# ma921/SOBER

Measured on AMD Instinct MI355X. Metric: recombination-step candidates/sec (N_rec=100000, N_nys=500, d=10, batch=100), higher is better.
Workload: dtype f64

## Files before the change

include/sober_hip.h:

```cpp
#ifndef SOBER_HIP_H
#define SOBER_HIP_H

#include <stdint.h>

#ifdef __cplusplus
extern "C" {
#endif

#define SOBER_ABI_VERSION 7

#define SOBER_KIND_RBF       0
#define SOBER_KIND_MATERN52  1
#define SOBER_KIND_TANIMOTO  2

#define SOBER_E_ARG      -1
#define SOBER_E_DIM      -2
#define SOBER_E_WS       -3
#define SOBER_E_EXCHANGE -5

int sober_abi_version(void);
int sober_diag_build(void);
int sober_reload_switches(void);
int sober_level_job_size(void);
int sober_nystrom_job_size(void);

int sober_padded_dim(int d);
int sober_bit_words(int d);

int sober_mt19937_uniform53(uint8_t* state, int64_t state_bytes, int64_t numel, double* out);
int sober_box_muller(const double* u, int64_t numel, double* out, void* stream);

int sober_scale_points(const double* X, int64_t n, int d, int64_t ldx,
                       const double* lengthscale, int ls_len,
                       double* out, int dt, void* stream);

int sober_scale_points_idx(const double* X, const int32_t* idx, int64_t n, int d, int64_t ldx, const double* lengthscale,
                           int ls_len, double* out, int dt, const double* gather_src, double* gather_out, void* stream);
int sober_pack_bits(const double* X, int64_t n, int d, int64_t ldx,
                    uint64_t* words, int nwords, double* norms, int32_t* bad_flag, void* stream);

int sober_pairwise(int kind, const void* a, const double* a_norm, int64_t m,
                   const void* b, const double* b_norm, const int32_t* idx, int64_t n,
                   int dt, double outputscale, double* out, int64_t ldo, void* stream);

int sober_kernel_matvec(int kind, const void* a, const double* a_norm, const double* v, int64_t m,
                        const void* b, const double* b_norm, int64_t n,
                        int dt, double outputscale, double c0, double* out, void* stream);

int sober_level_reduce(int kind, const void* rows, const double* rows_norm, int n_rows,
                       const void* cand, const double* cand_norm, int dt,
                       const int32_t* idx, int64_t pos0, int64_t count, int S,
                       const double* mu, const double* wmul, double outputscale,
                       int n_chunks, double* partG, int ldg, int col0,
                       double* partTot, int64_t tot_limit, void* stream);
int sober_aug_dim(int d);
int sober_augment_plan(const double* X_nys, int64_t M, int64_t ld_nys, const double* X_obs, int64_t n_obs, int64_t ld_obs,
                       const double* X_cand, int64_t N, int64_t ld_cand, int d, const double* lengthscale, int ls_len,
                       double* center, double* rows_aug, double* cand_aug, int da, void* stream);
int sober_augment_points(const double* X, int64_t n, int d, int64_t ldx, const double* lengthscale,
                         int ls_len, const double* center, int side, double* out, int da, void* stream);
int sober_level_reduce_mfma(int kind, const double* rows, int n_rows, const double* cand, int da,
                            const int32_t* idx, int64_t pos0, int64_t count, int S,
                            const double* mu, const double* wmul, double outputscale,
                            int n_chunks, double* partG, int ldg, int col0,
                            double* partTot, int64_t tot_limit, void* stream);

int64_t sober_nonzero_ws_bytes(int64_t N);
int sober_nonzero_i32(const double* mu, int64_t N, int32_t* idx_out, int64_t* count_out, void* ws, int64_t ws_bytes,
                      void* stream);

int sober_level_chunks(int n_rows, int64_t pos0, int64_t count, int S);
int sober_level_parts_mfma(int n_rows, int64_t pos0, int64_t count, int S);
int sober_level_parts_mfma_cap(int n_rows, int64_t e_total_ub, int S);

int sober_sum_partials(const double* partG, const double* partTot, int n_chunks, int n_rows,
                       int ldg, int S, const double* extraG, const double* extraTot,
                       int n_xchunks, int n_xcols, double* G, int ldo, double* tot, void* stream);

int sober_dgemm(int transa, int transb, int m, int n, int k, double alpha,
                const double* A, int lda, const double* B, int ldb,
                double beta, double* C, int ldc, void* stream);

int sober_barycentres(const double* Xtr, int ldx, int n, int S, const double* tot,
                      double* X_tmp, void* stream);
int sober_dgemm_coldiv_t(int m, int n, int k, const double* A, int lda, const double* B, int ldb, const double* coldiv,
                         double* Ct, int ldct, void* stream);

int sober_level_update(const int32_t* idx_cur, int64_t pos0, int64_t count, int S, int64_t E,
                       const int32_t* keep_rank, const double* w_star, const double* tot,
                       int n_keep, double* mu, int32_t* idx_new, int64_t new_pos0, void* stream);

int sober_scatter_weights(const int32_t* idx_cur, const int32_t* sel, const double* w, int n_sel,
                          double* mu, int64_t* out_idx, void* stream);

int sober_gather_f64(const double* src, const int32_t* idx, int64_t n, double* out, void* stream);
int sober_final_scatter(const int32_t* idx, int n, const int32_t* keep_rank, const double* w_star,
                        int64_t row_offset, double* mu, int64_t* out_idx, double* out_w, void* stream);
int sober_final_commit(const int32_t* idx, int n, const int32_t* keep_rank, const double* w_star, const int32_t* n_keep,
                       int64_t row_offset, double* mu, int64_t N, int64_t* out_idx, double* out_w, void* stream);

int sober_i64_to_i32(const int64_t* in, int64_t n, int32_t* out, void* stream);

int sober_car_pivot_host(double* h_Phi, int N, int m, double* h_mu);
int sober_car_pivot_host_fast(double* h_Phi, int N, int m, double* h_mu);

int sober_car_supported(int N, int m);
int64_t sober_car_ws_bytes(int N, int m);
int sober_car_device(const double* X, int ldx, int N, int m, const double* mu_in,
                     int32_t* keep_rank, double* w_star, int32_t* n_keep, double* mu_out,
                     double* phi_out, void* ws, int64_t ws_bytes, void* stream);
int sober_probe_rcp(const double* x, double* out, int64_t n, void* stream);

#define SOBER_CAR_DEFAULT 0
#define SOBER_CAR_SAFE 1
int sober_car_safe_supported(int N, int m);
int sober_car_giveup_forced(void);
int sober_car_device_ex(const double* X, int ldx, int N, int m, const double* mu_in,
                        int32_t* keep_rank, double* w_star, int32_t* n_keep, double* mu_out,
                        double* phi_out, void* ws, int64_t ws_bytes, int mode, void* stream);
int sober_obj_set_sums(const double* obj, const double* mu, const int32_t* idx, int64_t pos0, int64_t count, int S, int64_t E,
                       double* out, void* stream);
int sober_second_elimination(const double* phi, const double* objp, const double* w1, const int32_t* rank1, int n1,
                             int Nsets, int32_t* keep_rank, double* w_star, int32_t* n_keep, void* stream);
int sober_null_vector_supported(int nfun);
int sober_null_vector(const double* X, int ldx, int Nsets, int nfun, const int32_t* rank1, const int32_t* n_keep1, int n1,
                      double* null_row, int32_t* status, void* stream);
int sober_second_elimination_rows(const double* null_row, const double* obj_row, const double* w1, const int32_t* rank1,
                                  const int32_t* n_keep1, const int32_t* status, int n1, int Nsets, int32_t* keep_rank,
                                  double* w_star, int32_t* n_keep, void* stream);
int sober_obj_set_sums_queued(const double* obj, const double* mu, const int32_t* idx, int S, const int64_t* dR, int64_t R_known,
                              const double* tot, double* xcol, int ldx, double* ocol, void* stream);

int sober_car_mc_supported(int N, int m);
int64_t sober_car_mc_ws_bytes(int N, int m);
int sober_car_mc_device(const double* X, int ldx, int N, int m, const double* mu_in,
                        int32_t* keep_rank, double* w_star, int32_t* n_keep, double* mu_out,
                        double* phi_out, void* ws, int64_t ws_bytes, void* stream);
int sober_car_big_supported(int N, int m);
int64_t sober_car_big_ws_bytes(int N, int m);
int sober_car_big_device(const double* X, int ldx, int N, int m, const double* mu_in,
                         int32_t* keep_rank, double* w_star, int32_t* n_keep, double* mu_out,
                         double* phi_out, void* ws, int64_t ws_bytes, void* stream);
int sober_mc_selftest(const double* in, double* out, void* stream);

int sober_chol_max_n(void);
int sober_nystrom_max_n(void);
int sober_cholesky_probe_batched(const double* src, int n, int ld_src, const double* shifts, int n_shifts,
                                 double* work, int32_t* info, double* min_pivot, void* xinv_ws, int64_t ws_bytes,
                                 void* stream);
int sober_cholesky(double* A, int n, int ld, double shift, int32_t* info, double* min_pivot, void* stream);
int sober_cholesky_inv(double* A, int n, int ld, double shift, int32_t* info, double* min_pivot, double* xinv,
                       void* stream);
int sober_cholesky_inv_ratio(double* A, int n, int ld, double shift, int32_t* info, double* min_pivot, double* xinv,
                             double* ratio_out, void* stream);
int sober_trsm_blocks(const double* Y, int64_t m, int q, int ldy, const double* L, int ldl, const double* Xinv,
                      double* Q, int ldq, void* stream);
int sober_cholesky_probe(const double* src, int n, int ld_src, const double* shifts, int n_shifts,
                         double* work, int32_t* info, void* stream);
int sober_cholesky_probe_piv(const double* src, int n, int ld_src, const double* shifts, int n_shifts,
                             double* work, int32_t* info, double* min_pivot, void* stream);

int64_t sober_cholesky_probe_mc_ws_bytes(int n, int n_shifts);
int sober_cholesky_probe_mc(const double* src, int n, int ld_src, const double* shifts, int n_shifts,
                            double* work, int32_t* info, double* min_pivot, void* ws, int64_t ws_bytes,
                            void* stream);
int sober_abs_sym(const double* C, int n, int ld, double* out, int ldo, int32_t* flag, void* stream);
int sober_abs_sym_dmax(const double* C, int n, int ld, double* out, int ldo, int32_t* flag, double* dmax,
                       void* stream);

int sober_jitter_ladder(double* A, int n, int ld, int k, void* stream);
int sober_jitter_ladder_auto(double* A, int n, int ld, const int32_t* info, int n_rungs, int32_t* k_out,
                             void* stream);

int sober_level_reduce_tani_supported(int dt);
int sober_level_reduce_tani(const void* rows, const double* rows_norm, int n_rows, const void* cand,
                            const double* cand_norm, int dt, const int32_t* idx, int64_t pos0, int64_t count, int S,
                            const double* mu, const double* wmul, double outputscale, int n_chunks, double* partG,
                            int ldg, int col0, double* partTot, int64_t tot_limit, void* stream);

int sober_rank_scatter(const double* X, int ldx, int N, int n, const double* ocol, const int32_t* rank, int n1,
                       double* Xp, double* objp, void* stream);
int sober_set_i64(int64_t* dst, int64_t v, void* stream);

int sober_level_reduce_mfma_queued(int kind, const double* rows, int n_rows, const double* cand, int da,
                                   const int32_t* idx, int64_t count_ub, int S, int S_main, int leftover,
                                   const double* mu, const double* wmul, double outputscale, int n_chunks_ub,
                                   double* partG, int ldg, double* partTot, const int64_t* dR, void* stream);
int sober_level_reduce_mfma_queued_pair(int kind, const double* rows, int n_rows, const double* cand, int da,
                                        const int32_t* idx, int64_t count_ub, int S, int n_xcols, const double* mu,
                                        const double* wmul, double outputscale, int n_chunks_ub, double* partG,
                                        int ldg, double* partTot, int n_xchunks_ub, double* extraG, double* extraTot,
                                        const int64_t* dR, void* stream);
int sober_sum_partials_queued(const double* partG, const double* partTot, int n_rows, int ldg, int S,
                              const double* extraG, const double* extraTot, int n_xcols, double* G, int ldo,
                              double* tot, const int64_t* dR, int chunked, void* stream);
int sober_level_reduce_tani_queued(const void* rows, const double* rows_norm, int n_rows, const void* cand,
                                   const double* cand_norm, int dt, const int32_t* idx, int64_t count_ub, int S,
                                   int S_main, int leftover, const double* mu, const double* wmul, double outputscale,
                                   int n_chunks_ub, double* partG, int ldg, double* partTot, const int64_t* dR,
                                   void* stream);
int sober_level_reduce_tani_queued_pair(const void* rows, const double* rows_norm, int n_rows, const void* cand,
                                        const double* cand_norm, int dt, const int32_t* idx, int64_t count_ub, int S,
                                        int n_xcols, const double* mu, const double* wmul, double outputscale,
                                        int n_chunks_ub, double* partG, int ldg, double* partTot, int n_xchunks_ub,
                                        double* extraG, double* extraTot, const int64_t* dR, void* stream);
int sober_level_chunks_cap(int n_rows, int64_t e_total_ub, int S);
int sober_level_chunks_tani(int n_rows, int64_t pos0, int64_t count, int S);
int sober_level_chunks_tani_cap(int n_rows, int64_t e_total_ub, int S);
int sober_level_update_queued(const int32_t* idx_cur, int64_t R_ub, int S, const int32_t* keep_rank,
                              const double* w_star, const double* tot, double* mu, int32_t* idx_new,
                              const int64_t* dR_cur, int64_t* dR_next, int64_t R_ub_next, void* stream);

int sober_level_class_wpt(int n_rows, int64_t e_total, int S);
int sober_level_class_slots(int wpt);
int sober_level_reduce_mfma_wpt(int kind, const double* rows, int n_rows, const double* cand, int da,
                                const int32_t* idx, int64_t count, int S, const double* mu, const double* wmul,
                                double outputscale, int wpt, int n_chunks, double* partG, int ldg, double* partTot,
                                void* stream);
int sober_class_sum(const double* partG, const double* partTot, int n_chunks, int n_rows, int S, int CL,
                    double* Gc, double* totc, double* G, double* tot, void* stream);
int sober_class_derive_queued(const double* Gc, const double* totc, int n_rows, int S, int CL, const double* scale,
                              const int32_t* sof, double* Gn, double* totn, double* G, double* tot, const int64_t* dR,
                              void* stream);
int sober_level_update_queued_ex(const int32_t* idx_cur, int64_t R_ub, int S, const int32_t* keep_rank,
                                 const double* w_star, const double* tot, double* mu, int32_t* idx_new,
                                 const int64_t* dR_cur, int64_t* dR_next, int64_t R_ub_next, int need_keep,
                                 double* cls_scale, int32_t* cls_sof, int64_t R_known, void* stream);
int sober_level_update_queued_cls(const int32_t* idx_cur, int64_t R_ub, int S, const int32_t* keep_rank,
                                  const double* w_star, const double* tot, double* mu, int32_t* idx_new,
                                  const int64_t* dR_cur, int64_t* dR_next, int64_t R_ub_next, int need_keep,
                                  double* cls_scale, int32_t* cls_sof, void* stream);
#define SOBER_CLASS_MAX_DEPTH 4
int sober_level_class_depth(int variant, int n_rows, int64_t R, int S);

int64_t sober_kmeans_ws_bytes(int64_t N, int d, int K);
int64_t sober_kmeans_stat_offset(int64_t N, int d, int K);
int64_t sober_kmeans_ws_bytes_screened(int64_t N, int d, int K);
int sober_kmeans_lloyd(const double* X, int64_t N, int d, int K, int iters,
                       double* centroids, int32_t* labels, void* ws, int64_t ws_bytes, void* stream);

int sober_predict_fused_supported(int kind, int n_obs, int dt);
int sober_predict_fused(int kind, const void* obs, const double* obs_norm, int n_obs, const void* cand,
                        const double* cand_norm, int64_t N, int dt, double outputscale, const double* W, int ldw,
                        const double* alpha, double c0, double kxx_const, double noise, double* mean_out, double* var_out,
                        double eta, const double* eta_ptr, double* lfi_out, int log_flag, void* stream);
int sober_predict_fused_root(int kind, const void* obs, const double* obs_norm, int n_obs, const void* cand,
                             const double* cand_norm, int64_t N, int dt, double outputscale, const double* St, int ldst,
                             const int32_t* tri_flag, const double* alpha, double c0, double kxx_const, double noise,
                             double* mean_out, double* var_out, double eta, const double* eta_ptr, double* lfi_out, int log_flag,
                             void* stream);
int sober_predict_finish(const double* KX, const double* V, int n_obs, int64_t N, int64_t ld,
                         const double* mean, double kxx_const, const double* norms, double outputscale,
                         double noise, double* var_out, double eta, double* lfi_out, int log_flag,
                         void* stream);

int64_t sober_reduce_ws_bytes(int64_t n);
int sober_cleansing_weights(double* w, int64_t n, double eps, void* ws, int64_t ws_bytes, void* stream);

int sober_wkde_draw(const double* eps, int64_t n, int d, const int32_t* comp, const double* Xobs, int ldx,
                    const double* L, const double* lo, const double* hi, double* x, int32_t* inside,
                    void* stream);

int sober_level_gather(const double* Kmat, int n_rows, int64_t ldk, const int32_t* idx, int64_t pos0,
                       int64_t count, int S, const double* mu, const double* wmul, int n_chunks,
                       double* partG, int ldg, int col0, double* partTot, int64_t tot_limit, void* stream);

int sober_gspace_finish(double* K, const double* corr, int64_t n, int m, int64_t ldk, int64_t ldc,
                        const double* mug_cand, const double* mug_rows, void* stream);

#define SOBER_LEVEL_VALU        0
#define SOBER_LEVEL_MFMA        1
#define SOBER_LEVEL_GATHER      2
#define SOBER_LEVEL_TANI        3
#define SOBER_LEVEL_MAX_CHUNKS  64
#define SOBER_LEVEL_XS          16
typedef struct sober_level_job {
    int32_t variant, kind;
    const void* rows;   const double* rows_norm;
    const void* cand;   const double* cand_norm;
    int32_t n_rows, dim;
    int64_t kmat_ld;
    const double* wmul; double outputscale;
    int32_t S, n;
    const double* P;
    double *partG, *partTot, *extraG, *extraTot;
    double *G, *Xtr, *tot;
    double *X_tmp;
    int32_t* keep_rank;
    double *w_star, *mu_out;
    void* car_ws; int64_t car_ws_bytes;
    int32_t* h_flags;
    void* ev[4];
    const int32_t* idx; int64_t pos0, count, E;
    double* mu;
    int32_t phase;
    int64_t* dR; int64_t* h_dR;
    int32_t car_mode;
    uint64_t ev_used[2];
    int32_t class_depth;
    double* Gc[2]; double* totc[2];
    double* cls_scale; int32_t* cls_sof;
} sober_level_job;
#define SOBER_LEVEL_QUEUE 24
int sober_level_moments(const sober_level_job* job, void* stream);
int sober_level_car(const sober_level_job* job, void* stream);
int sober_level_car_retry(sober_level_job* job, void* stream);
#define SOBER_E_NOPROGRESS -4
int sober_level_loop(sober_level_job* job, int64_t R, int32_t* idx_a, int32_t* idx_b, int first_sums_ready,
                     void** events, int max_levels, int64_t* level_R, int32_t* n_levels, int64_t* R_final,
                     int32_t* in_b, void* stream);
typedef struct sober_obj_job {
    const double* obj;
    double* X_tmp;
    double* ocol;
    int32_t* kr1; double* w1; int32_t* nk1;
    double* null_row;
    int32_t* status;
} sober_obj_job;
int sober_obj_job_size(void);
int sober_level_loop_obj(sober_level_job* job, const sober_obj_job* obj_job, int64_t R, int32_t* idx_a, int32_t* idx_b,
                         int first_sums_ready, int max_levels, int64_t* level_R, int32_t* n_levels, int64_t* R_final,
                         int32_t* in_b, void* stream);
typedef int (*sober_allreduce_fn)(void* comm, double* buf, int64_t n, void* stream);
int sober_level_loop_sharded(sober_level_job* job, int rank, int world, int64_t* bounds, int32_t* idx_a,
                             int32_t* idx_b, int first_sums_ready, sober_allreduce_fn allreduce, void* comm,
                             int64_t R_stop, int max_levels, int64_t* level_R, int32_t* n_levels, int32_t* in_b,
                             void* stream);
int sober_rccl_load(const char* path);
int sober_rccl_unique_id(char* out128);
int sober_rccl_comm_init(const char* id128, int rank, int world, void** comm);
int sober_rccl_comm_destroy(void* comm);
int sober_rccl_allreduce_f64(void* comm, double* buf, int64_t n, void* stream);
int64_t sober_rccl_allreduce_ptr(void);

int64_t sober_peer_region_bytes(int64_t n_max);
int sober_peer_create(int rank, int world, int64_t n_max, void** comm, char* handle64);
int sober_peer_connect(void* comm, const char* handles);
int sober_peer_connect_ptrs(void* comm, void* const* regions);
int64_t sober_peer_region(void* comm);
int sober_peer_set_spin_limit(void* comm, unsigned spin_limit);
int sober_peer_allreduce_f64(void* comm, double* buf, int64_t n, void* stream);
int64_t sober_peer_allreduce_ptr(void);
int sober_peer_status(void* comm, double* restore, int64_t n, void* stream);
int sober_peer_destroy(void* comm);

int sober_level_final(const sober_level_job* job, const void* rows_sc, const double* rows_norm, const void* cand_sc,
                      const double* cand_norm, int dt, const int32_t* idx, int R, int64_t N, int64_t row_offset,
                      double* K, double* mu_live, int64_t* out_idx, double* out_w, void* stream);
int sober_plan_rows(int kind, const double* X_nys, int M, int64_t ld_nys, const double* X_obs, int n_obs,
                    int64_t ld_obs, int d, const double* lengthscale, int ls_len, double outputscale,
                    const double* S_cache, int ld_s, double* rows, int dt, double* Kall, double* W, double* T,
                    double* G, void* stream);

typedef struct sober_final_job {
    const void* rows_sc; const double* rows_norm;
    const void* cand_sc; const double* cand_norm;
    int32_t dt, done;
    int64_t N, row_offset;
    double *K, *mu_live;
    int64_t* out_idx; double* out_w;
    const double* cand_raw; int64_t ld_raw; int32_t d_raw, ls_len; const double* ls; double* sc_buf;
} sober_final_job;
int sober_level_final_job(const sober_level_job* job, const sober_final_job* final, const int32_t* idx, int R, void* stream);
int sober_final_job_size(void);
int sober_level_loop_final(sober_level_job* job, sober_final_job* final, int64_t R, int32_t* idx_a, int32_t* idx_b,
                           int first_sums_ready, void** events, int max_levels, int64_t* level_R, int32_t* n_levels,
                           int64_t* R_final, int32_t* in_b, void* stream);
int sober_projection(const double* Ut, int s, int M, const double* mean, const double* T, int n_obs, double* P,
                     void* stream);

typedef struct sober_nystrom_job {
    int32_t M, s, n_rungs, niter, probe_mc;
    int32_t reserved0;
    const double* G;
    const double* shifts;
    const double* R;
    double* C;
    double* chol_work;
    void* probe_ws; int64_t probe_ws_bytes;
    double* Y[2];
    double* Gm;
    double* xinv;
    void* flags_block; int64_t flags_bytes;
    void* h_flags_block;
    double* Ut;
    const double* T; int32_t n_obs;
    const double* mean_nys; double* P;
} sober_nystrom_job;
int64_t sober_nystrom_flags_bytes(int n_rungs, int niter);
int sober_nystrom_basis(const sober_nystrom_job* job, int phase, void* stream);

int sober_set_launch_events(void* start, void* stop);
int sober_record_event_pair(void* ev0, void* ev1, void* stream);

#ifdef __cplusplus
}
#endif
#endif
```

sober_amd/_native.py:

```python
from __future__ import annotations

import ctypes as C
import os
from typing import Optional

import torch

_HERE = os.path.dirname(os.path.abspath(__file__))
LIB_PATH = os.environ.get("SOBER_HIP_LIB") or os.path.join(_HERE, "libsober_hip.so")
ABI_VERSION = 7

KIND_RBF, KIND_MATERN52, KIND_TANIMOTO = 0, 1, 2
KIND_BY_NAME = {"rbf": KIND_RBF, "matern52": KIND_MATERN52, "tanimoto": KIND_TANIMOTO}

_vp, _i32, _i64, _f64 = C.c_void_p, C.c_int, C.c_int64, C.c_double

SIGNATURES = {
    "sober_abi_version": (_i32, []),
    "sober_diag_build": (_i32, []),
    "sober_reload_switches": (_i32, []),
    "sober_level_job_size": (_i32, []),
    "sober_nystrom_job_size": (_i32, []),
    "sober_final_job_size": (_i32, []),
    "sober_set_i64": (_i32, [_vp, _i64, _vp]),
    "sober_rank_scatter": (_i32, [_vp, _i32, _i32, _i32, _vp, _vp, _i32, _vp, _vp, _vp]),
    "sober_plan_rows": (_i32, [_i32, _vp, _i32, _i64, _vp, _i32, _i64, _i32, _vp, _i32, _f64, _vp, _i32, _vp, _i32, _vp,
                               _vp, _vp, _vp, _vp]),
    "sober_level_loop_final": (_i32, [_vp, _vp, _i64, _vp, _vp, _i32, _vp, _i32, _vp, _vp, _vp, _vp, _vp]),
    "sober_padded_dim": (_i32, [_i32]),
    "sober_bit_words": (_i32, [_i32]),
    "sober_scale_points": (_i32, [_vp, _i64, _i32, _i64, _vp, _i32, _vp, _i32, _vp]),
    "sober_augment_plan": (_i32, [_vp, _i64, _i64, _vp, _i64, _i64, _vp, _i64, _i64, _i32, _vp, _i32, _vp, _vp, _vp, _i32, _vp]),
    "sober_scale_points_idx": (_i32, [_vp, _vp, _i64, _i32, _i64, _vp, _i32, _vp, _i32, _vp, _vp, _vp]),
    "sober_pack_bits": (_i32, [_vp, _i64, _i32, _i64, _vp, _i32, _vp, _vp, _vp]),
    "sober_mt19937_uniform53": (_i32, [_vp, _i64, _i64, _vp]),
    "sober_box_muller": (_i32, [_vp, _i64, _vp, _vp]),
    "sober_pairwise": (_i32, [_i32, _vp, _vp, _i64, _vp, _vp, _vp, _i64, _i32, _f64, _vp, _i64, _vp]),
    "sober_kernel_matvec": (_i32, [_i32, _vp, _vp, _vp, _i64, _vp, _vp, _i64, _i32, _f64, _f64, _vp, _vp]),
    "sober_level_reduce": (_i32, [_i32, _vp, _vp, _i32, _vp, _vp, _i32, _vp, _i64, _i64, _i32, _vp, _vp,
                                  _f64, _i32, _vp, _i32, _i32, _vp, _i64, _vp]),
    "sober_nonzero_ws_bytes": (_i64, [_i64]),
    "sober_nonzero_i32": (_i32, [_vp, _i64, _vp, _vp, _vp, _i64, _vp]),
    "sober_dgemm_coldiv_t": (_i32, [_i32, _i32, _i32, _vp, _i32, _vp, _i32, _vp, _vp, _i32, _vp]),
    "sober_level_chunks": (_i32, [_i32, _i64, _i64, _i32]),
    "sober_level_parts_mfma": (_i32, [_i32, _i64, _i64, _i32]),
    "sober_level_parts_mfma_cap": (_i32, [_i32, _i64, _i32]),
    "sober_aug_dim": (_i32, [_i32]),
    "sober_augment_points": (_i32, [_vp, _i64, _i32, _i64, _vp, _i32, _vp, _i32, _vp, _i32, _vp]),
    "sober_level_reduce_mfma": (_i32, [_i32, _vp, _i32, _vp, _i32, _vp, _i64, _i64, _i32, _vp, _vp, _f64, _i32,
                                       _vp, _i32, _i32, _vp, _i64, _vp]),
    "sober_sum_partials": (_i32, [_vp, _vp, _i32, _i32, _i32, _i32, _vp, _vp, _i32, _i32, _vp, _i32, _vp, _vp]),
    "sober_dgemm": (_i32, [_i32, _i32, _i32, _i32, _i32, _f64, _vp, _i32, _vp, _i32, _f64, _vp, _i32, _vp]),
    "sober_barycentres": (_i32, [_vp, _i32, _i32, _i32, _vp, _vp, _vp]),
    "sober_level_update": (_i32, [_vp, _i64, _i64, _i32, _i64, _vp, _vp, _vp, _i32, _vp, _vp, _i64, _vp]),
    "sober_scatter_weights": (_i32, [_vp, _vp, _vp, _i32, _vp, _vp, _vp]),
    "sober_i64_to_i32": (_i32, [_vp, _i64, _vp, _vp]),
    "sober_car_pivot_host": (_i32, [_vp, _i32, _i32, _vp]),
    "sober_car_pivot_host_fast": (_i32, [_vp, _i32, _i32, _vp]),
    "sober_car_supported": (_i32, [_i32, _i32]),
    "sober_car_ws_bytes": (_i64, [_i32, _i32]),
    "sober_car_device": (_i32, [_vp, _i32, _i32, _i32, _vp, _vp, _vp, _vp, _vp, _vp, _vp, _i64, _vp]),
    "sober_probe_rcp": (_i32, [_vp, _vp, _i64, _vp]),
    "sober_second_elimination": (_i32, [_vp, _vp, _vp, _vp, _i32, _i32, _vp, _vp, _vp, _vp]),
    "sober_car_mc_supported": (_i32, [_i32, _i32]),
    "sober_car_mc_ws_bytes": (_i64, [_i32, _i32]),
    "sober_car_mc_device": (_i32, [_vp, _i32, _i32, _i32, _vp, _vp, _vp, _vp, _vp, _vp, _vp, _i64, _vp]),
    "sober_car_big_supported": (_i32, [_i32, _i32]),
    "sober_car_big_ws_bytes": (_i64, [_i32, _i32]),
    "sober_car_big_device": (_i32, [_vp, _i32, _i32, _i32, _vp, _vp, _vp, _vp, _vp, _vp, _vp, _i64, _vp]),
    "sober_car_device_ex": (_i32, [_vp, _i32, _i32, _i32, _vp, _vp, _vp, _vp, _vp, _vp, _vp, _i64, _i32, _vp]),
    "sober_obj_set_sums": (_i32, [_vp, _vp, _vp, _i64, _i64, _i32, _i64, _vp, _vp]),
    "sober_null_vector_supported": (_i32, [_i32]),
    "sober_null_vector": (_i32, [_vp, _i32, _i32, _i32, _vp, _vp, _i32, _vp, _vp, _vp]),
    "sober_second_elimination_rows": (_i32, [_vp, _vp, _vp, _vp, _vp, _vp, _i32, _i32, _vp, _vp, _vp, _vp]),
    "sober_obj_set_sums_queued": (_i32, [_vp, _vp, _vp, _i32, _vp, _i64, _vp, _vp, _i32, _vp, _vp]),
    "sober_obj_job_size": (_i32, []),
    "sober_level_loop_obj": (_i32, [_vp, _vp, _i64, _vp, _vp, _i32, _i32, _vp, _vp, _vp, _vp, _vp]),
    "sober_car_safe_supported": (_i32, [_i32, _i32]),
    "sober_car_giveup_forced": (_i32, []),
    "sober_final_commit": (_i32, [_vp, _i32, _vp, _vp, _vp, _i64, _vp, _i64, _vp, _vp, _vp]),
    "sober_level_car_retry": (_i32, [_vp, _vp]),
    "sober_mc_selftest": (_i32, [_vp, _vp, _vp]),
    "sober_chol_max_n": (_i32, []),
    "sober_nystrom_max_n": (_i32, []),
    "sober_cholesky_probe_batched": (_i32, [_vp, _i32, _i32, _vp, _i32, _vp, _vp, _vp, _vp, _i64, _vp]),
    "sober_cholesky": (_i32, [_vp, _i32, _i32, _f64, _vp, _vp, _vp]),
    "sober_cholesky_inv": (_i32, [_vp, _i32, _i32, _f64, _vp, _vp, _vp, _vp]),
    "sober_cholesky_inv_ratio": (_i32, [_vp, _i32, _i32, _f64, _vp, _vp, _vp, _vp, _vp]),
    "sober_trsm_blocks": (_i32, [_vp, _i64, _i32, _i32, _vp, _i32, _vp, _vp, _i32, _vp]),
    "sober_cholesky_probe": (_i32, [_vp, _i32, _i32, _vp, _i32, _vp, _vp, _vp]),
    "sober_cholesky_probe_piv": (_i32, [_vp, _i32, _i32, _vp, _i32, _vp, _vp, _vp, _vp]),
    "sober_cholesky_probe_mc_ws_bytes": (_i64, [_i32, _i32]),
    "sober_cholesky_probe_mc": (_i32, [_vp, _i32, _i32, _vp, _i32, _vp, _vp, _vp, _vp, _i64, _vp]),
    "sober_abs_sym": (_i32, [_vp, _i32, _i32, _vp, _i32, _vp, _vp]),
    "sober_abs_sym_dmax": (_i32, [_vp, _i32, _i32, _vp, _i32, _vp, _vp, _vp]),
    "sober_jitter_ladder": (_i32, [_vp, _i32, _i32, _i32, _vp]),
    "sober_jitter_ladder_auto": (_i32, [_vp, _i32, _i32, _vp, _i32, _vp, _vp]),
    "sober_kmeans_ws_bytes": (_i64, [_i64, _i32, _i32]),
    "sober_kmeans_stat_offset": (_i64, [_i64, _i32, _i32]),
    "sober_kmeans_ws_bytes_screened": (_i64, [_i64, _i32, _i32]),
    "sober_kmeans_lloyd": (_i32, [_vp, _i64, _i32, _i32, _i32, _vp, _vp, _vp, _i64, _vp]),
    "sober_predict_fused_supported": (_i32, [_i32, _i32, _i32]),
    "sober_predict_fused": (_i32, [_i32, _vp, _vp, _i32, _vp, _vp, _i64, _i32, _f64, _vp, _i32, _vp, _f64, _f64, _f64, _vp, _vp,
                                   _f64, _vp, _vp, _i32, _vp]),
    "sober_predict_fused_root": (_i32, [_i32, _vp, _vp, _i32, _vp, _vp, _i64, _i32, _f64, _vp, _i32, _vp, _vp, _f64, _f64, _f64, _vp,
                                        _vp, _f64, _vp, _vp, _i32, _vp]),
    "sober_predict_finish": (_i32, [_vp, _vp, _i32, _i64, _i64, _vp, _f64, _vp, _f64, _f64, _vp, _f64, _vp, _i32, _vp]),
    "sober_reduce_ws_bytes": (_i64, [_i64]),
    "sober_cleansing_weights": (_i32, [_vp, _i64, _f64, _vp, _i64, _vp]),
    "sober_level_gather": (_i32, [_vp, _i32, _i64, _vp, _i64, _i64, _i32, _vp, _vp, _i32, _vp, _i32, _i32, _vp, _i64,
                                  _vp]),
    "sober_gspace_finish": (_i32, [_vp, _vp, _i64, _i32, _i64, _i64, _vp, _vp, _vp]),
    "sober_wkde_draw": (_i32, [_vp, _i64, _i32, _vp, _vp, _i32, _vp, _vp, _vp, _vp, _vp, _vp]),
    "sober_level_moments": (_i32, [_vp, _vp]),
    "sober_level_car": (_i32, [_vp, _vp]),
    "sober_level_reduce_tani_supported": (_i32, [_i32]),
    "sober_level_reduce_tani": (_i32, [_vp, _vp, _i32, _vp, _vp, _i32, _vp, _i64, _i64, _i32, _vp, _vp, _f64, _i32, _vp,
                                       _i32, _i32, _vp, _i64, _vp]),
    "sober_level_loop_sharded": (_i32, [_vp, _i32, _i32, _vp, _vp, _vp, _i32, _vp, _vp, _i64, _i32, _vp, _vp, _vp, _vp]),
    "sober_rccl_load": (_i32, [C.c_char_p]),
    "sober_rccl_unique_id": (_i32, [_vp]),
    "sober_rccl_comm_init": (_i32, [_vp, _i32, _i32, _vp]),
    "sober_rccl_comm_destroy": (_i32, [_vp]),
    "sober_rccl_allreduce_f64": (_i32, [_vp, _vp, _i64, _vp]),
    "sober_rccl_allreduce_ptr": (_i64, []),
    "sober_peer_region_bytes": (_i64, [_i64]),
    "sober_peer_create": (_i32, [_i32, _i32, _i64, _vp, _vp]),
    "sober_peer_connect": (_i32, [_vp, C.c_char_p]),
    "sober_peer_connect_ptrs": (_i32, [_vp, _vp]),
    "sober_peer_region": (_i64, [_vp]),
    "sober_peer_set_spin_limit": (_i32, [_vp, C.c_uint]),
    "sober_peer_allreduce_f64": (_i32, [_vp, _vp, _i64, _vp]),
    "sober_peer_allreduce_ptr": (_i64, []),
    "sober_peer_status": (_i32, [_vp, _vp, _i64, _vp]),
    "sober_peer_destroy": (_i32, [_vp]),
    "sober_level_reduce_mfma_queued": (_i32, [_i32, _vp, _i32, _vp, _i32, _vp, _i64, _i32, _i32, _i32, _vp, _vp, _f64,
                                              _i32, _vp, _i32, _vp, _vp, _vp]),
    "sober_level_reduce_mfma_queued_pair": (_i32, [_i32, _vp, _i32, _vp, _i32, _vp, _i64, _i32, _i32, _vp, _vp, _f64, _i32,
                                                   _vp, _i32, _vp, _i32, _vp, _vp, _vp, _vp]),
    "sober_sum_partials_queued": (_i32, [_vp, _vp, _i32, _i32, _i32, _vp, _vp, _i32, _vp, _i32, _vp, _vp, _i32, _vp]),
    "sober_level_reduce_tani_queued": (_i32, [_vp, _vp, _i32, _vp, _vp, _i32, _vp, _i64, _i32, _i32, _i32, _vp, _vp, _f64,
                                              _i32, _vp, _i32, _vp, _vp, _vp]),
    "sober_level_reduce_tani_queued_pair": (_i32, [_vp, _vp, _i32, _vp, _vp, _i32, _vp, _i64, _i32, _i32, _vp, _vp, _f64, _i32,
                                                   _vp, _i32, _vp, _i32, _vp, _vp, _vp, _vp]),
    "sober_level_chunks_cap": (_i32, [_i32, _i64, _i32]),
    "sober_level_chunks_tani": (_i32, [_i32, _i64, _i64, _i32]),
    "sober_level_chunks_tani_cap": (_i32, [_i32, _i64, _i32]),
    "sober_level_update_queued": (_i32, [_vp, _i64, _i32, _vp, _vp, _vp, _vp, _vp, _vp, _vp, _i64, _vp]),
    "sober_level_update_queued_ex": (_i32, [_vp, _i64, _i32, _vp, _vp, _vp, _vp, _vp, _vp, _vp, _i64, _i32, _vp, _vp, _i64, _vp]),
    "sober_level_update_queued_cls": (_i32, [_vp, _i64, _i32, _vp, _vp, _vp, _vp, _vp, _vp, _vp, _i64, _i32, _vp, _vp, _vp]),
    "sober_level_class_wpt": (_i32, [_i32, _i64, _i32]),
    "sober_level_class_slots": (_i32, [_i32]),
    "sober_level_class_depth": (_i32, [_i32, _i32, _i64, _i32]),
    "sober_level_reduce_mfma_wpt": (_i32, [_i32, _vp, _i32, _vp, _i32, _vp, _i64, _i32, _vp, _vp, _f64, _i32, _i32, _vp, _i32,
                                           _vp, _vp]),
    "sober_class_sum": (_i32, [_vp, _vp, _i32, _i32, _i32, _i32, _vp, _vp, _vp, _vp, _vp]),
    "sober_class_derive_queued": (_i32, [_vp, _vp, _i32, _i32, _i32, _vp, _vp, _vp, _vp, _vp, _vp, _vp, _vp]),
    "sober_record_event_pair": (_i32, [_vp, _vp, _vp]),
    "sober_set_launch_events": (_i32, [_vp, _vp]),
    "sober_projection": (_i32, [_vp, _i32, _i32, _vp, _vp, _i32, _vp, _vp]),
    "sober_nystrom_flags_bytes": (_i64, [_i32, _i32]),
    "sober_nystrom_basis": (_i32, [_vp, _i32, _vp]),
    "sober_gather_f64": (_i32, [_vp, _vp, _i64, _vp, _vp]),
    "sober_final_scatter": (_i32, [_vp, _i32, _vp, _vp, _i64, _vp, _vp, _vp, _vp]),
    "sober_level_final": (_i32, [_vp, _vp, _vp, _vp, _vp, _i32, _vp, _i32, _i64, _i64, _vp, _vp, _vp, _vp, _vp]),
    "sober_level_final_job": (_i32, [_vp, _vp, _vp, _i32, _vp]),
    "sober_level_loop": (_i32, [_vp, _i64, _vp, _vp, _i32, _vp, _i32, _vp, _vp, _vp, _vp, _vp]),
}

LEVEL_VALU, LEVEL_MFMA, LEVEL_GATHER, LEVEL_TANI = 0, 1, 2, 3
LEVEL_MAX_CHUNKS, LEVEL_XS, LEVEL_QUEUE = 64, 16, 24


class FinalJob(C.Structure):
    _fields_ = [
        ("rows_sc", _vp), ("rows_norm", _vp), ("cand_sc", _vp), ("cand_norm", _vp),
        ("dt", _i32), ("done", _i32), ("N", _i64), ("row_offset", _i64),
        ("K", _vp), ("mu_live", _vp), ("out_idx", _vp), ("out_w", _vp),
        ("cand_raw", _vp), ("ld_raw", _i64), ("d_raw", _i32), ("ls_len", _i32), ("ls", _vp), ("sc_buf", _vp),
    ]


class ObjJob(C.Structure):
    _fields_ = [("obj", _vp), ("X_tmp", _vp), ("ocol", _vp), ("kr1", _vp), ("w1", _vp), ("nk1", _vp), ("null_row", _vp),
                ("status", _vp)]


class NystromJob(C.Structure):
    _fields_ = [
        ("M", _i32), ("s", _i32), ("n_rungs", _i32), ("niter", _i32), ("probe_mc", _i32), ("_pad0", _i32),
        ("G", _vp), ("shifts", _vp), ("R", _vp), ("C", _vp), ("chol_work", _vp),
        ("probe_ws", _vp), ("probe_ws_bytes", _i64),
        ("Y", _vp * 2), ("Gm", _vp), ("xinv", _vp),
        ("flags_block", _vp), ("flags_bytes", _i64), ("h_flags_block", _vp),
        ("Ut", _vp),
        ("T", _vp), ("n_obs", _i32), ("mean_nys", _vp), ("P", _vp),
    ]


class LevelJob(C.Structure):
    _fields_ = [
        ("variant", _i32), ("kind", _i32),
        ("rows", _vp), ("rows_norm", _vp), ("cand", _vp), ("cand_norm", _vp),
        ("n_rows", _i32), ("dim", _i32), ("kmat_ld", _i64),
        ("wmul", _vp), ("outputscale", _f64),
        ("S", _i32), ("n", _i32), ("P", _vp),
        ("partG", _vp), ("partTot", _vp), ("extraG", _vp), ("extraTot", _vp),
        ("G", _vp), ("Xtr", _vp), ("tot", _vp), ("X_tmp", _vp),
        ("keep_rank", _vp), ("w_star", _vp), ("mu_out", _vp),
        ("car_ws", _vp), ("car_ws_bytes", _i64), ("h_flags", _vp),
        ("ev", _vp * 4),
        ("idx", _vp), ("pos0", _i64), ("count", _i64), ("E", _i64), ("mu", _vp),
        ("phase", _i32),
        ("dR", _vp), ("h_dR", _vp),
        ("car_mode", _i32),
        ("ev_used", C.c_uint64 * 2),
        ("class_depth", _i32), ("Gc", _vp * 2), ("totc", _vp * 2), ("cls_scale", _vp), ("cls_sof", _vp),
    ]

E_DIM = -2
E_EXCHANGE = -5
CLASS_MAX_DEPTH = 4
CAR_DEFAULT, CAR_SAFE, CAR_HOST = 0, 1, 2

_lib: Optional[C.CDLL] = None


class SoberHipError(RuntimeError):
    pass


def load() -> C.CDLL:
    global _lib
    if _lib is not None:
        return _lib
    if not os.path.exists(LIB_PATH):
        raise SoberHipError(
            f"{LIB_PATH} not found: build it with `make -C sober_amd/csrc` "
            "(python -c 'import __graft_entry__ as g; g.build()').  sober_amd has no CPU fallback.")
    lib = C.CDLL(LIB_PATH)
    lib.sober_abi_version.restype = _i32
    got = lib.sober_abi_version()
    if got != ABI_VERSION:
        raise SoberHipError(f"libsober_hip ABI {got} != expected {ABI_VERSION}; rebuild (make -C sober_amd/csrc)")
    for name, (res, args) in SIGNATURES.items():
        fn = getattr(lib, name)
        fn.restype, fn.argtypes = res, args
    if lib.sober_diag_build() and os.environ.get("SOBER_ALLOW_DIAG_LIB") != "1":
        raise SoberHipError(f"{LIB_PATH} is a diagnostic build (in-kernel time stamps): not a library to compute with; "
                            "`make -C sober_amd/csrc` builds the product (SOBER_ALLOW_DIAG_LIB=1: the stamp scripts)")
    for name, cls in (("sober_level_job_size", LevelJob), ("sober_nystrom_job_size", NystromJob),
                      ("sober_final_job_size", FinalJob), ("sober_obj_job_size", ObjJob)):
        if getattr(lib, name)() != C.sizeof(cls):
            raise SoberHipError(f"{cls.__name__}: {C.sizeof(cls)} bytes here, {getattr(lib, name)()} in libsober_hip; "
                                "include/sober_hip.h and sober_amd/_native.py disagree")
    _lib = lib
    return lib


def reload_switches():
    load().sober_reload_switches()


def _check(rc: int, what: str):
    if rc == 0:
        return
    if rc < 0:
        msg = {-1: "bad argument", -2: "dimension not supported by the compiled tile set",
               -3: "workspace too small",
               -5: "a multi-workgroup Caratheodory kernel gave up waiting for a partner workgroup (no result)"}.get(rc, "error")
        raise SoberHipError(f"{what}: {msg} (code {rc})")
    raise SoberHipError(f"{what}: hipError_t {rc}")


def _ptr(t: Optional[torch.Tensor]) -> Optional[int]:
    return None if t is None else t.data_ptr()


_raw_stream = getattr(torch._C, "_cuda_getCurrentRawStream", None)


def _stream(t: torch.Tensor) -> Optional[int]:
    if not t.is_cuda:
        raise SoberHipError("sober_amd runs on the MI355X only: tensor is not on a HIP device")
    if _raw_stream is not None:
        return _raw_stream(t.device.index)
    return torch.cuda.current_stream(t.device).cuda_stream


def _req(t: torch.Tensor, dtype, name: str):
    if t.dtype != dtype or not t.is_contiguous():
        raise SoberHipError(f"{name}: need contiguous {dtype}, got {t.dtype} contiguous={t.is_contiguous()}")
    return t


def padded_dim(d: int, generic: bool = False) -> int:
    r = load().sober_padded_dim(d)
    if r == E_DIM and generic and d > 0:
        return (d + 3) // 4 * 4
    _check(min(r, 0), f"padded_dim({d})")
    return r


def bit_words(d: int, generic: bool = False) -> int:
    r = load().sober_bit_words(d)
    if r == E_DIM and generic and d > 0:
        return (d + 63) // 64
    _check(min(r, 0), f"bit_words({d})")
    return r


def fused_dim_supported(kind: int, d: int) -> bool:
    r = load().sober_bit_words(d) if kind == KIND_TANIMOTO else load().sober_padded_dim(d)
    return r > 0


def scale_points_idx(X, idx, n, lengthscale, out):
    _req(lengthscale, torch.float64, "lengthscale"); _req(out, torch.float64, "out"); _req(idx, torch.int32, "idx")
    if X.dtype != torch.float64 or X.stride(-1) != 1:
        raise SoberHipError("scale_points_idx: X must be float64 with unit inner stride")
    _check(load().sober_scale_points_idx(X.data_ptr(), idx.data_ptr(), int(n), X.shape[1], X.stride(0), lengthscale.data_ptr(),
                                         lengthscale.numel(), out.data_ptr(), out.shape[1], None, None, _stream(X)),
           "sober_scale_points_idx")


def scale_points(X, lengthscale, out):
    n, d = X.shape
    _req(X, torch.float64, "X"); _req(lengthscale, torch.float64, "lengthscale"); _req(out, torch.float64, "out")
    _check(load().sober_scale_points(X.data_ptr(), n, d, X.stride(0), lengthscale.data_ptr(),
                                     lengthscale.numel(), out.data_ptr(), out.shape[1], _stream(X)),
           "sober_scale_points")


def mt19937_uniform53(state, numel, out):
    _req(state, torch.uint8, "state"); _req(out, torch.float64, "out")
    if state.is_cuda or out.is_cuda or out.numel() < numel + 16:
        raise ValueError("mt19937_uniform53 takes host tensors, out of numel + 16 doubles")
    _check(load().sober_mt19937_uniform53(state.data_ptr(), state.numel(), numel, out.data_ptr()),
           "sober_mt19937_uniform53")


def box_muller(u, numel, out):
    _req(u, torch.float64, "u"); _req(out, torch.float64, "out")
    if u.numel() < numel + 16 or out.numel() < numel:
        raise ValueError("box_muller: u holds numel + 16 uniforms, out numel normals")
    _check(load().sober_box_muller(u.data_ptr(), numel, out.data_ptr(), _stream(out)), "sober_box_muller")


def pack_bits(X, words, norms, bad_flag):
    n, d = X.shape
    _req(X, torch.float64, "X"); _req(words, torch.int64, "words"); _req(norms, torch.float64, "norms")
    _req(bad_flag, torch.int32, "bad_flag")
    _check(load().sober_pack_bits(X.data_ptr(), n, d, X.stride(0), words.data_ptr(), words.shape[1],
                                  norms.data_ptr(), bad_flag.data_ptr(), _stream(X)), "sober_pack_bits")


def rank_scatter(X, n, ocol, rank, n1, Xp, objp):
    _req(X, torch.float64, "X"); _req(ocol, torch.float64, "ocol"); _req(rank, torch.int32, "rank")
    _check(load().sober_rank_scatter(X.data_ptr(), X.stride(0), X.shape[0], n, ocol.data_ptr(), rank.data_ptr(), n1,
                                     Xp.data_ptr(), objp.data_ptr(), _stream(X)), "sober_rank_scatter")


def plan_rows(kind, X_nys, X_obs, lengthscale, outputscale, S_cache, rows, Kall, W, T, G):
    M, d = X_nys.shape
    n_obs = 0 if X_obs is None else X_obs.shape[0]
    for t in (X_nys, X_obs, S_cache, rows, Kall, W, T, G):
        if t is not None and (t.dtype != torch.float64 or t.stride(-1) != 1):
            raise SoberHipError("plan_rows: float64 tensors with unit inner stride")
    _check(load().sober_plan_rows(kind, X_nys.data_ptr(), M, X_nys.stride(0), _ptr(X_obs), n_obs,
                                  X_obs.stride(0) if X_obs is not None else 0, d, lengthscale.data_ptr(),
                                  lengthscale.numel(), float(outputscale), _ptr(S_cache),
                                  S_cache.stride(0) if S_cache is not None else 0, rows.data_ptr(), rows.shape[1],
                                  _ptr(Kall), _ptr(W), _ptr(T), G.data_ptr(), _stream(G)), "sober_plan_rows")


def pairwise(kind, a, a_norm, b, b_norm, idx, n, dt, outputscale, out):
    _check(load().sober_pairwise(kind, a.data_ptr(), _ptr(a_norm), a.shape[0], b.data_ptr(), _ptr(b_norm),
                                 _ptr(idx), n, dt, float(outputscale), out.data_ptr(), out.stride(0),
                                 _stream(out)), "sober_pairwise")


def kernel_matvec(kind, a, a_norm, v, b, b_norm, dt, outputscale, c0, out):
    _check(load().sober_kernel_matvec(kind, a.data_ptr(), _ptr(a_norm), v.data_ptr(), a.shape[0],
                                      b.data_ptr(), _ptr(b_norm), b.shape[0], dt, float(outputscale),
                                      float(c0), out.data_ptr(), _stream(out)), "sober_kernel_matvec")


def nonzero_ws_bytes(N) -> int:
    r = load().sober_nonzero_ws_bytes(N)
    _check(min(int(r), 0), "sober_nonzero_ws_bytes")
    return int(r)


def nonzero_i32(mu, idx_out, count_out, ws):
    _req(mu, torch.float64, "mu"); _req(idx_out, torch.int32, "idx_out"); _req(count_out, torch.int64, "count_out")
    _check(load().sober_nonzero_i32(mu.data_ptr(), mu.numel(), idx_out.data_ptr(), count_out.data_ptr(), ws.data_ptr(),
                                    ws.numel() * ws.element_size(), _stream(mu)), "sober_nonzero_i32")


def level_chunks(n_rows, pos0, count, S) -> int:
    r = load().sober_level_chunks(n_rows, pos0, count, S)
    _check(min(r, 0), "sober_level_chunks")
    return r


def level_parts_mfma(n_rows, pos0, count, S) -> int:
    r = load().sober_level_parts_mfma(n_rows, pos0, count, S)
    _check(min(r, 0), "sober_level_parts_mfma")
    return r


def level_reduce(kind, rows, rows_norm, cand, cand_norm, dt, idx, idx_off, pos0, count, S, mu, wmul,
                 outputscale, n_chunks, partG, ldg, col0, partTot, tot_limit):
    _req(idx, torch.int32, "idx"); _req(mu, torch.float64, "mu")
    _check(load().sober_level_reduce(kind, rows.data_ptr(), _ptr(rows_norm), rows.shape[0], cand.data_ptr(),
                                     _ptr(cand_norm), dt, idx.data_ptr() + 4 * idx_off, pos0, count, S,
                                     mu.data_ptr(), _ptr(wmul), float(outputscale), n_chunks,
                                     partG.data_ptr(), ldg, col0, _ptr(partTot), tot_limit, _stream(mu)),
           "sober_level_reduce")


def aug_dim(d: int) -> int:
    r = load().sober_aug_dim(d)
    return r if r > 0 else -1


def augment_plan(X_nys, X_obs, X_cand, lengthscale, center, rows_aug, cand_aug):
    for t_, nm in ((X_nys, "X_nys"), (X_cand, "X_cand"), (X_obs, "X_obs")):
        if t_ is not None and (t_.dtype != torch.float64 or t_.stride(-1) != 1):
            raise SoberHipError(f"augment_plan: {nm} must be float64 with unit inner stride")
    _req(rows_aug, torch.float64, "rows_aug"); _req(cand_aug, torch.float64, "cand_aug"); _req(center, torch.float64, "center")
    n_obs = 0 if X_obs is None else X_obs.shape[0]
    _check(load().sober_augment_plan(X_nys.data_ptr(), X_nys.shape[0], X_nys.stride(0), _ptr(X_obs), n_obs,
                                     X_obs.stride(0) if n_obs else 0, X_cand.data_ptr(), X_cand.shape[0], X_cand.stride(0),
                                     X_nys.shape[1], lengthscale.data_ptr(), lengthscale.numel(), center.data_ptr(),
                                     rows_aug.data_ptr(), cand_aug.data_ptr(), rows_aug.shape[1], _stream(X_cand)),
           "sober_augment_plan")


def augment_points(X, lengthscale, center, side, out):
    n, d = X.shape
    _req(X, torch.float64, "X"); _req(out, torch.float64, "out"); _req(center, torch.float64, "center")
    _check(load().sober_augment_points(X.data_ptr(), n, d, X.stride(0), lengthscale.data_ptr(),
                                       lengthscale.numel(), center.data_ptr(), side, out.data_ptr(),
                                       out.shape[1], _stream(X)), "sober_augment_points")


def level_reduce_mfma(kind, rows, cand, da, idx, idx_off, pos0, count, S, mu, wmul, outputscale, n_chunks,
                      partG, ldg, col0, partTot, tot_limit):
    _req(idx, torch.int32, "idx"); _req(mu, torch.float64, "mu")
    _check(load().sober_level_reduce_mfma(kind, rows.data_ptr(), rows.shape[0], cand.data_ptr(), da,
                                          idx.data_ptr() + 4 * idx_off, pos0, count, S, mu.data_ptr(),
                                          _ptr(wmul), float(outputscale), n_chunks, partG.data_ptr(), ldg,
                                          col0, _ptr(partTot), tot_limit, _stream(mu)),
           "sober_level_reduce_mfma")


def sum_partials(partG, partTot, n_chunks, n_rows, ldg, S, extraG, extraTot, n_xchunks, n_xcols, G, tot):
    _check(load().sober_sum_partials(partG.data_ptr(), _ptr(partTot), n_chunks, n_rows, ldg, S,
                                     _ptr(extraG), _ptr(extraTot), n_xchunks, n_xcols, G.data_ptr(),
                                     G.stride(0), _ptr(tot), _stream(G)), "sober_sum_partials")


def dgemm(A, B, C_, transa=False, transb=False, alpha=1.0, beta=0.0):
    m, n = C_.shape
    k = A.shape[0] if transa else A.shape[1]
    for t, nm in ((A, "A"), (B, "B"), (C_, "C")):
        if t.dtype != torch.float64 or t.stride(1) != 1:
            raise SoberHipError(f"dgemm {nm}: need float64 with unit inner stride")
    ka = B.shape[1] if transb else B.shape[0]
    ma = A.shape[1] if transa else A.shape[0]
    na = B.shape[0] if transb else B.shape[1]
    if (ma, na, ka) != (m, n, k):
        raise SoberHipError(f"dgemm shape mismatch {A.shape} {B.shape} -> {C_.shape}")
    _check(load().sober_dgemm(int(transa), int(transb), m, n, k, float(alpha), A.data_ptr(), A.stride(0),
                              B.data_ptr(), B.stride(0), float(beta), C_.data_ptr(), C_.stride(0),
                              _stream(C_)), "sober_dgemm")


def barycentres(Xtr, n, S, tot, X_tmp):
    _check(load().sober_barycentres(Xtr.data_ptr(), Xtr.stride(0), n, S, _ptr(tot), X_tmp.data_ptr(),
                                    _stream(X_tmp)), "sober_barycentres")


def level_update(idx_cur, idx_off, pos0, count, S, E, keep_rank, w_star, tot, n_keep, mu, idx_new, new_pos0):
    _check(load().sober_level_update(idx_cur.data_ptr() + 4 * idx_off, pos0, count, S, E,
                                     keep_rank.data_ptr(), w_star.data_ptr(), tot.data_ptr(), n_keep,
                                     mu.data_ptr(), idx_new.data_ptr(), new_pos0, _stream(mu)),
           "sober_level_update")


def scatter_weights(idx_cur, sel, w, n_sel, mu, out_idx):
    _check(load().sober_scatter_weights(idx_cur.data_ptr(), sel.data_ptr(), w.data_ptr(), n_sel,
                                        mu.data_ptr(), out_idx.data_ptr(), _stream(mu)),
           "sober_scatter_weights")


def i64_to_i32(src, dst):
    _check(load().sober_i64_to_i32(src.data_ptr(), src.numel(), dst.data_ptr(), _stream(src)),
           "sober_i64_to_i32")


def car_pivot_host(Phi: torch.Tensor, mu: torch.Tensor, fast=None) -> int:
    if Phi.is_cuda or mu.is_cuda:
        raise SoberHipError("car_pivot_host takes host tensors")
    _req(Phi, torch.float64, "Phi"); _req(mu, torch.float64, "mu")
    N, m = Phi.shape
    fn = load().sober_car_pivot_host_fast if (fast or (fast is None and N > 200)) else load().sober_car_pivot_host
    r = fn(Phi.data_ptr(), N, m, mu.data_ptr())
    _check(min(r, 0), "sober_car_pivot_host")
    return r


_CAR_WS = {}


def car_supported(N: int, m: int) -> bool:
    return bool(load().sober_car_supported(N, m))


def car_safe_supported(N: int, m: int) -> bool:
    return bool(load().sober_car_safe_supported(N, m))


def probe_rcp(x):
    out = torch.empty_like(x)
    _check(load().sober_probe_rcp(x.data_ptr(), out.data_ptr(), x.numel(), _stream(x)), "sober_probe_rcp")
    return out


def car_device(X, mu_in, keep_rank, w_star, n_keep, mu_out, phi_out=None, multi_cu=False, mode=CAR_DEFAULT, big=False):
    N, n = X.shape
    lib = load()
    if mode != CAR_DEFAULT and not multi_cu and not big:
        nbytes = lib.sober_car_ws_bytes(N, n + 1)
        ws = _CAR_WS.get(X.device)
        if ws is None or ws.numel() * 8 < nbytes:
            ws = _CAR_WS[X.device] = torch.empty(max(nbytes // 8, 1), dtype=torch.float64, device=X.device)
        _check(lib.sober_car_device_ex(X.data_ptr(), X.stride(0), N, n + 1, mu_in.data_ptr(), keep_rank.data_ptr(),
                                       w_star.data_ptr(), n_keep.data_ptr(), mu_out.data_ptr(), _ptr(phi_out),
                                       ws.data_ptr(), nbytes, int(mode), _stream(X)), "sober_car_device_ex")
        return
    nbytes = max(lib.sober_car_ws_bytes(N, n + 1), lib.sober_car_mc_ws_bytes(N, n + 1) if multi_cu else 0,
                 lib.sober_car_big_ws_bytes(N, n + 1) if big else 0)
    ws = _CAR_WS.get(X.device)
    if ws is None or ws.numel() * 8 < nbytes:
        ws = torch.empty(max(nbytes // 8, 1), dtype=torch.float64, device=X.device)
        _CAR_WS[X.device] = ws
    fn, name = (lib.sober_car_big_device, "sober_car_big_device") if big else \
        (lib.sober_car_mc_device, "sober_car_mc_device") if multi_cu else (lib.sober_car_device, "sober_car_device")
    _check(fn(X.data_ptr(), X.stride(0), N, n + 1, mu_in.data_ptr(), keep_rank.data_ptr(),
              w_star.data_ptr(), n_keep.data_ptr(), mu_out.data_ptr(), _ptr(phi_out),
              ws.data_ptr(), nbytes, _stream(X)), name)


def obj_set_sums(obj, mu, idx, pos0, count, S, E, out):
    _req(obj, torch.float64, "obj"); _req(mu, torch.float64, "mu"); _req(idx, torch.int32, "idx"); _req(out, torch.float64, "out")
    _check(load().sober_obj_set_sums(obj.data_ptr(), mu.data_ptr(), idx.data_ptr(), int(pos0), int(count), int(S), int(E),
                                     out.data_ptr(), _stream(mu)), "sober_obj_set_sums")


def null_vector(X, nfun, rank1, n_keep1, n1, null_row, status):
    _check(load().sober_null_vector(X.data_ptr(), X.stride(0), X.shape[0], int(nfun), rank1.data_ptr(), n_keep1.data_ptr(),
                                    int(n1), null_row.data_ptr(), status.data_ptr(), _stream(X)), "sober_null_vector")


def second_elimination_rows(null_row, obj_row, w1, rank1, n_keep1, n1, keep_rank, w_star, n_keep, status=None):
    _check(load().sober_second_elimination_rows(null_row.data_ptr(), obj_row.data_ptr(), w1.data_ptr(), rank1.data_ptr(),
                                                n_keep1.data_ptr(), _ptr(status), int(n1), rank1.numel(), keep_rank.data_ptr(),
                                                w_star.data_ptr(), n_keep.data_ptr(), _stream(null_row)),
           "sober_second_elimination_rows")


def level_loop_obj(job, obj_job, R, idx_a, idx_b, first_sums_ready, stream):
    level_R = (_i64 * MAX_LEVELS)()
    n_levels, in_b, R_final = _i32(0), _i32(0), _i64(0)
    _check(load().sober_level_loop_obj(C.addressof(job), C.addressof(obj_job), R, idx_a.data_ptr(), idx_b.data_ptr(),
                                       int(bool(first_sums_ready)), MAX_LEVELS, level_R, C.byref(n_levels), C.byref(R_final),
                                       C.byref(in_b), stream), "sober_level_loop_obj")
    return list(level_R[:n_levels.value]), int(R_final.value), bool(in_b.value)


def second_elimination(phi, objp, w1, rank1, n1, keep_rank, w_star, n_keep):
    _check(load().sober_second_elimination(phi.data_ptr(), objp.data_ptr(), w1.data_ptr(), rank1.data_ptr(), int(n1),
                                           rank1.numel(), keep_rank.data_ptr(), w_star.data_ptr(), n_keep.data_ptr(),
                                           _stream(phi)), "sober_second_elimination")


def mc_selftest(x: torch.Tensor) -> torch.Tensor:
    out = torch.empty(128, dtype=torch.float64, device=x.device)
    _check(load().sober_mc_selftest(x.data_ptr(), out.data_ptr(), _stream(x)), "sober_mc_selftest")
    return out


def chol_max_n() -> int:
    return load().sober_chol_max_n()


def nystrom_max_n() -> int:
    return load().sober_nystrom_max_n()


def cholesky(A, shift, info, min_pivot=None):
    n = A.shape[0]
    _check(load().sober_cholesky(A.data_ptr(), n, A.stride(0), float(shift), info.data_ptr(), _ptr(min_pivot),
                                 _stream(A)), "sober_cholesky")


def cholesky_inv(A, shift, info, min_pivot, xinv, ratio=None):
    n = A.shape[0]
    if xinv.numel() < ((n + 31) // 32) * 1024:
        raise SoberHipError("cholesky_inv: xinv too small")
    _check(load().sober_cholesky_inv_ratio(A.data_ptr(), n, A.stride(0), float(shift), info.data_ptr(), _ptr(min_pivot),
                                           xinv.data_ptr(), _ptr(ratio), _stream(A)), "sober_cholesky_inv")


def trsm_blocks(Y, L, xinv, Q):
    m, q = Y.shape
    _check(load().sober_trsm_blocks(Y.data_ptr(), m, q, Y.stride(0), L.data_ptr(), L.stride(0), xinv.data_ptr(),
                                    Q.data_ptr(), Q.stride(0), _stream(Y)), "sober_trsm_blocks")


def cholesky_probe(src, shifts, work, info, min_pivot=None):
    n = src.shape[0]
    _check(load().sober_cholesky_probe_piv(src.data_ptr(), n, src.stride(0), shifts.data_ptr(), shifts.numel(),
                                           work.data_ptr(), info.data_ptr(), _ptr(min_pivot), _stream(src)),
           "sober_cholesky_probe_piv")


PROBE_NO_VERDICT = -7


def cholesky_probe_mc_ws_bytes(n: int, n_shifts: int) -> int:
    return int(load().sober_cholesky_probe_mc_ws_bytes(n, n_shifts))


def cholesky_probe_mc(src, shifts, work, info, min_pivot, ws):
    n = src.shape[0]
    _check(load().sober_cholesky_probe_mc(src.data_ptr(), n, src.stride(0), shifts.data_ptr(), shifts.numel(),
                                          work.data_ptr(), info.data_ptr(), _ptr(min_pivot), ws.data_ptr(),
                                          ws.numel() * ws.element_size(), _stream(src)), "sober_cholesky_probe_mc")


def abs_sym(C_, out, flag, dmax=None):
    n = C_.shape[0]
    _check(load().sober_abs_sym_dmax(C_.data_ptr(), n, C_.stride(0), out.data_ptr(), out.stride(0), flag.data_ptr(),
                                     _ptr(dmax), _stream(C_)), "sober_abs_sym")


def kmeans_lloyd(X, K, iters, centroids, labels):
    N, d = X.shape
    _req(X, torch.float64, "X"); _req(centroids, torch.float64, "centroids"); _req(labels, torch.int32, "labels")
    nbytes = int(load().sober_kmeans_ws_bytes(N, d, K))
    ws = torch.empty(max(nbytes, 8), dtype=torch.uint8, device=X.device)
    _check(load().sober_kmeans_lloyd(X.data_ptr(), N, d, K, iters, centroids.data_ptr(), labels.data_ptr(),
                                     ws.data_ptr(), nbytes, _stream(X)), "sober_kmeans_lloyd")


def predict_fused_supported(kind: int, n_obs: int, dt: int) -> bool:
    return bool(load().sober_predict_fused_supported(int(kind), int(n_obs), int(dt)))


def predict_fused(kind, obs, obs_norm, cand, cand_norm, n, dt, outputscale, W, alpha, c0, kxx_const, noise, mean_out,
                  var_out, eta=0.0, lfi_out=None, log=False, eta_dev=None, root_tri=None):
    if W.dtype != torch.float64 or W.dim() != 2 or W.stride(1) != 1:
        raise SoberHipError(f"predict_fused: W must be float64 with unit inner stride, got {W.dtype} strides {tuple(W.stride())}")
    if cand.dtype == torch.float64 and (cand.dim() != 2 or cand.stride(1) != 1 or cand.stride(0) != dt):
        raise SoberHipError(f"predict_fused: candidates must be rows of {dt} contiguous float64, got strides {tuple(cand.stride())}")
    for t_, nm in ((alpha, "alpha"), (mean_out, "mean_out"), (var_out, "var_out"), (lfi_out, "lfi_out"), (eta_dev, "eta_dev")):
        if t_ is not None:
            _req(t_, torch.float64, "predict_fused: " + nm)
    if alpha is not None and alpha.numel() != obs.shape[0]:
        raise SoberHipError(f"predict_fused: alpha has {alpha.numel()} entries for {obs.shape[0]} observations")
    if root_tri is not None:
        _req(root_tri, torch.int32, "predict_fused: root_tri")
        if W.shape[0] != W.shape[1] or W.shape[0] != obs.shape[0]:
            raise SoberHipError(f"predict_fused: the root must be {obs.shape[0]} x {obs.shape[0]}, got {tuple(W.shape)}")
        _check(load().sober_predict_fused_root(int(kind), obs.data_ptr(), _ptr(obs_norm), obs.shape[0], cand.data_ptr(),
                                               _ptr(cand_norm), int(n), int(dt), float(outputscale), W.data_ptr(), W.stride(0),
                                               root_tri.data_ptr(), _ptr(alpha), float(c0), float(kxx_const), float(noise),
                                               _ptr(mean_out), var_out.data_ptr(), float(eta), _ptr(eta_dev), _ptr(lfi_out),
                                               int(bool(log)), _stream(cand)), "sober_predict_fused_root")
        return
    _check(load().sober_predict_fused(int(kind), obs.data_ptr(), _ptr(obs_norm), obs.shape[0], cand.data_ptr(),
                                      _ptr(cand_norm), int(n), int(dt), float(outputscale), W.data_ptr(), W.stride(0),
                                      _ptr(alpha), float(c0), float(kxx_const), float(noise), _ptr(mean_out),
                                      var_out.data_ptr(), float(eta), _ptr(eta_dev), _ptr(lfi_out), int(bool(log)),
                                      _stream(cand)),
           "sober_predict_fused")


def predict_finish(KX, V, mean, kxx_const, norms, outputscale, noise, var_out, eta=0.0, lfi_out=None, log=False):
    n_obs, N = KX.shape
    _check(load().sober_predict_finish(KX.data_ptr(), V.data_ptr(), n_obs, N, KX.stride(0), _ptr(mean),
                                       float(kxx_const), _ptr(norms), float(outputscale), float(noise),
                                       var_out.data_ptr(), float(eta), _ptr(lfi_out), int(bool(log)),
                                       _stream(KX)), "sober_predict_finish")


def cleansing_weights(w, eps):
    _req(w, torch.float64, "weights")
    nbytes = load().sober_reduce_ws_bytes(w.numel())
    ws = torch.empty(nbytes // 8 + 1, dtype=torch.float64, device=w.device)
    _check(load().sober_cleansing_weights(w.data_ptr(), w.numel(), float(eps), ws.data_ptr(), nbytes,
                                          _stream(w)), "sober_cleansing_weights")


def wkde_draw(eps, comp, Xobs, L, lo, hi, x, inside):
    n, d = eps.shape
    _check(load().sober_wkde_draw(eps.data_ptr(), n, d, comp.data_ptr(), Xobs.data_ptr(), Xobs.stride(0),
                                  L.data_ptr(), lo.data_ptr() if lo is not None else None,
                                  hi.data_ptr() if hi is not None else None, x.data_ptr(),
                                  inside.data_ptr() if inside is not None else None, _stream(eps)),
           "sober_wkde_draw")


def level_gather(Kmat, idx, idx_off, pos0, count, S, mu, wmul, n_chunks, partG, ldg, col0, partTot, tot_limit):
    _req(idx, torch.int32, "idx"); _req(mu, torch.float64, "mu"); _req(Kmat, torch.float64, "Kmat")
    if Kmat.stride(1) != 1:
        raise SoberHipError("level_gather: Kmat needs unit inner stride")
    _check(load().sober_level_gather(Kmat.data_ptr(), Kmat.shape[1], Kmat.stride(0),
                                     idx.data_ptr() + 4 * idx_off, pos0, count, S, mu.data_ptr(), _ptr(wmul),
                                     n_chunks, partG.data_ptr(), ldg, col0, _ptr(partTot), tot_limit,
                                     _stream(partG)), "sober_level_gather")


def gspace_finish(K, corr, mug_cand, mug_rows):
    n, m = K.shape
    _check(load().sober_gspace_finish(K.data_ptr(), corr.data_ptr(), n, m, K.stride(0), corr.stride(0),
                                      mug_cand.data_ptr(), mug_rows.data_ptr(), _stream(K)), "sober_gspace_finish")


def car_ws_bytes(N: int, m: int) -> int:
    return load().sober_car_ws_bytes(N, m)


def level_moments(job: LevelJob, stream: int):
    _check(load().sober_level_moments(C.addressof(job), stream), "sober_level_moments")


def level_car(job: LevelJob, stream: int):
    _check(load().sober_level_car(C.addressof(job), stream), "sober_level_car")


def level_car_retry(job: LevelJob, stream: int) -> bool:
    rc = load().sober_level_car_retry(C.addressof(job), stream)
    if rc == E_EXCHANGE:
        return False
    _check(rc, "sober_level_car_retry")
    return True


E_NOPROGRESS = -4
MAX_LEVELS = 64


def level_loop(job: LevelJob, R: int, idx_a, idx_b, first_sums_ready: bool, events, stream: int, final: "FinalJob" = None):
    level_R = (_i64 * MAX_LEVELS)()
    n_levels, in_b, R_final = _i32(0), _i32(0), _i64(0)
    ev = None
    if events is not None:
        ev = (_vp * (4 * MAX_LEVELS))(*events)
    if final is not None:
        rc = load().sober_level_loop_final(C.addressof(job), C.addressof(final), R, idx_a.data_ptr(), idx_b.data_ptr(),
                                           int(bool(first_sums_ready)), ev, MAX_LEVELS, level_R, C.byref(n_levels),
                                           C.byref(R_final), C.byref(in_b), stream)
    else:
        rc = load().sober_level_loop(C.addressof(job), R, idx_a.data_ptr(), idx_b.data_ptr(), int(bool(first_sums_ready)),
                                     ev, MAX_LEVELS, level_R, C.byref(n_levels), C.byref(R_final), C.byref(in_b), stream)
    if rc == E_NOPROGRESS:
        raise RuntimeError("recombination made no progress (the Caratheodory step cancelled nothing, "
                           "SOBER/_rchq.py:241-242); the reference would loop forever here")
    if rc != E_EXCHANGE:
        _check(rc, "sober_level_loop")
    return list(level_R[:n_levels.value]), int(R_final.value), bool(in_b.value), rc == E_EXCHANGE


ALLREDUCE_FN = C.CFUNCTYPE(_i32, _vp, _vp, _i64, _vp)


def level_loop_sharded(job: LevelJob, rank: int, world: int, bounds, idx_a, idx_b, first_sums_ready: bool,
                       allreduce_ptr, comm_ptr, R_stop: int, stream: int):
    level_R = (_i64 * MAX_LEVELS)()
    n_levels, in_b = _i32(0), _i32(0)
    b = (_i64 * (world + 1))(*bounds)
    rc = load().sober_level_loop_sharded(C.addressof(job), rank, world, b, idx_a.data_ptr(), idx_b.data_ptr(),
                                         int(bool(first_sums_ready)), allreduce_ptr, comm_ptr, int(R_stop), MAX_LEVELS,
                                         level_R, C.byref(n_levels), C.byref(in_b), stream)
    if rc == E_NOPROGRESS:
        raise RuntimeError("recombination made no progress (the Caratheodory step cancelled nothing, "
                           "SOBER/_rchq.py:241-242); the reference would loop forever here")
    _check(rc, "sober_level_loop_sharded")
    return list(level_R[:n_levels.value]), list(b), bool(in_b.value)


class RcclComm:

    def __init__(self, dist, group, device):
        import torch as _t
        lib = load()
        path = os.path.join(os.path.dirname(_t.__file__), "lib", "librccl.so")
        _check(lib.sober_rccl_load(path.encode() if os.path.exists(path) else b""), "sober_rccl_load")
        rank, world = dist.get_rank(group), dist.get_world_size(group)
        buf = (C.c_char * 128)()
        if rank == 0:
            _check(lib.sober_rccl_unique_id(C.addressof(buf)), "sober_rccl_unique_id")
        on_dev = dist.get_backend(group) == "nccl"
        t = _t.frombuffer(bytearray(buf.raw), dtype=_t.uint8).clone()
        t = t.to(device) if on_dev else t
        dist.broadcast(t, src=dist.get_global_rank(group, 0) if group is not None else 0, group=group)
        ident = bytes(t.cpu().numpy().tobytes())
        self.handle = _vp()
        with _t.cuda.device(device):
            _check(lib.sober_rccl_comm_init(ident, rank, world, C.byref(self.handle)), "sober_rccl_comm_init")
        self.fn_ptr = lib.sober_rccl_allreduce_ptr()

    def close(self):
        if self.handle:
            load().sober_rccl_comm_destroy(self.handle)
            self.handle = _vp()


class PeerComm:

    def __init__(self, dist, group, device, n_max: int):
        import torch as _t
        lib = load()
        self.rank, self.world = dist.get_rank(group), dist.get_world_size(group)
        self.n_max, self.device, self.handle = int(n_max), device, _vp()
        self.fn_ptr = lib.sober_peer_allreduce_ptr()
        on_dev = dist.get_backend(group) == "nccl"
        hbuf = (C.c_char * 64)()
        with _t.cuda.device(device):
            rc = lib.sober_peer_create(self.rank, self.world, self.n_max, C.byref(self.handle), C.addressof(hbuf))
        mine = _t.frombuffer(bytearray(hbuf.raw), dtype=_t.uint8).clone()
        mine = _t.cat([mine, _t.tensor([0 if rc == 0 else 1], dtype=_t.uint8)])
        mine = mine.to(device) if on_dev else mine
        outs = [_t.empty_like(mine) for _ in range(self.world)]
        dist.all_gather(outs, mine, group=group)
        outs = [o.cpu() for o in outs]
        ok = rc == 0 and all(int(o[64]) == 0 for o in outs)
        if ok:
            allh = b"".join(bytes(o[:64].numpy().tobytes()) for o in outs)
            with _t.cuda.device(device):
                ok = lib.sober_peer_connect(self.handle, allh) == 0
        self.ok = self._agree(dist, group, on_dev, ok)
        if not self.ok:
            self.close()

    def _agree(self, dist, group, on_dev, ok: bool) -> bool:
        import torch as _t
        t = _t.tensor([1 if ok else 0], dtype=_t.int32)
        t = t.to(self.device) if on_dev else t
        dist.all_reduce(t, op=dist.ReduceOp.MIN, group=group)
        return bool(int(t.item()) == 1)

    def allreduce(self, buf, stream: int):
        _check(load().sober_peer_allreduce_f64(self.handle, buf.data_ptr(), buf.numel(), stream), "sober_peer_allreduce_f64")

    def status(self, stream: int = None) -> int:
        if stream is None:
            import torch as _t
            stream = _t.cuda.current_stream(self.device).cuda_stream
        return int(load().sober_peer_status(self.handle, None, 0, stream))

    def self_check(self, dist, group) -> bool:
        import torch as _t
        lib = load()
        on_dev = dist.get_backend(group) == "nccl"
        ok = True
        try:
            lib.sober_peer_set_spin_limit(self.handle, 1 << 21)
            dist.barrier(group=group)
            with _t.cuda.device(self.device):
                n = min(self.n_max, 4096)
                base = _t.arange(n, dtype=_t.float64, device=self.device)
                st = _t.cuda.current_stream(self.device)
                for rnd in range(4):
                    x = (base + rnd) * float(self.rank + 1)
                    self.allreduce(x, st.cuda_stream)
                    st.synchronize()
                    want = (base + rnd) * float(self.world * (self.world + 1) // 2)
                    ok = ok and self.status() == 0 and bool(_t.equal(x, want))
        except Exception:
            ok = False
        if self.handle:
            lib.sober_peer_set_spin_limit(self.handle, 1 << 27)
        self.ok = self._agree(dist, group, on_dev, ok)
        if not self.ok:
            self.close()
        return self.ok

    def close(self):
        if self.handle:
            load().sober_peer_destroy(self.handle)
            self.handle = _vp()


def level_final(job: LevelJob, rows, rows_norm, cand, cand_norm, dt, idx, R, N, row_offset, K, mu_live, out_idx,
                out_w, stream: int):
    _check(load().sober_level_final(C.addressof(job), rows.data_ptr(), _ptr(rows_norm), cand.data_ptr(),
                                    _ptr(cand_norm), dt, idx.data_ptr(), int(R), int(N), int(row_offset),
                                    K.data_ptr(), mu_live.data_ptr(), out_idx.data_ptr(), out_w.data_ptr(), stream),
           "sober_level_final")


def level_final_job(job: LevelJob, fin: "FinalJob", idx, R: int, stream: int):
    _check(load().sober_level_final_job(C.addressof(job), C.addressof(fin), idx.data_ptr(), int(R), stream), "sober_level_final_job")


def nystrom_flags_bytes(n_rungs: int, niter: int) -> int:
    return int(load().sober_nystrom_flags_bytes(n_rungs, niter))


def nystrom_basis(job: NystromJob, phase: int, stream: int):
    _check(load().sober_nystrom_basis(C.addressof(job), int(phase), stream), "sober_nystrom_basis")


def projection(Ut, mean, T, P):
    s_, M = Ut.shape
    _check(load().sober_projection(Ut.data_ptr(), s_, M, _ptr(mean), _ptr(T), 0 if T is None else T.shape[1], P.data_ptr(),
                                   _stream(P)), "sober_projection")


def record_event_pair(ev0, ev1, stream: int):
    _check(load().sober_record_event_pair(ev0.cuda_event, ev1.cuda_event, stream), "sober_record_event_pair")


def jitter_ladder_auto(A, info, k_out):
    _check(load().sober_jitter_ladder_auto(A.data_ptr(), A.shape[0], A.stride(0), info.data_ptr(), info.numel(),
                                           k_out.data_ptr(), _stream(A)), "sober_jitter_ladder_auto")


def jitter_ladder(A, k):
    _check(load().sober_jitter_ladder(A.data_ptr(), A.shape[0], A.stride(0), int(k), _stream(A)), "sober_jitter_ladder")
```

sober_amd/_ops_levels.py:

```python
from __future__ import annotations

import warnings

import torch

from . import _native as nat
from ._ops_plan import Plan


class _LevelOps:

    def _job(self, p: Plan, S: int, n: int = None) -> nat.LevelJob:
        n = p.n if n is None else n
        job = p.ws.get("job")
        if job is not None and job.S == S and job.n == n:
            if p.P is not None and job.P != p.P.data_ptr():
                if p.P.stride(0) != p.Mtot or p.P.stride(1) != 1:
                    p.P = p.P.contiguous()
                job.P = p.P.data_ptr()
            job.car_mode = min(self.car_mode, nat.CAR_SAFE)
            return job
        dev, f64 = self.device, torch.float64
        job = nat.LevelJob()
        Kmat = getattr(p, "Kmat", None)
        if Kmat is not None:
            job.variant, job.kind = nat.LEVEL_GATHER, 0
            job.cand, job.kmat_ld, job.n_rows = Kmat.data_ptr(), Kmat.stride(0), Kmat.shape[1]
            job.outputscale = 1.0
        elif p.da > 0:
            job.variant, job.kind = nat.LEVEL_MFMA, p.kind
            job.rows, job.cand, job.dim, job.n_rows = p.rows_aug.data_ptr(), p.cand_aug.data_ptr(), p.da, p.Mtot
            job.outputscale = float(p.spec.outputscale)
        else:
            tani = p.kind == nat.KIND_TANIMOTO and self.use_mfma and bool(nat.load().sober_level_reduce_tani_supported(p.rows.dt))
            job.variant, job.kind = (nat.LEVEL_TANI if tani else nat.LEVEL_VALU), p.kind
            job.rows, job.rows_norm = p.rows.data.data_ptr(), nat._ptr(p.rows.norm)
            job.cand, job.cand_norm = p.cand.data.data_ptr(), nat._ptr(p.cand.norm)
            job.dim, job.n_rows = p.rows.dt, p.Mtot
            job.outputscale = float(p.spec.outputscale)
        job.wmul = nat._ptr(p.wmul)
        if p.P is not None and (p.P.stride(0) != p.Mtot or p.P.stride(1) != 1):
            p.P = p.P.contiguous()
        job.S, job.n, job.P = S, n, nat._ptr(p.P)
        nr, mc, xs = job.n_rows, nat.LEVEL_MAX_CHUNKS, nat.LEVEL_XS
        w = p.ws
        w["partG"], w["partTot"] = torch.empty(mc * nr * S, dtype=f64, device=dev), torch.empty(mc * S, dtype=f64, device=dev)
        w["extraG"], w["extraTot"] = torch.empty(mc * nr * xs, dtype=f64, device=dev), torch.empty(mc * xs, dtype=f64, device=dev)
        w["G"] = torch.empty(nr, S, dtype=f64, device=dev)
        w["XT"] = torch.empty(n * S + S, dtype=f64, device=dev)
        w["Xtr"], w["tot"] = w["XT"][:n * S].view(n, S), w["XT"][n * S:]
        w["X_tmp"] = torch.empty(S, n, dtype=f64, device=dev)
        w["keep_rank"] = torch.empty(S + 1, dtype=torch.int32, device=dev)
        w["w_star"], w["mu_out"] = torch.empty(S, dtype=f64, device=dev), torch.empty(S, dtype=f64, device=dev)
        w["h_flags"] = torch.empty(S + 1, dtype=torch.int32, pin_memory=True)
        w["h_flags_np"] = w["h_flags"].numpy()
        if job.variant in (nat.LEVEL_MFMA, nat.LEVEL_TANI) and self.queue_levels:
            w["dR"] = torch.empty(nat.LEVEL_QUEUE + 1, dtype=torch.int64, device=dev)
            w["h_dR"] = torch.zeros(nat.LEVEL_QUEUE + 1, dtype=torch.int64, pin_memory=True)
            job.dR, job.h_dR = w["dR"].data_ptr(), w["h_dR"].data_ptr()
            if S % 2 == 0:
                cl = 1 << nat.CLASS_MAX_DEPTH
                w["Gc"] = [torch.empty(nr * S * (cl >> k), dtype=f64, device=dev) for k in (0, 1)]
                w["totc"] = [torch.empty(S * (cl >> k), dtype=f64, device=dev) for k in (0, 1)]
                w["cls_scale"], w["cls_sof"] = torch.empty(S, dtype=f64, device=dev), torch.empty(S, dtype=torch.int32, device=dev)
                for k in (0, 1):
                    job.Gc[k], job.totc[k] = w["Gc"][k].data_ptr(), w["totc"][k].data_ptr()
                job.cls_scale, job.cls_sof = w["cls_scale"].data_ptr(), w["cls_sof"].data_ptr()
        for k in ("partG", "partTot", "extraG", "extraTot", "G", "Xtr", "tot", "X_tmp", "keep_rank", "w_star", "mu_out",
                  "h_flags"):
            setattr(job, k, w[k].data_ptr())
        if nat.car_supported(S, n + 1):
            nbytes = nat.car_ws_bytes(S, n + 1)
            w["car_ws"] = torch.empty(max(nbytes // 8, 1), dtype=f64, device=dev)
            job.car_ws, job.car_ws_bytes = w["car_ws"].data_ptr(), nbytes
        job.car_mode = min(self.car_mode, nat.CAR_SAFE)
        w["job"] = job
        return job

    def _car_downgrade(self, mode: int, why: str):
        if mode > self.car_mode:
            self.car_mode = mode
            warnings.warn("sober_amd: a multi-workgroup Caratheodory launch gave up waiting for its partner workgroups "
                          f"({why}); this and the following steps use "
                          + ("the kernels without such waits (one workgroup, or a launch per dependency beyond batch 100)" if mode == nat.CAR_SAFE
                             else "the host LAPACK route")
                          + " for that step -- same result, slower")

    def level_moments(self, p: Plan, idx, pos0, count, S, E, mu, phase: int = 0, n: int = None):
        job = self._job(p, S, n)
        job.phase = phase
        if count <= 0 and phase != 2:
            p.ws["XT"].zero_(); p.ws["G"].zero_()
            return p.ws["Xtr"], p.ws["tot"]
        if phase == 2:
            nat.level_moments(job, nat._stream(p.ws["G"]))
            return p.ws["Xtr"], p.ws["tot"]
        nat._req(idx, torch.int32, "idx"); nat._req(mu, torch.float64, "mu")
        job.idx, job.pos0, job.count, job.E, job.mu = idx.data_ptr(), pos0, count, E, mu.data_ptr()
        job.class_depth = 0
        if phase == 1 and pos0 == 0 and count == E * S and job.Gc[0] and job.dR and self.level_classes:
            job.class_depth = int(nat.load().sober_level_class_depth(job.variant, job.n_rows, count, S))
        pair = None
        if self.prof is not None:
            n_left = max(pos0 + count - max(pos0, E * S), 0)
            pair, pair2 = self._prof_pair(), (self._prof_pair() if n_left > 0 else None)
            job.ev[0], job.ev[1] = pair[0].cuda_event, pair[1].cuda_event
            job.ev[2], job.ev[3] = (pair2[0].cuda_event, pair2[1].cuda_event) if pair2 else (None, None)
        nat.level_moments(job, nat._stream(mu))
        if pair is not None:
            self.prof.append((pair[0], pair[1], int(count * job.n_rows), 1))
            if pair2 is not None:
                self.prof.append((pair2[0], pair2[1], int(n_left * job.n_rows), 1))
            for k in range(4):
                job.ev[k] = None
        return p.ws["Xtr"], p.ws["tot"]

    def level_loop_obj(self, p: Plan, idx_cur, idx_new, R: int, S: int, mu, obj, sums_ready: bool):
        job = self._job(p, S)
        n = job.n
        if not self.queue_obj_levels or not self.queue_levels or not job.dR or job.variant not in (nat.LEVEL_MFMA, nat.LEVEL_TANI):
            return None
        if self.car_mode == nat.CAR_HOST or not self.obj_null_kernel or not self.car_supported(S, n + 2) \
                or not bool(nat.load().sober_null_vector_supported(n)):
            return None
        nat._req(mu, torch.float64, "mu"); nat._req(idx_cur, torch.int32, "idx"); nat._req(idx_new, torch.int32, "idx")
        nat._req(obj, torch.float64, "obj")
        dev, f64, w = self.device, torch.float64, p.ws
        if "obj_job" not in w:
            oj = nat.ObjJob()
            w["obj_X"] = torch.empty(S, n + 1, dtype=f64, device=dev)
            w["obj_f"] = torch.empty(3, S, dtype=f64, device=dev)
            w["obj_i"] = torch.empty(S + 2, dtype=torch.int32, device=dev)
            nbytes = nat.car_ws_bytes(S, n + 2)
            w["obj_car_ws"] = (torch.empty(max(nbytes // 8, 1), dtype=f64, device=dev), nbytes)
            oj.X_tmp, oj.ocol, oj.w1, oj.null_row = (w["obj_X"].data_ptr(), w["obj_f"][0].data_ptr(), w["obj_f"][1].data_ptr(),
                                                       w["obj_f"][2].data_ptr())
            oj.kr1, oj.nk1, oj.status = w["obj_i"].data_ptr(), w["obj_i"][S:].data_ptr(), w["obj_i"][S + 1:].data_ptr()
            w["obj_job"] = oj
        oj = w["obj_job"]
        oj.obj = obj.data_ptr()
        job.mu = mu.data_ptr()
        saved = (job.car_ws, job.car_ws_bytes, job.class_depth)
        job.car_ws, job.car_ws_bytes, job.class_depth = w["obj_car_ws"][0].data_ptr(), w["obj_car_ws"][1], 0
        try:
            level_R, R_final, in_b = nat.level_loop_obj(job, oj, R, idx_cur, idx_new, sums_ready, nat._stream(mu))
        finally:
            job.car_ws, job.car_ws_bytes, job.class_depth = saved
        if in_b:
            idx_cur, idx_new = idx_new, idx_cur
        return idx_cur, idx_new, R_final, len(level_R)

    def level_loop(self, p: Plan, idx_cur, idx_new, R: int, S: int, mu, sums_ready: bool, row_offset: int = 0):
        import math
        job = self._job(p, S)
        nat._req(mu, torch.float64, "mu"); nat._req(idx_cur, torch.int32, "idx"); nat._req(idx_new, torch.int32, "idx")
        job.mu = mu.data_ptr()
        if not sums_ready:
            job.class_depth = 0
        events = pairs = None
        if self.prof is not None:
            n_max = min(nat.MAX_LEVELS, int(math.log2(max(R / S, 1.0))) + 3)
            pairs = [(self._prof_pair(), self._prof_pair()) for _ in range(n_max)]
            events = [None] * (4 * nat.MAX_LEVELS)
            for l, (a, b) in enumerate(pairs):
                events[4 * l:4 * l + 4] = [a[0].cuda_event, a[1].cuda_event, b[0].cuda_event, b[1].cuda_event]
        fin = None
        p.ws.pop("final_done", None)
        if not p.weighted and getattr(p, "Kmat", None) is None and self.car_mode != nat.CAR_HOST and job.car_ws:
            fin = self._final_job(p, S, mu, row_offset)
        level_R, R_final, in_b, gave_up = nat.level_loop(job, R, idx_cur, idx_new, sums_ready, events, nat._stream(mu), fin)
        self.last_levels = {"R": [int(v) for v in level_R], "derived": int(job.class_depth) if sums_ready else 0}
        if fin is not None and fin.done:
            n_keep = int(p.ws["h_flags_np"][S])
            if n_keep >= 0:
                lst = idx_new if in_b else idx_cur
                p.ws["final_done"] = (lst.data_ptr(), R_final, row_offset, p._fin_out[0][:n_keep], p._fin_out[1][:n_keep])
        if job.car_mode > min(self.car_mode, nat.CAR_SAFE):
            self._car_downgrade(nat.CAR_SAFE, "level loop")
        if gave_up:
            self._car_downgrade(nat.CAR_HOST, "level loop")
        if pairs is not None:
            for l, (a, b) in enumerate(pairs):
                Rl = level_R[l] if l < len(level_R) else 0
                both = not ((job.ev_used[1] >> l) & 1)
                for which, pr, ent in ((0, a, Rl + (Rl % S if both else 0)), (1, b, Rl % S)):
                    if (job.ev_used[which] >> l) & 1 and not (l == 0 and sums_ready):
                        self.prof.append((pr[0], pr[1], int(ent * job.n_rows), 1))
                    else:
                        self._ev_pool.append(pr)
        return (idx_new, idx_cur, R_final) if in_b else (idx_cur, idx_new, R_final)

    def level_loop_sharded(self, p: Plan, idx_cur, idx_new, bounds, S: int, mu, sums_ready: bool, comm, R_stop: int):
        job = self._job(p, S)
        nat._req(mu, torch.float64, "mu"); nat._req(idx_cur, torch.int32, "idx"); nat._req(idx_new, torch.int32, "idx")
        job.mu = mu.data_ptr()
        job.class_depth = 0
        fn_ptr, comm_ptr, keep = comm.native_allreduce(p.ws["XT"], self.device)
        _, new_bounds, in_b = nat.level_loop_sharded(job, comm.rank, comm.world, bounds, idx_cur, idx_new, sums_ready,
                                                     fn_ptr, comm_ptr, R_stop, nat._stream(mu))
        del keep
        if job.car_mode > min(self.car_mode, nat.CAR_SAFE):
            self._car_downgrade(nat.CAR_SAFE, "sharded level loop")
        return (idx_new, idx_cur, new_bounds) if in_b else (idx_cur, idx_new, new_bounds)

    def _final_job(self, p: Plan, S: int, mu, row_offset: int = 0):
        dev = self.device
        f = nat.FinalJob()
        f.rows_sc, f.rows_norm = p.rows.data.data_ptr(), nat._ptr(p.rows.norm)
        if p.cand is not None:
            f.cand_sc, f.cand_norm = p.cand.data.data_ptr(), nat._ptr(p.cand.norm)
        else:
            Xr, ls = p.cand_raw, p.spec.lengthscale
            f.cand_sc, f.cand_norm = None, None
            f.cand_raw, f.ld_raw, f.d_raw = Xr.data_ptr(), Xr.stride(0), Xr.shape[1]
            f.ls, f.ls_len = ls.data_ptr(), ls.numel()
            f.sc_buf = self._buf(p, "sc_final", S * p.rows.dt).data_ptr()
        f.dt, f.done, f.N, f.row_offset = p.rows.dt, 0, mu.numel(), row_offset
        p._fin_out = (torch.empty(S, dtype=torch.int64, device=dev), torch.empty(S, dtype=torch.float64, device=dev))
        f.K, f.mu_live = self._buf(p, "K_final", p.Mtot * S).data_ptr(), self._buf(p, "mu_live", S).data_ptr()
        f.out_idx, f.out_w = p._fin_out[0].data_ptr(), p._fin_out[1].data_ptr()
        return f

    def level_final(self, p: Plan, idx_cur, R: int, S: int, mu, row_offset: int):
        if p.weighted or getattr(p, "Kmat", None) is not None or not nat.car_supported(R, p.n + 1) \
                or self.car_mode == nat.CAR_HOST or (self.car_mode == nat.CAR_SAFE and not nat.car_safe_supported(R, p.n + 1)):
            return None
        done = p.ws.pop("final_done", None)
        if done is not None:
            if done[:3] != (idx_cur.data_ptr(), R, row_offset):
                raise nat.SoberHipError("level_final: the final level that rode in level_loop was another one")
            return done[3], done[4]
        job = self._job(p, S)
        if not job.car_ws:
            return None
        dev = self.device
        job.mu = mu.data_ptr()
        fin = self._final_job(p, S, mu, row_offset)
        out_idx, out_w = p._fin_out
        st = torch.cuda.current_stream(dev)
        nat.level_final_job(job, fin, idx_cur, R, st.cuda_stream)
        st.synchronize()
        n_keep = int(p.ws["h_flags_np"][S])
        if n_keep < 0:
            if job.car_mode == nat.CAR_DEFAULT and nat.car_safe_supported(R, p.n + 1):
                self._car_downgrade(nat.CAR_SAFE, "final level")
                return self.level_final(p, idx_cur, R, S, mu, row_offset)
            self._car_downgrade(nat.CAR_HOST, "final level")
            return None
        return out_idx[:n_keep], out_w[:n_keep]

    def level_flat(self, p: Plan):
        return p.ws["XT"]

    def level_car(self, p: Plan, S: int):
        job = self._job(p, S)
        st = torch.cuda.current_stream(self.device)
        nat.level_car(job, st.cuda_stream)
        st.synchronize()
        flags = p.ws["h_flags_np"]
        if int(flags[S]) < 0:
            if not nat.level_car_retry(job, st.cuda_stream):
                self._car_downgrade(nat.CAR_HOST, "level")
                return None
            self._car_downgrade(nat.CAR_SAFE, "level")
        return p.ws["keep_rank"][:S], p.ws["w_star"], flags[:S].copy(), int(flags[S])

    def level_barycentres(self, p: Plan):
        return p.ws["X_tmp"], p.ws["tot"]

    def level_trace(self, p: Plan):
        return self.to_host(p.ws["X_tmp"], p.ws["tot"], p.ws["w_star"])

    def direct_columns(self, p: Plan, idx, count):
        dev = self.device
        K = torch.empty(p.Mtot, count, dtype=torch.float64, device=dev)
        if p.cand is not None:
            nat.pairwise(p.kind, p.rows.data, p.rows.norm, p.cand.data, p.cand.norm, idx, count, p.rows.dt,
                         p.spec.outputscale, K)
        else:
            sc = torch.empty(count, p.rows.dt, dtype=torch.float64, device=dev)
            nat.scale_points_idx(p.cand_raw, idx, count, p.spec.lengthscale, sc)
            nat.pairwise(p.kind, p.rows.data, p.rows.norm, sc, None, None, count, p.rows.dt, p.spec.outputscale, K)
        if p.weighted:
            K = K * p.wmul[idx[:count].long()].unsqueeze(0)
        Xtr = torch.empty(p.n, count, dtype=torch.float64, device=dev)
        nat.dgemm(p.P, K, Xtr)
        out = torch.empty(count, p.n, dtype=torch.float64, device=dev)
        nat.barycentres(Xtr, p.n, count, None, out)
        return out

    def barycentres(self, Xtr, tot):
        n, S = Xtr.shape
        out = torch.empty(S, n, dtype=torch.float64, device=self.device)
        nat.barycentres(Xtr, n, S, tot, out)
        return out

    def car_supported(self, N, m):
        if not nat.car_supported(N, m) or self.car_mode == nat.CAR_HOST:
            return False
        return self.car_mode == nat.CAR_DEFAULT or nat.car_safe_supported(N, m)

    def car_device(self, X, mu_in, phi_out=None):
        N = X.shape[0]
        dev = self.device
        keep_rank = torch.empty(N, dtype=torch.int32, device=dev)
        w_star = torch.empty(N, dtype=torch.float64, device=dev)
        n_keep = torch.empty(1, dtype=torch.int32, device=dev)
        mu_out = torch.empty(N, dtype=torch.float64, device=dev)
        nat.car_device(X, mu_in, keep_rank, w_star, n_keep, mu_out, phi_out=phi_out, mode=min(self.car_mode, nat.CAR_SAFE))
        return keep_rank, w_star, n_keep, mu_out

    def car_device_checked(self, X, mu_in, phi_out=None, also=()):
        N, m = X.shape[0], X.shape[1] + 1
        for _ in range(2):
            if not self.car_supported(N, m):
                return None
            keep_rank, w_star, n_keep_d, _mu = self.car_device(X, mu_in, phi_out)
            host = self.to_host(keep_rank, n_keep_d, *also)
            n_keep = int(host[1][0])
            if n_keep >= 0:
                return keep_rank, w_star, host[0], n_keep, host[2:]
            self._car_downgrade(nat.CAR_SAFE if nat.car_safe_supported(N, m) and self.car_mode == nat.CAR_DEFAULT
                                else nat.CAR_HOST, "Caratheodory step")
        return None

    def car_obj_device(self, X, mu_in, obj_head=None):
        N, n1f = X.shape
        dev = self.device
        n1 = n1f + 1
        if self.obj_null_kernel and bool(nat.load().sober_null_vector_supported(n1f - 1)) and self.car_supported(N, n1f + 1):
            for _ in range(2):
                flags = torch.empty(2 * N + 3, dtype=torch.int32, device=dev)
                keep_rank, n_keep, nk1_d, status, kr1 = flags[:N], flags[N:N + 1], flags[N + 1:N + 2], flags[N + 2:N + 3], flags[N + 3:]
                w1 = torch.empty(N, dtype=torch.float64, device=dev)
                mu1 = torch.empty(N, dtype=torch.float64, device=dev)
                nat.car_device(X, mu_in, kr1, w1, nk1_d, mu1, mode=min(self.car_mode, nat.CAR_SAFE))
                null_row = torch.empty(N, dtype=torch.float64, device=dev)
                nat.null_vector(X, n1f - 1, kr1, nk1_d, n1, null_row, status)
                ocol = (X[:, n1f - 1] if obj_head is None else obj_head[:N]).contiguous()
                w_star = torch.empty(N, dtype=torch.float64, device=dev)
                nat.second_elimination_rows(null_row, ocol, w1, kr1, nk1_d, n1, keep_rank, w_star, n_keep, status=status)
                (fl_h,) = self.to_host(flags)
                keep_h, nk_h, nk1, st_h, kr1_h = fl_h[:N], int(fl_h[N]), int(fl_h[N + 1]), int(fl_h[N + 2]), fl_h[N + 3:]
                if nk1 == n1 and st_h == 0:
                    return keep_rank, w_star, keep_h, nk_h, (kr1_h, w1, n1)
                if nk1 >= 0:
                    return None
                self._car_downgrade(nat.CAR_SAFE if nat.car_safe_supported(N, n1f + 1) and self.car_mode == nat.CAR_DEFAULT
                                    else nat.CAR_HOST, "Caratheodory step")
                if not self.car_supported(N, n1f + 1):
                    return None
            return None
        for _ in range(2):
            if not self.car_supported(N, n1f + 1) or not self.car_supported(n1, n1f):
                return None
            kr1, w1, nk1_d, _mu = self.car_device(X, mu_in)
            Xp = torch.zeros(n1, n1f - 1, dtype=torch.float64, device=dev)
            objp = torch.zeros(n1, dtype=torch.float64, device=dev)
            ocol = (X[:, n1f - 1] if obj_head is None else obj_head[:N]).contiguous()
            nat.rank_scatter(X, n1f - 1, ocol, kr1, n1, Xp, objp)
            phi = torch.empty(n1, 1, dtype=torch.float64, device=dev)
            scratch = [torch.empty(n1, dtype=t_, device=dev) for t_ in (torch.int32, torch.float64, torch.float64)]
            nkx = torch.empty(1, dtype=torch.int32, device=dev)
            nat.car_device(Xp, w1[:n1].contiguous(), scratch[0], scratch[1], nkx, scratch[2], phi_out=phi)
            keep_rank = torch.empty(N, dtype=torch.int32, device=dev)
            w_star = torch.empty(N, dtype=torch.float64, device=dev)
            n_keep = torch.empty(1, dtype=torch.int32, device=dev)
            nat.second_elimination(phi, objp, w1, kr1, n1, keep_rank, w_star, n_keep)
            (kr1_h, nk1_h, keep_h, nk_h) = self.to_host(kr1, nk1_d, keep_rank, n_keep)
            nk1 = int(nk1_h[0])
            if nk1 < 0:
                self._car_downgrade(nat.CAR_SAFE if nat.car_safe_supported(N, n1f + 1) and self.car_mode == nat.CAR_DEFAULT
                                    else nat.CAR_HOST, "Caratheodory step")
                continue
            if nk1 != n1:
                return None
            return keep_rank, w_star, keep_h, int(nk_h[0]), (kr1_h, w1, n1)
        return None

    def obj_set_sums(self, obj, mu, idx_cur, pos0, count, S, E):
        out = torch.empty(S, dtype=torch.float64, device=self.device)
        nat.obj_set_sums(obj, mu, idx_cur, pos0, count, S, E, out)
        return out

    def level_update(self, idx_cur, pos0, count, S, E, keep_rank, w_star, tot, n_keep, mu, idx_new, new_pos0):
        nat.level_update(idx_cur, 0, pos0, count, S, E, keep_rank, w_star, tot, n_keep, mu, idx_new, new_pos0)

    def scatter_weights(self, idx_cur, sel, w, mu):
        out = torch.empty(sel.numel(), dtype=torch.int64, device=self.device)
        if sel.numel():
            nat.scatter_weights(idx_cur, sel, w, sel.numel(), mu, out)
        return out
```

sober_amd/csrc/level_exec.cpp:

```cpp
#include <hip/hip_runtime.h>
#include <cstdio>
#include <cstdlib>

#include "../../include/sober_hip.h"
#include "switches.hpp"

extern "C" int sober_level_job_size(void) { return (int)sizeof(sober_level_job); }
extern "C" int sober_obj_job_size(void) { return (int)sizeof(sober_obj_job); }

#define LX_TRY(call)                 \
    do {                             \
        const int rc_ = (call);      \
        if (rc_ != 0) return rc_;    \
    } while (0)

static inline bool lx_timed_in_dispatch(const sober_level_job* j) {
    return j->variant == SOBER_LEVEL_MFMA || j->variant == SOBER_LEVEL_TANI;
}
#define LX_EVENTS_BEFORE(A, B)                                                                   \
    if ((A) && (B)) {                                                                            \
        if (lx_timed_in_dispatch(j)) { LX_TRY(sober_set_launch_events((A), (B))); }              \
        else { const hipError_t e_ = hipEventRecord((hipEvent_t)(A), (hipStream_t)stream); if (e_ != hipSuccess) return (int)e_; } \
    }
#define LX_EVENTS_AFTER(A, B)                                                                    \
    if ((A) && (B) && !lx_timed_in_dispatch(j)) {                                                \
        const hipError_t e_ = hipEventRecord((hipEvent_t)(B), (hipStream_t)stream);              \
        if (e_ != hipSuccess) return (int)e_;                                                    \
    }

static int lx_reduce(const sober_level_job* j, const int32_t* idx, int64_t pos0, int64_t count, int S, int n_chunks,
                     double* partG, double* partTot, int64_t tot_limit, void* stream) {
    switch (j->variant) {
        case SOBER_LEVEL_MFMA:
            return sober_level_reduce_mfma(j->kind, (const double*)j->rows, j->n_rows, (const double*)j->cand, j->dim,
                                           idx, pos0, count, S, j->mu, j->wmul, j->outputscale, n_chunks, partG, S, 0,
                                           partTot, tot_limit, stream);
        case SOBER_LEVEL_VALU:
            return sober_level_reduce(j->kind, j->rows, j->rows_norm, j->n_rows, j->cand, j->cand_norm, j->dim, idx,
                                      pos0, count, S, j->mu, j->wmul, j->outputscale, n_chunks, partG, S, 0, partTot,
                                      tot_limit, stream);
        case SOBER_LEVEL_TANI:
            return sober_level_reduce_tani(j->rows, j->rows_norm, j->n_rows, j->cand, j->cand_norm, j->dim, idx, pos0, count,
                                           S, j->mu, j->wmul, j->outputscale, n_chunks, partG, S, 0, partTot, tot_limit,
                                           stream);
        case SOBER_LEVEL_GATHER:
            return sober_level_gather((const double*)j->cand, j->n_rows, j->kmat_ld, idx, pos0, count, S, j->mu,
                                      j->wmul, n_chunks, partG, S, 0, partTot, tot_limit, stream);
        default:
            return SOBER_E_ARG;
    }
}

extern "C" int sober_level_class_depth(int variant, int n_rows, int64_t R, int S) {
    if (n_rows <= 0 || R <= 0 || S <= 0 || (S & 1) || sober::switches().level_no_classes) return 0;
    if (variant != SOBER_LEVEL_MFMA && variant != SOBER_LEVEL_TANI) return 0;
    int D = 0;
    while (D < SOBER_CLASS_MAX_DEPTH) {
        const int64_t SC = (int64_t)S << (D + 1);
        if (R % SC != 0 || R / SC < 2) break;
        int slots;
        if (variant == SOBER_LEVEL_MFMA) {
            const int wpt = sober_level_class_wpt(n_rows, R / SC, (int)SC);
            slots = wpt > 0 ? sober_level_class_slots(wpt) : 0;
        } else {
            slots = sober_level_chunks_tani(n_rows, 0, R, (int)SC);
            const int64_t rb = (n_rows + 255) / 256;
            const int64_t wg_c = (int64_t)slots * ((SC + 15) / 16 + 1) * rb;
            const int64_t wg_0 = (int64_t)sober_level_chunks_tani(n_rows, 0, R, S) * ((S + 15) / 16 + 1) * rb;
            if (slots > 0 && wg_c * 100 < wg_0 * 85) break;
        }
        if (slots <= 0 || slots * (1 << (D + 1)) > SOBER_LEVEL_MAX_CHUNKS) break;
        ++D;
    }
    return D;
}

static int lx_class_first(const sober_level_job* j, void* stream) {
    const int S = j->S, D = j->class_depth, CL = 1 << D, SC = S * CL;
    if ((j->variant != SOBER_LEVEL_MFMA && j->variant != SOBER_LEVEL_TANI) || D < 1 || D > SOBER_CLASS_MAX_DEPTH ||
        j->pos0 != 0 || j->count % SC != 0 || j->count / SC < 2 || !j->Gc[0] || !j->totc[0])
        return SOBER_E_ARG;
    int nch;
    if (j->variant == SOBER_LEVEL_MFMA) {
        const int wpt = sober_level_class_wpt(j->n_rows, j->count / SC, SC);
        if (wpt <= 0) return wpt < 0 ? wpt : SOBER_E_ARG;
        nch = sober_level_class_slots(wpt);
        if (nch <= 0 || nch * CL > SOBER_LEVEL_MAX_CHUNKS) return SOBER_E_WS;
        LX_EVENTS_BEFORE(j->ev[0], j->ev[1])
        LX_TRY(sober_level_reduce_mfma_wpt(j->kind, (const double*)j->rows, j->n_rows, (const double*)j->cand, j->dim, j->idx,
                                           j->count, SC, j->mu, j->wmul, j->outputscale, wpt, nch, j->partG, SC, j->partTot,
                                           stream));
    } else {
        nch = sober_level_chunks_tani(j->n_rows, 0, j->count, SC);
        if (nch <= 0 || nch * CL > SOBER_LEVEL_MAX_CHUNKS) return nch <= 0 ? nch : SOBER_E_WS;
        LX_EVENTS_BEFORE(j->ev[0], j->ev[1])
        LX_TRY(sober_level_reduce_tani(j->rows, j->rows_norm, j->n_rows, j->cand, j->cand_norm, j->dim, j->idx, 0, j->count, SC,
                                       j->mu, j->wmul, j->outputscale, nch, j->partG, SC, 0, j->partTot, j->count, stream));
    }
    return sober_class_sum(j->partG, j->partTot, nch, j->n_rows, S, CL, j->Gc[0], j->totc[0], j->G, j->tot, stream);
}

extern "C" int sober_level_moments(const sober_level_job* j, void* stream) {
    if (!j || !j->G || !j->tot || j->n_rows <= 0 || j->S <= 0 || j->n <= 0 || j->phase < 0 || j->phase > 2)
        return SOBER_E_ARG;
    const int S = j->S;
    if (j->phase == 2) {
        if (!j->P || !j->Xtr) return SOBER_E_ARG;
        return sober_dgemm(0, 0, j->n, S, j->n_rows, 1.0, j->P, j->n_rows, j->G, S, 0.0, j->Xtr, S, stream);
    }
    if (!j->cand || !j->idx || !j->mu || !j->partG || !j->partTot || (j->phase == 0 && (!j->P || !j->Xtr)))
        return SOBER_E_ARG;
    if (j->count <= 0 || j->pos0 < 0 || j->E < 0) return SOBER_E_ARG;
    if (j->phase == 1 && j->class_depth > 0) return lx_class_first(j, stream);
    const int64_t ES = j->E * S;
    const bool mfma = j->variant == SOBER_LEVEL_MFMA;
    const bool tani_k = j->variant == SOBER_LEVEL_TANI;
    const int n_chunks = mfma ? sober_level_parts_mfma(j->n_rows, j->pos0, j->count, S)
                              : (tani_k ? sober_level_chunks_tani(j->n_rows, j->pos0, j->count, S)
                                        : sober_level_chunks(j->n_rows, j->pos0, j->count, S));
    if (n_chunks <= 0 || n_chunks > SOBER_LEVEL_MAX_CHUNKS) return n_chunks <= 0 ? n_chunks : SOBER_E_WS;
    LX_EVENTS_BEFORE(j->ev[0], j->ev[1])
    LX_TRY(lx_reduce(j, j->idx, j->pos0, j->count, S, n_chunks, j->partG, j->partTot, ES, stream));
    LX_EVENTS_AFTER(j->ev[0], j->ev[1])
    const int64_t lo = j->pos0 > ES ? j->pos0 : ES;
    const int64_t n_left = j->pos0 + j->count - lo;
    int n_xchunks = 0;
    if (n_left > 0) {
        if (!j->extraG || !j->extraTot) return SOBER_E_ARG;
        n_xchunks = mfma ? sober_level_parts_mfma(j->n_rows, 0, n_left, SOBER_LEVEL_XS)
                         : (tani_k ? sober_level_chunks_tani(j->n_rows, 0, n_left, SOBER_LEVEL_XS)
                                   : sober_level_chunks(j->n_rows, 0, n_left, SOBER_LEVEL_XS));
        if (n_xchunks <= 0 || n_xchunks > SOBER_LEVEL_MAX_CHUNKS) return n_xchunks <= 0 ? n_xchunks : SOBER_E_WS;
        LX_EVENTS_BEFORE(j->ev[2], j->ev[3])
        LX_TRY(lx_reduce(j, j->idx + (lo - j->pos0), 0, n_left, SOBER_LEVEL_XS, n_xchunks, j->extraG, j->extraTot,
                         n_left, stream));
        LX_EVENTS_AFTER(j->ev[2], j->ev[3])
    }
    LX_TRY(sober_sum_partials(j->partG, j->partTot, n_chunks, j->n_rows, S, S, n_left > 0 ? j->extraG : nullptr,
                              n_left > 0 ? j->extraTot : nullptr, n_xchunks, SOBER_LEVEL_XS, j->G, S, j->tot, stream));
    if (j->phase == 1) return 0;
    return sober_dgemm(0, 0, j->n, S, j->n_rows, 1.0, j->P, j->n_rows, j->G, S, 0.0, j->Xtr, S, stream);
}

extern "C" int sober_level_car(const sober_level_job* j, void* stream) {
    if (!j || !j->Xtr || !j->tot || !j->X_tmp || !j->keep_rank || !j->w_star || !j->mu_out || !j->car_ws || !j->h_flags)
        return SOBER_E_ARG;
    const int S = j->S, n = j->n;
    if (!sober_car_supported(S, n + 1)) return SOBER_E_DIM;
    LX_TRY(sober_barycentres(j->Xtr, S, n, S, j->tot, j->X_tmp, stream));
    LX_TRY(sober_car_device_ex(j->X_tmp, n, S, n + 1, j->tot, j->keep_rank, j->w_star, j->keep_rank + S, j->mu_out,
                               nullptr, j->car_ws, j->car_ws_bytes, j->car_mode, stream));
    const hipError_t e = hipMemcpyAsync(j->h_flags, j->keep_rank, sizeof(int32_t) * (size_t)(S + 1),
                                        hipMemcpyDeviceToHost, (hipStream_t)stream);
    return e == hipSuccess ? 0 : (int)e;
}

extern "C" int sober_level_car_retry(sober_level_job* j, void* stream) {
    if (!j || !j->X_tmp || !j->tot || !j->keep_rank || !j->w_star || !j->mu_out || !j->car_ws || !j->h_flags) return SOBER_E_ARG;
    const int S = j->S, n = j->n;
    if (j->car_mode == SOBER_CAR_SAFE || !sober_car_safe_supported(S, n + 1)) return SOBER_E_EXCHANGE;
    j->car_mode = SOBER_CAR_SAFE;
    LX_TRY(sober_car_device_ex(j->X_tmp, n, S, n + 1, j->tot, j->keep_rank, j->w_star, j->keep_rank + S, j->mu_out,
                               nullptr, j->car_ws, j->car_ws_bytes, SOBER_CAR_SAFE, stream));
    hipError_t e = hipMemcpyAsync(j->h_flags, j->keep_rank, sizeof(int32_t) * (size_t)(S + 1), hipMemcpyDeviceToHost,
                                  (hipStream_t)stream);
    if (e == hipSuccess) e = hipStreamSynchronize((hipStream_t)stream);
    if (e != hipSuccess) return (int)e;
    return j->h_flags[S] < 0 ? SOBER_E_EXCHANGE : 0;
}

static int lx_chunks(int n_rows, int64_t e_total, int S) { return sober_level_parts_mfma_cap(n_rows, e_total, S); }

static int lx_loop_queued(sober_level_job* j, const sober_obj_job* oj, int64_t R0, int32_t* idx_a, int32_t* idx_b,
                          int first_sums_ready, void** events, int max_levels, int64_t* level_R, int* done, int64_t* R_out,
                          void* stream) {
    const int S = j->S, n = j->n, b = n + 1;
    *done = 0;
    *R_out = R0;
    int64_t Rlo[SOBER_LEVEL_QUEUE + 1], Rub[SOBER_LEVEL_QUEUE + 1];
    Rlo[0] = Rub[0] = R0;
    int L = 0;
    while (L < SOBER_LEVEL_QUEUE && L < max_levels && Rlo[L] > S) {
        Rlo[L + 1] = (Rlo[L] / S) * b;
        Rub[L + 1] = (Rub[L] / S) * b + (Rlo[L] == Rub[L] ? Rub[L] % S : S - 1);
        ++L;
    }
    if (L < 2) return 0;
    if (!sober_car_supported(S, oj ? b + 1 : b)) return SOBER_E_DIM;
    if (oj && (!sober_null_vector_supported(n) || b + 1 > 512)) return SOBER_E_DIM;
    int D = 0;
    if (first_sums_ready && j->class_depth > 0 && !oj) {
        D = j->class_depth;
        if ((j->variant != SOBER_LEVEL_MFMA && j->variant != SOBER_LEVEL_TANI) || D > SOBER_CLASS_MAX_DEPTH || D >= L ||
            R0 % ((int64_t)S << D) != 0 ||
            !j->Gc[0] || !j->Gc[1] || !j->totc[0] || !j->totc[1] || !j->cls_scale || !j->cls_sof)
            return SOBER_E_ARG;
    }
    hipStream_t st = (hipStream_t)stream;
    if (!first_sums_ready) LX_TRY(sober_set_i64(j->dR, R0, stream));
    hipError_t e = hipSuccess;
    for (int l = 0; l < L; ++l) {
        int32_t* cur = (l & 1) ? idx_b : idx_a;
        int32_t* nxt = (l & 1) ? idx_a : idx_b;
        for (int k = 0; k < 4; ++k) j->ev[k] = events ? events[4 * l + k] : nullptr;
        if (l >= 1 && l <= D) {
            LX_TRY(sober_class_derive_queued(j->Gc[(l - 1) & 1], j->totc[(l - 1) & 1], j->n_rows, S, 1 << (D - l + 1),
                                             j->cls_scale, j->cls_sof, j->Gc[l & 1], j->totc[l & 1], j->G, j->tot, j->dR + l,
                                             stream));
        } else if (!(l == 0 && first_sums_ready)) {
            const bool tani = j->variant == SOBER_LEVEL_TANI;
            const int64_t e_ub = (Rub[l] + S - 1) / S, ex_ub = (S - 1 + SOBER_LEVEL_XS - 1) / SOBER_LEVEL_XS;
            const int nch = tani ? sober_level_chunks_tani_cap(j->n_rows, e_ub, S) : lx_chunks(j->n_rows, e_ub, S);
            const int nxch = tani ? sober_level_chunks_tani_cap(j->n_rows, ex_ub, SOBER_LEVEL_XS) : lx_chunks(j->n_rows, ex_ub, SOBER_LEVEL_XS);
            if (nch <= 0 || nch > SOBER_LEVEL_MAX_CHUNKS || nxch <= 0 || nxch > SOBER_LEVEL_MAX_CHUNKS) return SOBER_E_WS;
            LX_EVENTS_BEFORE(j->ev[0], j->ev[1])
            if (j->ev[0] && j->ev[1]) j->ev_used[0] |= 1ull << l;
            const bool no_left = Rlo[l] == Rub[l] && Rub[l] % S == 0;
            if (tani && !no_left && !sober::switches().level_two_launches) {
                LX_TRY(sober_level_reduce_tani_queued_pair(j->rows, j->rows_norm, j->n_rows, j->cand, j->cand_norm, j->dim, cur,
                                                           Rub[l], S, SOBER_LEVEL_XS, j->mu, j->wmul, j->outputscale, nch,
                                                           j->partG, S, j->partTot, nxch, j->extraG, j->extraTot, j->dR + l,
                                                           stream));
            } else if (tani) {
                LX_TRY(sober_level_reduce_tani_queued(j->rows, j->rows_norm, j->n_rows, j->cand, j->cand_norm, j->dim, cur,
                                                      Rub[l], S, S, 0, j->mu, j->wmul, j->outputscale, nch, j->partG, S,
                                                      j->partTot, j->dR + l, stream));
                if (!no_left) {
                    LX_EVENTS_BEFORE(j->ev[2], j->ev[3])
                    if (j->ev[2] && j->ev[3]) j->ev_used[1] |= 1ull << l;
                    LX_TRY(sober_level_reduce_tani_queued(j->rows, j->rows_norm, j->n_rows, j->cand, j->cand_norm, j->dim, cur,
                                                          S - 1, SOBER_LEVEL_XS, S, 1, j->mu, j->wmul, j->outputscale, nxch,
                                                          j->extraG, SOBER_LEVEL_XS, j->extraTot, j->dR + l, stream));
                }
            } else if (no_left || sober::switches().level_two_launches) {
                LX_TRY(sober_level_reduce_mfma_queued(j->kind, (const double*)j->rows, j->n_rows, (const double*)j->cand,
                                                      j->dim, cur, Rub[l], S, S, 0, j->mu, j->wmul, j->outputscale, nch,
                                                      j->partG, S, j->partTot, j->dR + l, stream));
                if (!no_left) {
                    LX_EVENTS_BEFORE(j->ev[2], j->ev[3])
                    if (j->ev[2] && j->ev[3]) j->ev_used[1] |= 1ull << l;
                    LX_TRY(sober_level_reduce_mfma_queued(j->kind, (const double*)j->rows, j->n_rows, (const double*)j->cand,
                                                          j->dim, cur, S - 1, SOBER_LEVEL_XS, S, 1, j->mu, j->wmul,
                                                          j->outputscale, nxch, j->extraG, SOBER_LEVEL_XS, j->extraTot,
                                                          j->dR + l, stream));
                }
            } else {
                LX_TRY(sober_level_reduce_mfma_queued_pair(j->kind, (const double*)j->rows, j->n_rows, (const double*)j->cand,
                                                           j->dim, cur, Rub[l], S, SOBER_LEVEL_XS, j->mu, j->wmul,
                                                           j->outputscale, nch, j->partG, S, j->partTot, nxch, j->extraG,
                                                           j->extraTot, j->dR + l, stream));
            }
            LX_TRY(sober_sum_partials_queued(j->partG, j->partTot, j->n_rows, S, S, j->extraG, j->extraTot,
                                             SOBER_LEVEL_XS, j->G, S, j->tot, j->dR + l, tani ? 1 : 0, stream));
        }
        if (oj) {
            LX_TRY(sober_dgemm_coldiv_t(n, S, j->n_rows, j->P, j->n_rows, j->G, S, j->tot, oj->X_tmp, n + 1, stream));
            LX_TRY(sober_obj_set_sums_queued(oj->obj, j->mu, cur, S, j->dR + l, (l == 0 && first_sums_ready) ? R0 : (int64_t)-1,
                                             j->tot, oj->X_tmp + n, n + 1, oj->ocol, stream));
            LX_TRY(sober_car_device_ex(oj->X_tmp, n + 1, S, n + 2, j->tot, oj->kr1, oj->w1, oj->nk1, j->mu_out, nullptr,
                                       j->car_ws, j->car_ws_bytes, j->car_mode, stream));
            LX_TRY(sober_null_vector(oj->X_tmp, n + 1, S, n, oj->kr1, oj->nk1, n + 2, oj->null_row, oj->status, stream));
            LX_TRY(sober_second_elimination_rows(oj->null_row, oj->ocol, oj->w1, oj->kr1, oj->nk1, oj->status, n + 2, S,
                                                 j->keep_rank, j->w_star, j->keep_rank + S, stream));
        } else {
            LX_TRY(sober_dgemm_coldiv_t(n, S, j->n_rows, j->P, j->n_rows, j->G, S, j->tot, j->X_tmp, n, stream));
            LX_TRY(sober_car_device_ex(j->X_tmp, n, S, n + 1, j->tot, j->keep_rank, j->w_star, j->keep_rank + S, j->mu_out,
                                       nullptr, j->car_ws, j->car_ws_bytes, j->car_mode, stream));
        }
        LX_TRY(sober_level_update_queued_ex(cur, Rub[l], S, j->keep_rank, j->w_star, j->tot, j->mu, nxt, j->dR + l,
                                            j->dR + l + 1, Rub[l + 1], l < D ? b : 0, j->cls_scale, j->cls_sof,
                                            (l == 0 && first_sums_ready) ? R0 : (int64_t)-1, stream));
    }
    for (int k = 0; k < 4; ++k) j->ev[k] = nullptr;
    e = hipMemcpyAsync(j->h_dR, j->dR, sizeof(int64_t) * (size_t)(L + 1), hipMemcpyDeviceToHost, st);
    if (e != hipSuccess) return (int)e;
    e = hipStreamSynchronize(st);
    if (e != hipSuccess) return (int)e;
    j->h_dR[0] = R0;
    int d = 0;
    while (d < L && j->h_dR[d + 1] >= 0) { level_R[d] = j->h_dR[d]; ++d; }
    *done = d;
    *R_out = j->h_dR[d];
    return 0;
}

extern "C" int sober_level_loop_obj(sober_level_job* j, const sober_obj_job* oj, int64_t R, int32_t* idx_a, int32_t* idx_b,
                                    int first_sums_ready, int max_levels, int64_t* level_R, int32_t* n_levels, int64_t* R_final,
                                    int32_t* in_b, void* stream) {
    if (!j || !oj || !idx_a || !idx_b || !level_R || !n_levels || !R_final || !in_b || !j->mu || R <= 0 || !j->dR || !j->h_dR)
        return SOBER_E_ARG;
    if (!oj->obj || !oj->X_tmp || !oj->ocol || !oj->kr1 || !oj->w1 || !oj->nk1 || !oj->null_row || !oj->status) return SOBER_E_ARG;
    if (j->variant != SOBER_LEVEL_MFMA && j->variant != SOBER_LEVEL_TANI) return SOBER_E_ARG;
    int done = 0;
    int64_t R_after = R;
    j->ev_used[0] = j->ev_used[1] = 0;
    LX_TRY(lx_loop_queued(j, oj, R, idx_a, idx_b, first_sums_ready, nullptr, max_levels, level_R, &done, &R_after, stream));
    *n_levels = done;
    *R_final = R_after;
    *in_b = (done & 1) ? 1 : 0;
    return 0;
}

extern "C" int sober_level_loop(sober_level_job* j, int64_t R, int32_t* idx_a, int32_t* idx_b, int first_sums_ready,
                                void** events, int max_levels, int64_t* level_R, int32_t* n_levels, int64_t* R_final,
                                int32_t* in_b, void* stream) {
    if (!j || !idx_a || !idx_b || !level_R || !n_levels || !R_final || !in_b || !j->h_flags || !j->mu || R <= 0)
        return SOBER_E_ARG;
    const int S = j->S;
    int32_t *cur = idx_a, *nxt = idx_b;
    int levels = 0;
    j->ev_used[0] = j->ev_used[1] = 0;
    if (j->dR && j->h_dR && (j->variant == SOBER_LEVEL_MFMA || (j->variant == SOBER_LEVEL_TANI && !sober::switches().tani_no_queue))) {
        int done = 0;
        int64_t R_after = R;
        LX_TRY(lx_loop_queued(j, nullptr, R, idx_a, idx_b, first_sums_ready, events, max_levels, level_R, &done, &R_after, stream));
        if (done > 0) {
            levels = done;
            R = R_after;
            first_sums_ready = 0;
            if (done & 1) { cur = idx_b; nxt = idx_a; }
        }
    }
    while (R > S) {
        if (levels >= max_levels) return SOBER_E_WS;
        const int64_t E = R / S, r = R - E * S;
        j->idx = cur; j->pos0 = 0; j->count = R; j->E = E;
        j->phase = (levels == 0 && first_sums_ready) ? 2 : 0;
        for (int k = 0; k < 4; ++k) j->ev[k] = (events && levels < max_levels) ? events[4 * levels + k] : nullptr;
        if (j->phase != 2 && levels < 64) {
            if (j->ev[0] && j->ev[1]) j->ev_used[0] |= 1ull << levels;
            if (j->ev[2] && j->ev[3] && r > 0) j->ev_used[1] |= 1ull << levels;
        }
        LX_TRY(sober_level_moments(j, stream));
        LX_TRY(sober_level_car(j, stream));
        const hipError_t e = hipStreamSynchronize((hipStream_t)stream);
        if (e != hipSuccess) return (int)e;
        if (j->h_flags[S] < 0) {
            const int rc = sober_level_car_retry(j, stream);
            if (rc != 0) {
                *n_levels = levels; *R_final = R; *in_b = (cur == idx_b) ? 1 : 0;
                for (int k = 0; k < 4; ++k) j->ev[k] = nullptr;
                j->phase = 0;
                return rc;
            }
        }
        const int n_keep = j->h_flags[S];
        const bool last_kept = j->h_flags[S - 1] >= 0;
        const int64_t R_new = E * n_keep + (last_kept ? r : 0);
        level_R[levels++] = R;
        if (R_new >= R) { *n_levels = levels; return SOBER_E_NOPROGRESS; }
        LX_TRY(sober_level_update(cur, 0, R, S, E, j->keep_rank, j->w_star, j->tot, n_keep, j->mu, nxt, 0, stream));
        int32_t* t = cur; cur = nxt; nxt = t;
        R = R_new;
    }
    for (int k = 0; k < 4; ++k) j->ev[k] = nullptr;
    j->phase = 0;
    *n_levels = levels;
    *R_final = R;
    *in_b = (cur == idx_b) ? 1 : 0;
    return 0;
}

extern "C" int sober_level_final_job(const sober_level_job* j, const sober_final_job* f, const int32_t* idx, int R,
                                     void* stream) {
    if (!j || !f || !f->rows_sc || (!f->cand_sc && (!f->cand_raw || !f->ls || !f->sc_buf)) || !idx || !f->K || !f->mu_live ||
        !f->out_idx || !f->out_w || !j->P || !j->Xtr || !j->X_tmp || !j->keep_rank || !j->w_star || !j->mu_out || !j->car_ws ||
        !j->h_flags || !j->mu)
        return SOBER_E_ARG;
    const int S = j->S, n = j->n;
    if (R <= n + 1 || R > S || f->N <= 0) return SOBER_E_ARG;
    if (!sober_car_supported(R, n + 1)) return SOBER_E_DIM;
    if (f->cand_sc) {
        LX_TRY(sober_pairwise(j->kind, f->rows_sc, f->rows_norm, j->n_rows, f->cand_sc, f->cand_norm, idx, R, f->dt,
                              j->outputscale, f->K, R, stream));
    } else {
        LX_TRY(sober_scale_points_idx(f->cand_raw, idx, R, f->d_raw, f->ld_raw, f->ls, f->ls_len, f->sc_buf, f->dt, j->mu,
                                      f->mu_live, stream));
        LX_TRY(sober_pairwise(j->kind, f->rows_sc, f->rows_norm, j->n_rows, f->sc_buf, nullptr, nullptr, R, f->dt,
                              j->outputscale, f->K, R, stream));
    }
    LX_TRY(sober_dgemm_coldiv_t(n, R, j->n_rows, j->P, j->n_rows, f->K, R, nullptr, j->X_tmp, n, stream));
    if (f->cand_sc) LX_TRY(sober_gather_f64(j->mu, idx, R, f->mu_live, stream));
    LX_TRY(sober_car_device_ex(j->X_tmp, n, R, n + 1, f->mu_live, j->keep_rank, j->w_star, j->keep_rank + S, j->mu_out,
                               nullptr, j->car_ws, j->car_ws_bytes, j->car_mode, stream));
    LX_TRY(sober_final_commit(idx, R, j->keep_rank, j->w_star, j->keep_rank + S, f->row_offset, j->mu, f->N, f->out_idx,
                              f->out_w, stream));
    hipError_t e = hipMemcpyAsync(j->h_flags + S, j->keep_rank + S, sizeof(int32_t), hipMemcpyDeviceToHost, (hipStream_t)stream);
    return e == hipSuccess ? 0 : (int)e;
}

extern "C" int sober_level_final(const sober_level_job* j, const void* rows_sc, const double* rows_norm,
                                 const void* cand_sc, const double* cand_norm, int dt, const int32_t* idx, int R,
                                 int64_t N, int64_t row_offset, double* K, double* mu_live, int64_t* out_idx,
                                 double* out_w, void* stream) {
    if (!cand_sc) return SOBER_E_ARG;
    sober_final_job f = {};
    f.rows_sc = rows_sc; f.rows_norm = rows_norm; f.cand_sc = cand_sc; f.cand_norm = cand_norm; f.dt = dt;
    f.N = N; f.row_offset = row_offset; f.K = K; f.mu_live = mu_live; f.out_idx = out_idx; f.out_w = out_w;
    return sober_level_final_job(j, &f, idx, R, stream);
}

extern "C" int sober_final_job_size(void) { return (int)sizeof(sober_final_job); }

extern "C" int sober_level_loop_final(sober_level_job* j, sober_final_job* f, int64_t R, int32_t* idx_a, int32_t* idx_b,
                                      int first_sums_ready, void** events, int max_levels, int64_t* level_R,
                                      int32_t* n_levels, int64_t* R_final, int32_t* in_b, void* stream) {
    if (f) f->done = 0;
    const int rc = sober_level_loop(j, R, idx_a, idx_b, first_sums_ready, events, max_levels, level_R, n_levels, R_final,
                                    in_b, stream);
    if (rc != 0 || !f) return rc;
    const int S = j->S, n = j->n;
    const int64_t Rf = *R_final;
    if (Rf <= n + 1 || Rf > S) return 0;
    if (j->car_mode != SOBER_CAR_DEFAULT && j->car_mode != SOBER_CAR_SAFE) return 0;
    if (!sober_car_supported((int)Rf, n + 1)) return 0;
    if (j->car_mode == SOBER_CAR_SAFE && !sober_car_safe_supported((int)Rf, n + 1)) return 0;
    LX_TRY(sober_level_final_job(j, f, *in_b ? idx_b : idx_a, (int)Rf, stream));
    const hipError_t e = hipStreamSynchronize((hipStream_t)stream);
    if (e != hipSuccess) return (int)e;
    f->done = 1;
    return 0;
}

extern "C" int sober_record_event_pair(void* ev0, void* ev1, void* stream) {
    if (!ev0 || !ev1) return SOBER_E_ARG;
    hipError_t e = hipEventRecord((hipEvent_t)ev0, (hipStream_t)stream);
    if (e == hipSuccess) e = hipEventRecord((hipEvent_t)ev1, (hipStream_t)stream);
    return e == hipSuccess ? 0 : (int)e;
}

static int64_t lx_survivors_before(int64_t p, int S, int64_t E, const int32_t* kept_prefix, int n_keep, bool last_kept) {
    const int64_t ES = E * S;
    if (p <= ES) return (p / S) * n_keep + kept_prefix[p % S];
    return E * (int64_t)n_keep + (last_kept ? (p - ES) : 0);
}

extern "C" int sober_level_loop_sharded(sober_level_job* j, int rank, int world, int64_t* bounds, int32_t* idx_a,
                                        int32_t* idx_b, int first_sums_ready, sober_allreduce_fn allreduce,
                                        void* comm, int64_t R_stop, int max_levels, int64_t* level_R,
                                        int32_t* n_levels, int32_t* in_b, void* stream) {
    if (!j || !bounds || !idx_a || !idx_b || !allreduce || !level_R || !n_levels || !in_b || !j->h_flags || !j->mu ||
        world <= 0 || rank < 0 || rank >= world || world > 1024)
        return SOBER_E_ARG;
    const int S = j->S, n = j->n;
    if (j->Xtr + (size_t)n * S != j->tot) return SOBER_E_ARG;
    if (!sober_car_supported(S, n + 1)) return SOBER_E_DIM;
    hipStream_t st = (hipStream_t)stream;
    int32_t *cur = idx_a, *nxt = idx_b;
    int levels = 0;
    int32_t kept_prefix[1024 + 1];
    if (S > 1024) return SOBER_E_DIM;
    while (bounds[world] > S && bounds[world] > R_stop) {
        if (levels >= max_levels) return SOBER_E_WS;
        const int64_t R = bounds[world], E = R / S, r = R - E * S;
        const int64_t pos0 = bounds[rank], count = bounds[rank + 1] - bounds[rank];
        if (levels == 0 && first_sums_ready) {
            j->phase = 2;
            LX_TRY(sober_level_moments(j, stream));
        } else if (count > 0) {
            j->idx = cur; j->pos0 = pos0; j->count = count; j->E = E; j->phase = 0;
            LX_TRY(sober_level_moments(j, stream));
        } else {
            hipError_t e = hipMemsetAsync(j->Xtr, 0, sizeof(double) * ((size_t)n * S + S), st);
            if (e != hipSuccess) return (int)e;
        }
        if (world > 1 || comm) LX_TRY(allreduce(comm, j->Xtr, (int64_t)n * S + S, stream));
        LX_TRY(sober_level_car(j, stream));
        hipError_t e = hipStreamSynchronize(st);
        if (e != hipSuccess) return (int)e;
        if ((void*)allreduce == (void*)&sober_peer_allreduce_f64 && comm) {
            const int prc = sober_peer_status(comm, nullptr, 0, stream);
            if (prc != 0) { *n_levels = levels; *in_b = (cur == idx_b) ? 1 : 0; j->phase = 0; return prc; }
        }
        if (j->h_flags[S] < 0) {
            const int rc = sober_level_car_retry(j, stream);
            if (rc != 0) { *n_levels = levels; *in_b = (cur == idx_b) ? 1 : 0; j->phase = 0; return rc; }
        }
        const int n_keep = j->h_flags[S];
        const bool last_kept = j->h_flags[S - 1] >= 0;
        const int64_t R_new = E * n_keep + (last_kept ? r : 0);
        level_R[levels++] = R;
        if (R_new >= R) { *n_levels = levels; return SOBER_E_NOPROGRESS; }
        kept_prefix[0] = 0;
        for (int s = 0; s < S; ++s) kept_prefix[s + 1] = kept_prefix[s] + (j->h_flags[s] >= 0 ? 1 : 0);
        int64_t nb_lo = lx_survivors_before(bounds[rank], S, E, kept_prefix, n_keep, last_kept);
        if (count > 0)
            LX_TRY(sober_level_update(cur, pos0, count, S, E, j->keep_rank, j->w_star, j->tot, n_keep, j->mu, nxt,
                                      nb_lo, stream));
        for (int q = 0; q <= world; ++q) bounds[q] = lx_survivors_before(bounds[q], S, E, kept_prefix, n_keep, last_kept);
        int32_t* t = cur; cur = nxt; nxt = t;
    }
    j->phase = 0;
    *n_levels = levels;
    *in_b = (cur == idx_b) ? 1 : 0;
    return 0;
}
```

sober_amd/csrc/level_reduce_mfma.hip:

```cpp
#include "common.hpp"
#include <cstdlib>

namespace sober {

#include "kern_exp.inc"

template <int KIND, int KT>
__global__ __launch_bounds__(SOBER_LW_W * 64, 8 / SOBER_LW_W) void k_level_reduce_wave(
    const double* __restrict__ rows, int n_rows, const double* __restrict__ cand,
    const int32_t* __restrict__ idx, int64_t pos0, int64_t count, int S,
    const double* __restrict__ mu, const double* __restrict__ wmul, double os,
    int64_t e_first, int e_total,
    double* __restrict__ partG, int ldg, int col0,
    double* __restrict__ partTot, int64_t tot_limit,
    const int64_t* __restrict__ dR, int S_main, int leftover,
    int S_x, double* __restrict__ partG_x, int ldg_x, double* __restrict__ partTot_x, int grid_main, int wpt_ov) {
    constexpr int DA = 4 * KT;
    constexpr int W = SOBER_LW_W;
#ifdef LW_STAMPS
    unsigned long long st_[8] = {0, 0, 0, 0, 0, 0, 0, 0};
    unsigned long long* const st_out_ = (unsigned long long*)(partG + (size_t)6 * n_rows * ldg) + ((size_t)blockIdx.x * W + (threadIdx.x >> 6)) * 8;
#define LW_STAMP(K) do { unsigned long long t_; asm volatile("s_memrealtime %0\n\ts_waitcnt lgkmcnt(0)" : "=s"(t_) :: "memory"); st_[K] = t_; } while (0)
#define LW_STAMP_V(K, VAL) do { unsigned long long t_; asm volatile("s_memrealtime %0\n\ts_waitcnt lgkmcnt(0)" : "=s"(t_), "+v"(VAL) :: "memory"); st_[K] = t_; } while (0)
#define LW_STAMP_FLUSH() do { if ((threadIdx.x & 63) == 0) for (int k_ = 0; k_ < 8; ++k_) st_out_[k_] = st_[k_]; } while (0)
    LW_STAMP(0);
#else
#define LW_STAMP(K) do { } while (0)
#define LW_STAMP_V(K, VAL) do { } while (0)
#define LW_STAMP_FLUSH() do { } while (0)
#endif
    __shared__ double s_T[EXP_TAB];
    __shared__ double s_tot[W * 16];
    __shared__ double s_red[W * 16 * 64];

    int bid = blockIdx.x, gdim = gridDim.x;
    if (dR != nullptr) {
        const int64_t R = __hip_atomic_load(dR, __ATOMIC_RELAXED, __HIP_MEMORY_SCOPE_AGENT);
        if (R <= S_main) return;
        const int64_t ES = (R / S_main) * S_main;
        if (leftover == 2) {
            if (bid >= grid_main) {
                leftover = 1; bid -= grid_main; gdim -= grid_main;
                S = S_x; partG = partG_x; ldg = ldg_x; partTot = partTot_x;
            } else {
                leftover = 0; gdim = grid_main;
            }
        }
        if (!leftover) { count = R; tot_limit = ES; }
        else { idx += ES; count = R - ES; tot_limit = count; }
        if (count <= 0) return;
        pos0 = 0; e_first = 0;
        e_total = (int)((count + S - 1) / S);
    }
#ifdef LW_STAMPS
    { unsigned hw_, xc_; asm volatile("s_getreg_b32 %0, hwreg(HW_REG_HW_ID)" : "=s"(hw_)); asm volatile("s_getreg_b32 %0, hwreg(HW_REG_XCC_ID)" : "=s"(xc_));
      st_[1] = ((unsigned long long)xc_ << 32) | hw_; }
#endif
    const int tid = threadIdx.x, lane = tid & 63;
    const int wave = __builtin_amdgcn_readfirstlane(tid >> 6);
    const int lj = lane & 15, lk = lane >> 4;
    const int G = (S + 15) >> 4, RT = (n_rows + 63) >> 6;
    const int wpt = wpt_ov > 0 ? wpt_ov : level_wave_wpt(n_rows, e_total, S);
    const int n_slots = level_wave_slots(wpt);
    const int n_waves = G * RT * wpt;
    const int per_xcd = gdim >> 3;
    const int q = (bid & 7) * per_xcd + (bid >> 3);
    if (q * W >= n_waves) return;
    const int v = q * W + wave;
    const bool live = v < n_waves;
    const int tile = live ? v / wpt : -1, sub = live ? v - tile * wpt : 0;
    const int g = live ? tile / RT : 0, rt = live ? tile - g * RT : 0;
    const int e_base = e_total / wpt, e_rem = e_total - e_base * wpt;
    const int ea = live ? sub * e_base + min(sub, e_rem) : 0;
    const int eb = live ? ea + e_base + (sub < e_rem ? 1 : 0) : 0;
    const int row0 = rt * 64;
    const int s = g * 16 + lj;
    const bool s_ok = s < S;

    static_assert(SOBER_LW_W * 64 >= EXP_TAB, "one table entry per thread");
    if (tid < EXP_TAB) s_T[tid] = exp_tab_entry(tid);

    double afr[4][KT];
#pragma unroll
    for (int t = 0; t < 4; ++t) {
        const int r = min(row0 + 16 * t + lj, n_rows - 1);
#pragma unroll
        for (int ks = 0; ks < KT; ++ks) afr[t][ks] = rows[(size_t)r * DA + lk * KT + ks];
    }
    double4_t acc[4];
#pragma unroll
    for (int t = 0; t < 4; ++t) acc[t] = (double4_t){0.0, 0.0, 0.0, 0.0};
    double tot_acc = 0.0;

    const double* wm_ptr = wmul ? wmul : mu;
    const int rel0 = s - (int)(pos0 - e_first * S);
    const int cnt32 = (int)count;
    const int tl32 = (int)max((int64_t)INT32_MIN, min((int64_t)INT32_MAX, tot_limit - pos0));
#define LW_REL(e, R, OK)                                                                   \
    const int R = (e) * S + rel0;                                                          \
    const bool OK = s_ok && (e) < eb && R >= 0 && R < cnt32;
#define LW_IDX(e, C) C = idx[min(max((e) * S + rel0, 0), cnt32 - 1)];
#define LW_LOAD(e, C, Q)                                                                   \
    {                                                                                      \
        LW_REL(e, rl_, okl_)                                                               \
        m[Q] = mu[C];                                                                      \
        wv[Q] = wm_ptr[C];                                                                 \
        const double* src_ = cand + (size_t)C * DA + lk * KT;                              \
        _Pragma("unroll") for (int ks = 0; ks < KT; ++ks) b[Q][ks] = src_[ks];             \
        ok[Q] = okl_;                                                                      \
        okt[Q] = okl_ && rl_ < tl32;                                                       \
    }
#define LW_MFMA(Q)                                                                         \
    {                                                                                      \
        _Pragma("unroll") for (int t = 0; t < 4; ++t) cc[Q][t] = (double4_t){0.0, 0.0, 0.0, 0.0}; \
        _Pragma("unroll") for (int ks = 0; ks < KT; ++ks)                                  \
            _Pragma("unroll") for (int t = 0; t < 4; ++t)                                  \
                cc[Q][t] = __builtin_amdgcn_mfma_f64_16x16x4f64(afr[t][ks], b[Q][ks], cc[Q][t], 0, 0, 0); \
        w[Q] = ok[Q] ? (wmul ? m[Q] * wv[Q] : m[Q]) * os : 0.0;                            \
        tot_acc += okt[Q] ? m[Q] : 0.0;                                                    \
    }
#define LW_HALF(e, Q, QN)                                                                  \
    {                                                                                      \
        asm volatile("" : "+v"(cF));        \
        int cG_;                                                                           \
        LW_IDX((e) + 3, cG_)                                                               \
        LW_LOAD((e) + 2, cF, Q)                                                            \
        cF = cG_;                                                                          \
        __builtin_amdgcn_sched_barrier(0);                                                 \
        LW_MFMA(QN)                                                                        \
        _Pragma("unroll") for (int t = 0; t < 4; ++t) {                                    \
            double k_[4];                                                                  \
            const double4_t c_ = ccv[Q][t];                                                \
            kern_from_arg4<KIND>(c_, s_T, k_);                                             \
            _Pragma("unroll") for (int r = 0; r < 4; ++r) acc[t][r] = fma(k_[r], wcv[Q], acc[t][r]); \
             \
             \
             \
             \
                             \
            __builtin_amdgcn_sched_barrier(0x0008);                                        \
        }                                                                                  \
        LW_INTERLEAVE                                                                      \
    }

#if defined(LW_SCHED) && LW_SCHED > 0
#define LW_INTERLEAVE                                                                      \
    _Pragma("unroll") for (int i_ = 0; i_ < 4 * KT; ++i_) {                                \
        __builtin_amdgcn_sched_group_barrier(0x008, 1, 0);                                 \
        __builtin_amdgcn_sched_group_barrier(0x002, LW_SCHED, 0);                          \
    }
#else
#define LW_INTERLEAVE
#endif
    double4_t cc[2][4];
    double w[2];
    double b[2][KT], m[2], wv[2];
    bool ok[2], okt[2];
    int cA = 0, cB = 0, cF = 0;
    LW_IDX(ea, cA)
    LW_IDX(ea + 1, cB)
    LW_IDX(ea + 2, cF)
    __syncthreads();
    LW_STAMP(2);
    LW_STAMP_V(3, afr[3][KT - 1]);
    LW_LOAD(ea, cA, 0)
    LW_LOAD(ea + 1, cB, 1)
    LW_STAMP_V(4, b[1][KT - 1]);
    LW_MFMA(0)
#define ccv cc
#define wcv w
    int e = ea;
    for (; e + 1 < eb; e += 2) {
        LW_HALF(e, 0, 1)
        LW_HALF(e + 1, 1, 0)
    }
    if (e < eb) LW_HALF(e, 0, 1)
    LW_STAMP_V(5, acc[3][3]);
#undef ccv
#undef wcv
#undef LW_REL
#undef LW_IDX
#undef LW_LOAD
#undef LW_MFMA
#undef LW_HALF
#undef LW_INTERLEAVE

    __shared__ int s_tile[W];
#pragma unroll
    for (int t = 0; t < 4; ++t)
#pragma unroll
        for (int r = 0; r < 4; ++r) s_red[(wave * 16 + t * 4 + r) * 64 + lane] = acc[t][r];
    if (lk == 0) s_tot[wave * 16 + lj] = tot_acc;
    if (lane == 0) s_tile[wave] = tile;
    __syncthreads();
    LW_STAMP(6);
    if (!live || (wave > 0 && s_tile[wave - 1] == tile)) { LW_STAMP_FLUSH(); return; }
    for (int w = wave + 1; w < W && s_tile[w] == tile; ++w) {
#pragma unroll
        for (int t = 0; t < 4; ++t)
#pragma unroll
            for (int r = 0; r < 4; ++r) acc[t][r] += s_red[(w * 16 + t * 4 + r) * 64 + lane];
        tot_acc += s_tot[w * 16 + lj];
    }
    const int slot = q - (tile * wpt) / W;
    const int last_q = (tile * wpt + wpt - 1) / W;
    if (!s_ok) { LW_STAMP_FLUSH(); return; }
    for (int sl = slot; sl < (q == last_q ? n_slots : slot + 1); ++sl) {
        const bool mine = sl == slot;
#pragma unroll
        for (int t = 0; t < 4; ++t)
#pragma unroll
            for (int r = 0; r < 4; ++r) {
                const int row = row0 + 16 * t + lk + 4 * r;
                if (row < n_rows) partG[((size_t)sl * n_rows + row) * ldg + col0 + s] = mine ? acc[t][r] : 0.0;
            }
        if (partTot != nullptr && rt == 0 && lk == 0) partTot[(size_t)sl * ldg + col0 + s] = mine ? tot_acc : 0.0;
    }
    LW_STAMP(7);
    LW_STAMP_FLUSH();
}

template <int CTRL>
__device__ __forceinline__ double aug_dpp(double v) {
    int lo = __double2loint(v), hi = __double2hiint(v);
    lo = __builtin_amdgcn_mov_dpp(lo, CTRL, 0xf, 0xf, true);
    hi = __builtin_amdgcn_mov_dpp(hi, CTRL, 0xf, 0xf, true);
    return __hiloint2double(hi, lo);
}
__global__ __launch_bounds__(256) void k_augment_points(const double* __restrict__ X, int64_t n, int d, int64_t ldx,
                                                        const double* __restrict__ ls, int ls_len,
                                                        const double* __restrict__ center, int side,
                                                        double* __restrict__ out, int da) {
    const int64_t i = ((int64_t)blockIdx.x * blockDim.x + threadIdx.x) >> 4;
    const int l16 = threadIdx.x & 15;
    const bool live = i < n;
    const int64_t ir = live ? i : n - 1;
    const double sc = (side == 0) ? 369.3299304675746 : 1.0;
    double v[2], nrm = 0.0;
#pragma unroll
    for (int h = 0; h < 2; ++h) {
        const int j = l16 + 16 * h, jc = min(j, d - 1);
        const double x = (X[ir * ldx + jc] - center[jc]) / ls[ls_len == 1 ? 0 : jc];
        v[h] = (j < d) ? x : 0.0;
        nrm = fma(v[h], v[h], nrm);
    }
    nrm += aug_dpp<0x128>(nrm);
    nrm += aug_dpp<0x124>(nrm);
    nrm += aug_dpp<0x122>(nrm);
    nrm += aug_dpp<0x121>(nrm);
#pragma unroll
    for (int h = 0; h < 2; ++h) {
        const int j = l16 + 16 * h;
        double o = v[h] * sc;
        if (j == d + side) o = -0.5 * nrm * sc;
        else if (j == d + 1 - side) o = sc;
        else if (j >= d) o = 0.0;
        if (live && j < da) out[i * da + j] = o;
    }
}

__global__ __launch_bounds__(1024) void k_center_mean(const double* __restrict__ X, int64_t n, int d, int64_t ldx,
                                                      double* __restrict__ center) {
    __shared__ double s_p[32][33];
    const int j = threadIdx.x & 31, g = threadIdx.x >> 5;
    double acc = 0.0;
    if (j < d) {
#pragma unroll 4
        for (int64_t i = g; i < n; i += 32) acc += X[i * ldx + j];
    }
    s_p[g][j] = acc;
    __syncthreads();
    if (g == 0 && j < d) {
        double t = 0.0;
#pragma unroll
        for (int q = 0; q < 32; ++q) t += s_p[q][j];
        center[j] = t / (double)n;
    }
}

__global__ __launch_bounds__(256) void k_augment_all(const double* __restrict__ Xa, int64_t na, int64_t lda,
                                                     const double* __restrict__ Xb, int64_t nb, int64_t ldb,
                                                     const double* __restrict__ Xc, int64_t nc, int64_t ldc, int d,
                                                     const double* __restrict__ ls, int ls_len,
                                                     const double* __restrict__ center, double* __restrict__ rows_out,
                                                     double* __restrict__ cand_out, int da) {
    const int64_t i = ((int64_t)blockIdx.x * blockDim.x + threadIdx.x) >> 4;
    const int l16 = threadIdx.x & 15;
    const int64_t n_rows = na + nb, n_all = n_rows + nc;
    const bool live = i < n_all;
    const int64_t ir = live ? i : n_all - 1;
    const int side = ir < n_rows ? 0 : 1;
    const double* src = ir < na ? Xa + ir * lda : (ir < n_rows ? Xb + (ir - na) * ldb : Xc + (ir - n_rows) * ldc);
    double* dst = side == 0 ? rows_out + ir * da : cand_out + (ir - n_rows) * da;
    const double sc = (side == 0) ? 369.3299304675746 : 1.0;
    double v[2], nrm = 0.0;
#pragma unroll
    for (int h = 0; h < 2; ++h) {
        const int j = l16 + 16 * h, jc = min(j, d - 1);
        const double x = (src[jc] - center[jc]) / ls[ls_len == 1 ? 0 : jc];
        v[h] = (j < d) ? x : 0.0;
        nrm = fma(v[h], v[h], nrm);
    }
    nrm += aug_dpp<0x128>(nrm);
    nrm += aug_dpp<0x124>(nrm);
    nrm += aug_dpp<0x122>(nrm);
    nrm += aug_dpp<0x121>(nrm);
#pragma unroll
    for (int h = 0; h < 2; ++h) {
        const int j = l16 + 16 * h;
        double o = v[h] * sc;
        if (j == d + side) o = -0.5 * nrm * sc;
        else if (j == d + 1 - side) o = sc;
        else if (j >= d) o = 0.0;
        if (live && j < da) dst[j] = o;
    }
}

template <int KIND, int KT>
static int launch_lm(const double* rows, int n_rows, const double* cand, const int32_t* idx, int64_t pos0,
                     int64_t count, int S, const double* mu, const double* wmul, double os, int n_chunks,
                     double* partG, int ldg, int col0, double* partTot, int64_t tot_limit, hipStream_t st,
                     const int64_t* dR = nullptr, int S_main = 0, int leftover = 0, int S_x = 0, int n_xchunks = 0,
                     double* partG_x = nullptr, int ldg_x = 0, double* partTot_x = nullptr, int wpt_ov = 0) {
    const int64_t e_first = pos0 / S;
    const int e_total = (int)((pos0 + count + S - 1) / S - e_first);
    if (wpt_ov < 0 || wpt_ov > e_total || (wpt_ov > 0 && (dR != nullptr || leftover))) return SOBER_E_ARG;
    const int wpt = wpt_ov > 0 ? wpt_ov : level_wave_wpt(n_rows, e_total, S);
    if (n_chunks != level_wave_slots(wpt)) return SOBER_E_ARG;
    if (count + 2 * (int64_t)S > 0x7fffffffLL) return SOBER_E_ARG;
    const int64_t n_waves = level_wave_tiles(n_rows, S) * wpt;
    const int64_t n_wg = (n_waves + SOBER_LW_W - 1) / SOBER_LW_W;
    const int grid_main = (int)(8 * ((n_wg + 7) / 8));
    int grid_x = 0;
    if (leftover == 2) {
        const int e_x = (S_main - 1 + S_x - 1) / S_x;
        const int wpt_x = level_wave_wpt(n_rows, e_x, S_x);
        if (dR == nullptr || S_x <= 0 || n_xchunks != level_wave_slots(wpt_x) || !partG_x || ldg_x < S_x) return SOBER_E_ARG;
        const int64_t n_wg_x = (level_wave_tiles(n_rows, S_x) * wpt_x + SOBER_LW_W - 1) / SOBER_LW_W;
        grid_x = (int)(8 * ((n_wg_x + 7) / 8));
    }
    SOBER_LAUNCH_TIMED((k_level_reduce_wave<KIND, KT>), dim3((unsigned)(grid_main + grid_x)), dim3(SOBER_LW_W * 64), 0,
                       st, rows, n_rows, cand, idx, pos0, count, S, mu, wmul, os, e_first, e_total, partG, ldg, col0,
                       partTot, tot_limit, dR, S_main, leftover, S_x, partG_x, ldg_x, partTot_x, grid_main, wpt_ov);
    LAUNCH_CHECK();
    return 0;
}

}

using namespace sober;

extern "C" int sober_level_parts_mfma(int n_rows, int64_t pos0, int64_t count, int S) {
    if (n_rows <= 0 || pos0 < 0 || count <= 0 || S <= 0) return SOBER_E_ARG;
    return level_parts_mfma_for(n_rows, (pos0 + count + S - 1) / S - pos0 / S, S);
}

extern "C" int sober_level_parts_mfma_cap(int n_rows, int64_t e_total_ub, int S) {
    if (n_rows <= 0 || e_total_ub <= 0 || S <= 0) return SOBER_E_ARG;
    return level_parts_mfma_cap(n_rows, e_total_ub, S);
}

extern "C" int sober_aug_dim(int d) {
    if (d <= 0) return SOBER_E_ARG;
    const int da = ((d + 2 + 3) / 4) * 4;
    return da <= 32 ? da : SOBER_E_DIM;
}

extern "C" int sober_augment_points(const double* X, int64_t n, int d, int64_t ldx, const double* lengthscale,
                                    int ls_len, const double* center, int side, double* out, int da,
                                    void* stream) {
    if (!X || !lengthscale || !center || !out || n <= 0 || d <= 0 || ldx < d || da < d + 2) return SOBER_E_ARG;
    if ((ls_len != 1 && ls_len != d) || (side != 0 && side != 1)) return SOBER_E_ARG;
    if (da > 32) return SOBER_E_DIM;
    hipLaunchKernelGGL(k_augment_points, dim3((unsigned)((n + 15) / 16)), dim3(256), 0, (hipStream_t)stream, X, n,
                       d, ldx, lengthscale, ls_len, center, side, out, da);
    LAUNCH_CHECK();
    return 0;
}

extern "C" int sober_augment_plan(const double* X_nys, int64_t M, int64_t ld_nys, const double* X_obs, int64_t n_obs,
                                  int64_t ld_obs, const double* X_cand, int64_t N, int64_t ld_cand, int d,
                                  const double* lengthscale, int ls_len, double* center, double* rows_aug, double* cand_aug,
                                  int da, void* stream) {
    if (!X_nys || !X_cand || !lengthscale || !center || !rows_aug || !cand_aug || M <= 0 || N <= 0 || n_obs < 0 || d <= 0 ||
        (n_obs > 0 && !X_obs) || ld_nys < d || ld_cand < d || (n_obs > 0 && ld_obs < d) || da < d + 2)
        return SOBER_E_ARG;
    if ((ls_len != 1 && ls_len != d) || d > 30) return SOBER_E_ARG;
    if (da > 32) return SOBER_E_DIM;
    hipLaunchKernelGGL(k_center_mean, dim3(1), dim3(1024), 0, (hipStream_t)stream, X_nys, M, d, ld_nys, center);
    LAUNCH_CHECK();
    const int64_t n_all = M + n_obs + N;
    hipLaunchKernelGGL(k_augment_all, dim3((unsigned)((n_all + 15) / 16)), dim3(256), 0, (hipStream_t)stream, X_nys, M, ld_nys,
                       X_obs, n_obs, ld_obs, X_cand, N, ld_cand, d, lengthscale, ls_len, center, rows_aug, cand_aug, da);
    LAUNCH_CHECK();
    return 0;
}

static int level_reduce_mfma_impl(int kind, const double* rows, int n_rows, const double* cand, int da,
                                  const int32_t* idx, int64_t pos0, int64_t count, int S, const double* mu,
                                  const double* wmul, double outputscale, int n_chunks, double* partG,
                                  int ldg, int col0, double* partTot, int64_t tot_limit, void* stream,
                                  const int64_t* dR, int S_main, int leftover, int S_x = 0, int n_xchunks = 0,
                                  double* partG_x = nullptr, int ldg_x = 0, double* partTot_x = nullptr, int wpt_ov = 0);

extern "C" int sober_level_reduce_mfma(int kind, const double* rows, int n_rows, const double* cand, int da,
                                       const int32_t* idx, int64_t pos0, int64_t count, int S, const double* mu,
                                       const double* wmul, double outputscale, int n_chunks, double* partG,
                                       int ldg, int col0, double* partTot, int64_t tot_limit, void* stream) {
    return level_reduce_mfma_impl(kind, rows, n_rows, cand, da, idx, pos0, count, S, mu, wmul, outputscale, n_chunks,
                                  partG, ldg, col0, partTot, tot_limit, stream, nullptr, 0, 0);
}

extern "C" int sober_level_reduce_mfma_queued(int kind, const double* rows, int n_rows, const double* cand, int da,
                                              const int32_t* idx, int64_t count_ub, int S, int S_main,
                                              int leftover, const double* mu, const double* wmul,
                                              double outputscale, int n_chunks_ub, double* partG, int ldg,
                                              double* partTot, const int64_t* dR, void* stream) {
    if (!dR || S_main <= 0 || (!leftover && S != S_main)) return SOBER_E_ARG;
    return level_reduce_mfma_impl(kind, rows, n_rows, cand, da, idx, 0, count_ub, S, mu, wmul, outputscale,
                                  n_chunks_ub, partG, ldg, 0, partTot, 0, stream, dR, S_main, leftover);
}

extern "C" int sober_level_class_wpt(int n_rows, int64_t e_total, int S) {
    if (n_rows <= 0 || e_total <= 0 || S <= 0) return SOBER_E_ARG;
    return level_class_wpt(n_rows, e_total, S);
}
extern "C" int sober_level_class_slots(int wpt) { return wpt > 0 ? level_wave_slots(wpt) : SOBER_E_ARG; }
extern "C" int sober_level_reduce_mfma_wpt(int kind, const double* rows, int n_rows, const double* cand, int da,
                                           const int32_t* idx, int64_t count, int S, const double* mu,
                                           const double* wmul, double outputscale, int wpt, int n_chunks, double* partG,
                                           int ldg, double* partTot, void* stream) {
    if (wpt <= 0 || count <= 0 || S <= 0 || count % S != 0) return SOBER_E_ARG;
    return level_reduce_mfma_impl(kind, rows, n_rows, cand, da, idx, 0, count, S, mu, wmul, outputscale, n_chunks, partG,
                                  ldg, 0, partTot, count, stream, nullptr, 0, 0, 0, 0, nullptr, 0, nullptr, wpt);
}

extern "C" int sober_level_reduce_mfma_queued_pair(int kind, const double* rows, int n_rows, const double* cand, int da,
                                                   const int32_t* idx, int64_t count_ub, int S, int n_xcols,
                                                   const double* mu, const double* wmul, double outputscale,
                                                   int n_chunks_ub, double* partG, int ldg, double* partTot,
                                                   int n_xchunks_ub, double* extraG, double* extraTot,
                                                   const int64_t* dR, void* stream) {
    if (!dR || S <= 1 || n_xcols <= 0 || !extraG || !extraTot) return SOBER_E_ARG;
    return level_reduce_mfma_impl(kind, rows, n_rows, cand, da, idx, 0, count_ub, S, mu, wmul, outputscale,
                                  n_chunks_ub, partG, ldg, 0, partTot, 0, stream, dR, S, 2, n_xcols, n_xchunks_ub, extraG,
                                  n_xcols, extraTot);
}

static int level_reduce_mfma_impl(int kind, const double* rows, int n_rows, const double* cand, int da,
                                  const int32_t* idx, int64_t pos0, int64_t count, int S, const double* mu,
                                  const double* wmul, double outputscale, int n_chunks, double* partG,
                                  int ldg, int col0, double* partTot, int64_t tot_limit, void* stream,
                                  const int64_t* dR, int S_main, int leftover, int S_x, int n_xchunks,
                                  double* partG_x, int ldg_x, double* partTot_x, int wpt_ov) {
    if (!rows || !cand || !idx || !mu || !partG) return SOBER_E_ARG;
    if (n_rows <= 0 || pos0 < 0 || count <= 0 || S <= 0 || n_chunks <= 0 || ldg < col0 + S) return SOBER_E_ARG;
    hipStream_t st = (hipStream_t)stream;
#define LM_CASE(K, T)                                                                                          \
    case 4 * T:                                                                                                \
        return launch_lm<K, T>(rows, n_rows, cand, idx, pos0, count, S, mu, wmul, outputscale, n_chunks, partG, \
                               ldg, col0, partTot, tot_limit, st, dR, S_main, leftover, S_x, n_xchunks, partG_x,   \
                               ldg_x, partTot_x, wpt_ov);
    switch (kind) {
        case SOBER_KIND_RBF:
            switch (da) { LM_CASE(SOBER_KIND_RBF, 1) LM_CASE(SOBER_KIND_RBF, 2) LM_CASE(SOBER_KIND_RBF, 3)
                          LM_CASE(SOBER_KIND_RBF, 4) LM_CASE(SOBER_KIND_RBF, 5) LM_CASE(SOBER_KIND_RBF, 6)
                          LM_CASE(SOBER_KIND_RBF, 7) LM_CASE(SOBER_KIND_RBF, 8) default: return SOBER_E_DIM; }
        case SOBER_KIND_MATERN52:
            switch (da) { LM_CASE(SOBER_KIND_MATERN52, 1) LM_CASE(SOBER_KIND_MATERN52, 2)
                          LM_CASE(SOBER_KIND_MATERN52, 3) LM_CASE(SOBER_KIND_MATERN52, 4)
                          LM_CASE(SOBER_KIND_MATERN52, 5) LM_CASE(SOBER_KIND_MATERN52, 6)
                          LM_CASE(SOBER_KIND_MATERN52, 7) LM_CASE(SOBER_KIND_MATERN52, 8)
                          default: return SOBER_E_DIM; }
        default: return SOBER_E_ARG;
    }
#undef LM_CASE
}
```

Baseline: 27.32 million.

## Add fused small-level kernel combining kernel reduction and Nystrom projection

Adds a new single-launch kernel for late recombination levels with few candidates per subset (at most 125). It computes the kernel-row reductions with MFMA into LDS, then projects them through P straight into X_tmp, and combines split workgroups with an atomic last-block pattern. This replaces the multi-chunk reduce, partial-sum and dgemm_coldiv launches for those levels, cutting launch overhead and global traffic for partials. The cost is an extra workspace buffer, atomic cross-workgroup combining, and a second code path to keep correct.

After: 27.57 million, median of 2. About the same (+0.9%).

```diff
diff --git a/include/sober_hip.h b/include/sober_hip.h
--- a/include/sober_hip.h
+++ b/include/sober_hip.h
@@ -7,7 +7,7 @@
 extern "C" {
 #endif
 
-#define SOBER_ABI_VERSION 7
+#define SOBER_ABI_VERSION 8
 
 #define SOBER_KIND_RBF       0
 #define SOBER_KIND_MATERN52  1
@@ -194,6 +194,18 @@
 int sober_sum_partials_queued(const double* partG, const double* partTot, int n_rows, int ldg, int S,
                               const double* extraG, const double* extraTot, int n_xcols, double* G, int ldo,
                               double* tot, const int64_t* dR, int chunked, void* stream);
+#define SOBER_LEVEL_SMALL_E 125
+#define SOBER_LEVEL_SMALL_PREADS (16LL << 20)
+int sober_level_small_e(void);
+int sober_level_small_supported(int n_rows, int n, int da, int S, int64_t count_ub);
+int64_t sober_level_small_ws_doubles(int n, int S);
+int sober_level_small_queued(int kind, const double* rows, int n_rows, const double* cand, int da,
+                             const int32_t* idx, int64_t count_ub, int S, const double* mu, const double* wmul,
+                             double outputscale, const double* P, int n, const int64_t* dR, double* X_tmp, int ldx,
+                             double* tot, double* ws, int64_t ws_doubles, void* stream);
+int sober_level_small_sized(int kind, const double* rows, int n_rows, const double* cand, int da, const int32_t* idx,
+                            int64_t R, int S, const double* mu, const double* wmul, double outputscale, const double* P,
+                            int n, double* X_tmp, double* tot, double* Xtr, double* ws, int64_t ws_doubles, void* stream);
 int sober_level_reduce_tani_queued(const void* rows, const double* rows_norm, int n_rows, const void* cand,
                                    const double* cand_norm, int dt, const int32_t* idx, int64_t count_ub, int S,
                                    int S_main, int leftover, const double* mu, const double* wmul, double outputscale,
@@ -300,6 +312,7 @@
     int32_t class_depth;
     double* Gc[2]; double* totc[2];
     double* cls_scale; int32_t* cls_sof;
+    double* small_ws; int64_t small_ws_doubles;
 } sober_level_job;
 #define SOBER_LEVEL_QUEUE 24
 int sober_level_moments(const sober_level_job* job, void* stream);
diff --git a/sober_amd/_native.py b/sober_amd/_native.py
--- a/sober_amd/_native.py
+++ b/sober_amd/_native.py
@@ -8,7 +8,7 @@
 
 _HERE = os.path.dirname(os.path.abspath(__file__))
 LIB_PATH = os.environ.get("SOBER_HIP_LIB") or os.path.join(_HERE, "libsober_hip.so")
-ABI_VERSION = 7
+ABI_VERSION = 8
 
 KIND_RBF, KIND_MATERN52, KIND_TANIMOTO = 0, 1, 2
 KIND_BY_NAME = {"rbf": KIND_RBF, "matern52": KIND_MATERN52, "tanimoto": KIND_TANIMOTO}
@@ -138,6 +138,13 @@
                                               _i32, _vp, _i32, _vp, _vp, _vp]),
     "sober_level_reduce_mfma_queued_pair": (_i32, [_i32, _vp, _i32, _vp, _i32, _vp, _i64, _i32, _i32, _vp, _vp, _f64, _i32,
                                                    _vp, _i32, _vp, _i32, _vp, _vp, _vp, _vp]),
+    "sober_level_small_e": (_i32, []),
+    "sober_level_small_supported": (_i32, [_i32, _i32, _i32, _i32, _i64]),
+    "sober_level_small_ws_doubles": (_i64, [_i32, _i32]),
+    "sober_level_small_sized": (_i32, [_i32, _vp, _i32, _vp, _i32, _vp, _i64, _i32, _vp, _vp, _f64, _vp, _i32, _vp, _vp, _vp,
+                                       _vp, _i64, _vp]),
+    "sober_level_small_queued": (_i32, [_i32, _vp, _i32, _vp, _i32, _vp, _i64, _i32, _vp, _vp, _f64, _vp, _i32, _vp, _vp,
+                                        _i32, _vp, _vp, _i64, _vp]),
     "sober_sum_partials_queued": (_i32, [_vp, _vp, _i32, _i32, _i32, _vp, _vp, _i32, _vp, _i32, _vp, _vp, _i32, _vp]),
     "sober_level_reduce_tani_queued": (_i32, [_vp, _vp, _i32, _vp, _vp, _i32, _vp, _i64, _i32, _i32, _i32, _vp, _vp, _f64,
                                               _i32, _vp, _i32, _vp, _vp, _vp]),
@@ -216,6 +223,7 @@
         ("car_mode", _i32),
         ("ev_used", C.c_uint64 * 2),
         ("class_depth", _i32), ("Gc", _vp * 2), ("totc", _vp * 2), ("cls_scale", _vp), ("cls_sof", _vp),
+        ("small_ws", _vp), ("small_ws_doubles", _i64),
     ]
 
 E_DIM = -2
@@ -454,6 +462,39 @@
                                           _ptr(wmul), float(outputscale), n_chunks, partG.data_ptr(), ldg,
                                           col0, _ptr(partTot), tot_limit, _stream(mu)),
            "sober_level_reduce_mfma")
+
+
+def level_small_e() -> int:
+    return int(load().sober_level_small_e())
+
+
+def level_small_ws_doubles(n, S) -> int:
+    r = int(load().sober_level_small_ws_doubles(n, S))
+    _check(min(r, 0), "sober_level_small_ws_doubles")
+    return r
+
+
+def level_small_queued(kind, rows, cand, da, idx, count_ub, S, mu, wmul, outputscale, P, dR, X_tmp, tot, ws):
+    _req(ws, torch.float64, "ws")
+    _req(idx, torch.int32, "idx"); _req(mu, torch.float64, "mu"); _req(P, torch.float64, "P")
+    _req(tot, torch.float64, "tot"); _req(dR, torch.int64, "dR")
+    if X_tmp.dtype != torch.float64 or X_tmp.stride(1) != 1:
+        raise SoberHipError("X_tmp: need float64 rows with unit inner stride")
+    _check(load().sober_level_small_queued(kind, rows.data_ptr(), rows.shape[0], cand.data_ptr(), da, idx.data_ptr(),
+                                           count_ub, S, mu.data_ptr(), _ptr(wmul), float(outputscale), P.data_ptr(),
+                                           P.shape[0], dR.data_ptr(), X_tmp.data_ptr(), X_tmp.stride(0), tot.data_ptr(), ws.data_ptr(),
+                                           ws.numel(),
+                                           _stream(mu)),
+           "sober_level_small_queued")
+
+
+def level_small_sized(kind, rows, cand, da, idx, R, S, mu, wmul, outputscale, P, X_tmp, tot, Xtr, ws):
+    _req(idx, torch.int32, "idx"); _req(mu, torch.float64, "mu"); _req(P, torch.float64, "P"); _req(ws, torch.float64, "ws")
+    _req(X_tmp, torch.float64, "X_tmp"); _req(tot, torch.float64, "tot")
+    _check(load().sober_level_small_sized(kind, rows.data_ptr(), rows.shape[0], cand.data_ptr(), da, idx.data_ptr(), R, S,
+                                          mu.data_ptr(), _ptr(wmul), float(outputscale), P.data_ptr(), P.shape[0],
+                                          X_tmp.data_ptr(), tot.data_ptr(), _ptr(Xtr), ws.data_ptr(), ws.numel(), _stream(mu)),
+           "sober_level_small_sized")
 
 
 def sum_partials(partG, partTot, n_chunks, n_rows, ldg, S, extraG, extraTot, n_xchunks, n_xcols, G, tot):
diff --git a/sober_amd/_ops_levels.py b/sober_amd/_ops_levels.py
--- a/sober_amd/_ops_levels.py
+++ b/sober_amd/_ops_levels.py
@@ -58,6 +58,9 @@
             w["dR"] = torch.empty(nat.LEVEL_QUEUE + 1, dtype=torch.int64, device=dev)
             w["h_dR"] = torch.zeros(nat.LEVEL_QUEUE + 1, dtype=torch.int64, pin_memory=True)
             job.dR, job.h_dR = w["dR"].data_ptr(), w["h_dR"].data_ptr()
+            if job.variant == nat.LEVEL_MFMA:
+                w["small_ws"] = torch.zeros(nat.level_small_ws_doubles(n, S), dtype=f64, device=dev)
+                job.small_ws, job.small_ws_doubles = w["small_ws"].data_ptr(), w["small_ws"].numel()
             if S % 2 == 0:
                 cl = 1 << nat.CLASS_MAX_DEPTH
                 w["Gc"] = [torch.empty(nr * S * (cl >> k), dtype=f64, device=dev) for k in (0, 1)]
diff --git a/sober_amd/csrc/level_entry.inc b/sober_amd/csrc/level_entry.inc
--- /dev/null
+++ b/sober_amd/csrc/level_entry.inc
@@ -0,0 +1,39 @@
+#pragma once
+
+
+#define LEVEL_FRAG_LOAD(KT_, ROW, LK, F)                                                   \
+    {                                                                                      \
+        const double* src_ = (ROW) + (LK) * (KT_);                                         \
+        _Pragma("unroll") for (int ks = 0; ks < (KT_); ++ks) F[ks] = src_[ks];             \
+    }
+
+#define LEVEL_ARGS_MFMA(KT_, AFR, B, CC)                                                   \
+    {                                                                                      \
+        _Pragma("unroll") for (int t = 0; t < 4; ++t) CC[t] = (double4_t){0.0, 0.0, 0.0, 0.0}; \
+        _Pragma("unroll") for (int ks = 0; ks < (KT_); ++ks)                               \
+            _Pragma("unroll") for (int t = 0; t < 4; ++t)                                  \
+                CC[t] = __builtin_amdgcn_mfma_f64_16x16x4f64(AFR[t][ks], B[ks], CC[t], 0, 0, 0); \
+    }
+
+#define LEVEL_ENTRIES_ADD(KIND_, C, T, W, ACC)                                             \
+    {                                                                                      \
+        double k_[4];                                                                      \
+        const double4_t c_ = C;                                                            \
+        kern_from_arg4<KIND_>(c_, T, k_);                                                  \
+        _Pragma("unroll") for (int r = 0; r < 4; ++r) ACC[r] = fma(k_[r], W, ACC[r]);      \
+    }
+
+template <int CTRL>
+__device__ __forceinline__ double aug_dpp(double v) {
+    int lo = __double2loint(v), hi = __double2hiint(v);
+    lo = __builtin_amdgcn_mov_dpp(lo, CTRL, 0xf, 0xf, true);
+    hi = __builtin_amdgcn_mov_dpp(hi, CTRL, 0xf, 0xf, true);
+    return __hiloint2double(hi, lo);
+}
+__device__ __forceinline__ double row16_sum(double v) {
+    v += aug_dpp<0x128>(v);
+    v += aug_dpp<0x124>(v);
+    v += aug_dpp<0x122>(v);
+    v += aug_dpp<0x121>(v);
+    return v;
+}
diff --git a/sober_amd/csrc/level_exec.cpp b/sober_amd/csrc/level_exec.cpp
--- a/sober_amd/csrc/level_exec.cpp
+++ b/sober_amd/csrc/level_exec.cpp
@@ -100,6 +100,8 @@
     return sober_class_sum(j->partG, j->partTot, nch, j->n_rows, S, CL, j->Gc[0], j->totc[0], j->G, j->tot, stream);
 }
 
+static bool lx_small_level(const sober_level_job* j, const sober_obj_job* oj, int64_t R_ub);
+
 extern "C" int sober_level_moments(const sober_level_job* j, void* stream) {
     if (!j || !j->G || !j->tot || j->n_rows <= 0 || j->S <= 0 || j->n <= 0 || j->phase < 0 || j->phase > 2)
         return SOBER_E_ARG;
@@ -112,6 +114,12 @@
         return SOBER_E_ARG;
     if (j->count <= 0 || j->pos0 < 0 || j->E < 0) return SOBER_E_ARG;
     if (j->phase == 1 && j->class_depth > 0) return lx_class_first(j, stream);
+    if (j->phase == 0 && j->pos0 == 0 && j->count > S && j->count / S == j->E && lx_small_level(j, nullptr, j->count)) {
+        LX_EVENTS_BEFORE(j->ev[0], j->ev[1])
+        return sober_level_small_sized(j->kind, (const double*)j->rows, j->n_rows, (const double*)j->cand, j->dim, j->idx,
+                                       j->count, S, j->mu, j->wmul, j->outputscale, j->P, j->n, j->X_tmp, j->tot, j->Xtr,
+                                       j->small_ws, j->small_ws_doubles, stream);
+    }
     const int64_t ES = j->E * S;
     const bool mfma = j->variant == SOBER_LEVEL_MFMA;
     const bool tani_k = j->variant == SOBER_LEVEL_TANI;
@@ -171,6 +179,15 @@
 
 static int lx_chunks(int n_rows, int64_t e_total, int S) { return sober_level_parts_mfma_cap(n_rows, e_total, S); }
 
+static bool lx_small_level(const sober_level_job* j, const sober_obj_job* oj, int64_t R_ub) {
+    if (j->variant != SOBER_LEVEL_MFMA || !j->P || !j->X_tmp || !j->small_ws || (oj && !oj->X_tmp)) return false;
+    if (j->small_ws_doubles < sober_level_small_ws_doubles(j->n, j->S)) return false;
+    if (j->kind != SOBER_KIND_RBF && j->kind != SOBER_KIND_MATERN52) return false;
+    if ((R_ub + j->S - 1) / j->S > SOBER_LEVEL_SMALL_E) return false;
+    if ((int64_t)j->S * j->n * j->n_rows > SOBER_LEVEL_SMALL_PREADS) return false;
+    return sober_level_small_supported(j->n_rows, j->n, j->dim, j->S, R_ub) != 0;
+}
+
 static int lx_loop_queued(sober_level_job* j, const sober_obj_job* oj, int64_t R0, int32_t* idx_a, int32_t* idx_b,
                           int first_sums_ready, void** events, int max_levels, int64_t* level_R, int* done, int64_t* R_out,
                           void* stream) {
@@ -203,10 +220,19 @@
         int32_t* cur = (l & 1) ? idx_b : idx_a;
         int32_t* nxt = (l & 1) ? idx_a : idx_b;
         for (int k = 0; k < 4; ++k) j->ev[k] = events ? events[4 * l + k] : nullptr;
+        bool projected = false;
         if (l >= 1 && l <= D) {
             LX_TRY(sober_class_derive_queued(j->Gc[(l - 1) & 1], j->totc[(l - 1) & 1], j->n_rows, S, 1 << (D - l + 1),
                                              j->cls_scale, j->cls_sof, j->Gc[l & 1], j->totc[l & 1], j->G, j->tot, j->dR + l,
                                              stream));
+        } else if (!(l == 0 && first_sums_ready) && lx_small_level(j, oj, Rub[l])) {
+            LX_EVENTS_BEFORE(j->ev[0], j->ev[1])
+            if (j->ev[0] && j->ev[1]) j->ev_used[0] |= 1ull << l;
+            LX_TRY(sober_level_small_queued(j->kind, (const double*)j->rows, j->n_rows, (const double*)j->cand, j->dim, cur,
+                                            Rub[l], S, j->mu, j->wmul, j->outputscale, j->P, n, j->dR + l,
+                                            oj ? oj->X_tmp : j->X_tmp, oj ? n + 1 : n, j->tot, j->small_ws,
+                                            j->small_ws_doubles, stream));
+            projected = true;
         } else if (!(l == 0 && first_sums_ready)) {
             const bool tani = j->variant == SOBER_LEVEL_TANI;
             const int64_t e_ub = (Rub[l] + S - 1) / S, ex_ub = (S - 1 + SOBER_LEVEL_XS - 1) / SOBER_LEVEL_XS;
@@ -254,7 +280,8 @@
                                              SOBER_LEVEL_XS, j->G, S, j->tot, j->dR + l, tani ? 1 : 0, stream));
         }
         if (oj) {
-            LX_TRY(sober_dgemm_coldiv_t(n, S, j->n_rows, j->P, j->n_rows, j->G, S, j->tot, oj->X_tmp, n + 1, stream));
+            if (!projected)
+                LX_TRY(sober_dgemm_coldiv_t(n, S, j->n_rows, j->P, j->n_rows, j->G, S, j->tot, oj->X_tmp, n + 1, stream));
             LX_TRY(sober_obj_set_sums_queued(oj->obj, j->mu, cur, S, j->dR + l, (l == 0 && first_sums_ready) ? R0 : (int64_t)-1,
                                              j->tot, oj->X_tmp + n, n + 1, oj->ocol, stream));
             LX_TRY(sober_car_device_ex(oj->X_tmp, n + 1, S, n + 2, j->tot, oj->kr1, oj->w1, oj->nk1, j->mu_out, nullptr,
@@ -263,7 +290,8 @@
             LX_TRY(sober_second_elimination_rows(oj->null_row, oj->ocol, oj->w1, oj->kr1, oj->nk1, oj->status, n + 2, S,
                                                  j->keep_rank, j->w_star, j->keep_rank + S, stream));
         } else {
-            LX_TRY(sober_dgemm_coldiv_t(n, S, j->n_rows, j->P, j->n_rows, j->G, S, j->tot, j->X_tmp, n, stream));
+            if (!projected)
+                LX_TRY(sober_dgemm_coldiv_t(n, S, j->n_rows, j->P, j->n_rows, j->G, S, j->tot, j->X_tmp, n, stream));
             LX_TRY(sober_car_device_ex(j->X_tmp, n, S, n + 1, j->tot, j->keep_rank, j->w_star, j->keep_rank + S, j->mu_out,
                                        nullptr, j->car_ws, j->car_ws_bytes, j->car_mode, stream));
         }
diff --git a/sober_amd/csrc/level_reduce_mfma.hip b/sober_amd/csrc/level_reduce_mfma.hip
--- a/sober_amd/csrc/level_reduce_mfma.hip
+++ b/sober_amd/csrc/level_reduce_mfma.hip
@@ -4,6 +4,7 @@
 namespace sober {
 
 #include "kern_exp.inc"
+#include "level_entry.inc"
 
 template <int KIND, int KT>
 __global__ __launch_bounds__(SOBER_LW_W * 64, 8 / SOBER_LW_W) void k_level_reduce_wave(
@@ -84,8 +85,7 @@
 #pragma unroll
     for (int t = 0; t < 4; ++t) {
         const int r = min(row0 + 16 * t + lj, n_rows - 1);
-#pragma unroll
-        for (int ks = 0; ks < KT; ++ks) afr[t][ks] = rows[(size_t)r * DA + lk * KT + ks];
+        LEVEL_FRAG_LOAD(KT, rows + (size_t)r * DA, lk, afr[t])
     }
     double4_t acc[4];
 #pragma unroll
@@ -105,17 +105,13 @@
         LW_REL(e, rl_, okl_)                                                               \
         m[Q] = mu[C];                                                                      \
         wv[Q] = wm_ptr[C];                                                                 \
-        const double* src_ = cand + (size_t)C * DA + lk * KT;                              \
-        _Pragma("unroll") for (int ks = 0; ks < KT; ++ks) b[Q][ks] = src_[ks];             \
+        LEVEL_FRAG_LOAD(KT, cand + (size_t)C * DA, lk, b[Q])                               \
         ok[Q] = okl_;                                                                      \
         okt[Q] = okl_ && rl_ < tl32;                                                       \
     }
 #define LW_MFMA(Q)                                                                         \
     {                                                                                      \
-        _Pragma("unroll") for (int t = 0; t < 4; ++t) cc[Q][t] = (double4_t){0.0, 0.0, 0.0, 0.0}; \
-        _Pragma("unroll") for (int ks = 0; ks < KT; ++ks)                                  \
-            _Pragma("unroll") for (int t = 0; t < 4; ++t)                                  \
-                cc[Q][t] = __builtin_amdgcn_mfma_f64_16x16x4f64(afr[t][ks], b[Q][ks], cc[Q][t], 0, 0, 0); \
+        LEVEL_ARGS_MFMA(KT, afr, b[Q], cc[Q])                                               \
         w[Q] = ok[Q] ? (wmul ? m[Q] * wv[Q] : m[Q]) * os : 0.0;                            \
         tot_acc += okt[Q] ? m[Q] : 0.0;                                                    \
     }
@@ -129,10 +125,7 @@
         __builtin_amdgcn_sched_barrier(0);                                                 \
         LW_MFMA(QN)                                                                        \
         _Pragma("unroll") for (int t = 0; t < 4; ++t) {                                    \
-            double k_[4];                                                                  \
-            const double4_t c_ = ccv[Q][t];                                                \
-            kern_from_arg4<KIND>(c_, s_T, k_);                                             \
-            _Pragma("unroll") for (int r = 0; r < 4; ++r) acc[t][r] = fma(k_[r], wcv[Q], acc[t][r]); \
+            LEVEL_ENTRIES_ADD(KIND, ccv[Q][t], s_T, wcv[Q], acc[t])                       \
              \
              \
              \
@@ -220,13 +213,6 @@
     LW_STAMP_FLUSH();
 }
 
-template <int CTRL>
-__device__ __forceinline__ double aug_dpp(double v) {
-    int lo = __double2loint(v), hi = __double2hiint(v);
-    lo = __builtin_amdgcn_mov_dpp(lo, CTRL, 0xf, 0xf, true);
-    hi = __builtin_amdgcn_mov_dpp(hi, CTRL, 0xf, 0xf, true);
-    return __hiloint2double(hi, lo);
-}
 __global__ __launch_bounds__(256) void k_augment_points(const double* __restrict__ X, int64_t n, int d, int64_t ldx,
                                                         const double* __restrict__ ls, int ls_len,
                                                         const double* __restrict__ center, int side,
diff --git a/sober_amd/csrc/level_small.hip b/sober_amd/csrc/level_small.hip
--- /dev/null
+++ b/sober_amd/csrc/level_small.hip
@@ -0,0 +1,305 @@
+#include "common.hpp"
+#include <cstdlib>
+
+namespace sober {
+
+#include "kern_exp.inc"
+#include "level_entry.inc"
+
+#define LS_WAVES 8
+#define LS_THREADS (LS_WAVES * 64)
+#define LS_MAX_LDS (60 * 1024)
+#define LS_XCOLS 16
+
+typedef double double2_t __attribute__((ext_vector_type(2)));
+
+__host__ __device__ inline size_t level_small_lds(int n_rows, int64_t cols_cap) {
+    return sizeof(double) * (size_t)(((n_rows + 63) / 64) * 64) + (size_t)cols_cap * (2 * sizeof(double) + sizeof(int32_t));
+}
+static inline int64_t level_small_cols(int64_t count_ub, int S) { return count_ub / S + 1 + LS_XCOLS; }
+__host__ __device__ inline int level_small_xwg(int S) { return (S - 1 + LS_XCOLS - 1) / LS_XCOLS; }
+static inline int64_t level_small_ws(int n, int S) { return 1 + (int64_t)(1 + level_small_xwg(S)) * (n + 1); }
+
+template <int VEC> struct LsVec;
+template <> struct LsVec<1> {
+    typedef double type;
+    static __device__ __forceinline__ double get(const double& v, int) { return v; }
+};
+template <> struct LsVec<2> {
+    typedef double2_t type;
+    static __device__ __forceinline__ double get(const double2_t& v, int c) { return v[c]; }
+};
+
+template <int VEC, int NO, int U>
+__device__ __forceinline__ void ls_dots(const double* (&p)[NO], const double* __restrict__ g, int n_rows, int l16,
+                                        double (&a)[NO]) {
+    typedef typename LsVec<VEC>::type vec_t;
+#pragma unroll
+    for (int o = 0; o < NO; ++o) a[o] = 0.0;
+    for (int k0 = l16 * VEC; k0 < n_rows; k0 += 16 * VEC * U) {
+        vec_t v[NO][U];
+#pragma unroll
+        for (int u = 0; u < U; ++u) {
+            const int kc = min(k0 + 16 * VEC * u, n_rows - VEC);
+#pragma unroll
+            for (int o = 0; o < NO; ++o) v[o][u] = *(const vec_t*)(p[o] + kc);
+        }
+#pragma unroll
+        for (int u = 0; u < U; ++u) {
+            const int k = k0 + 16 * VEC * u;
+            const bool ok = k < n_rows;
+            const vec_t gv = *(const vec_t*)(g + min(k, n_rows - VEC));
+#pragma unroll
+            for (int c = 0; c < VEC; ++c) {
+                const double gc = ok ? LsVec<VEC>::get(gv, c) : 0.0;
+#pragma unroll
+                for (int o = 0; o < NO; ++o) a[o] = fma(LsVec<VEC>::get(v[o][u], c), gc, a[o]);
+            }
+        }
+    }
+#pragma unroll
+    for (int o = 0; o < NO; ++o) a[o] = row16_sum(a[o]);
+}
+
+template <int KIND, int KT>
+__global__ __launch_bounds__(LS_THREADS) void k_level_small(
+    const double* __restrict__ rows, int n_rows, const double* __restrict__ cand, const int32_t* __restrict__ idx,
+    int64_t count_ub, int S, const double* __restrict__ mu, const double* __restrict__ wmul, double os,
+    const double* __restrict__ P, int n, int p_vec2, const int64_t* __restrict__ dR, double* __restrict__ X_tmp,
+    double* __restrict__ tot, int cols_cap, double* ws, int64_t R_val, double* __restrict__ Xtr, int ldx) {
+    constexpr int DA = 4 * KT;
+    extern __shared__ double s_dyn[];
+    __shared__ double s_T[EXP_TAB];
+    __shared__ double s_tot;
+    __shared__ int s_last;
+    const int RT = (n_rows + 63) >> 6;
+    double* const s_g = s_dyn;
+    double* const s_w = s_g + RT * 64;
+    double* const s_m = s_w + cols_cap;
+    int32_t* const s_c = (int32_t*)(s_m + cols_cap);
+
+    const bool extra = (int)blockIdx.x >= S;
+    const int s = extra ? S - 1 : (int)blockIdx.x;
+    const int x = extra ? (int)blockIdx.x - S : 0;
+    const int tid = threadIdx.x, lane = tid & 63;
+    const int wave = __builtin_amdgcn_readfirstlane(tid >> 6);
+    const int lj = lane & 15, lk = lane >> 4;
+
+    if (tid < EXP_TAB) s_T[tid] = exp_tab_entry(tid);
+    double afr[4][KT];
+#pragma unroll
+    for (int t = 0; t < 4; ++t) {
+        const int r = min(wave * 64 + 16 * t + lj, n_rows - 1);
+        LEVEL_FRAG_LOAD(KT, rows + (size_t)r * DA, lk, afr[t])
+    }
+
+    const int64_t R = dR != nullptr ? __hip_atomic_load(dR, __ATOMIC_RELAXED, __HIP_MEMORY_SCOPE_AGENT) : R_val;
+    if (R <= S || R > count_ub) return;
+    const int E = (int)(R / S);
+    const int64_t ES = (int64_t)E * S;
+    const int r_left = (int)(R - ES);
+    const int n_x = (r_left + LS_XCOLS - 1) / LS_XCOLS;
+    if (extra && x >= n_x) return;
+    const int n_main = extra ? 0 : E + (s < r_left ? 1 : 0);
+    const int x_first = x * LS_XCOLS;
+    const int n_cols = extra ? min(LS_XCOLS, r_left - x_first) : n_main;
+    const bool shared = (s == S - 1) && r_left > 0;
+
+    for (int q = tid; q < n_cols; q += LS_THREADS) {
+        const int64_t p = extra ? ES + x_first + q : (int64_t)q * S + s;
+        const int32_t c = idx[p];
+        const double m = mu[c];
+        s_c[q] = c;
+        s_w[q] = (wmul ? m * wmul[c] : m) * os;
+        s_m[q] = (extra || q < E) ? m : 0.0;
+    }
+    __syncthreads();
+    if (wave == LS_WAVES - 1) {
+        double a = 0.0;
+        for (int q = lane; q < n_cols; q += 64) a += s_m[q];
+#pragma unroll
+        for (int o = 32; o >= 1; o >>= 1) a += __shfl_xor(a, o, 64);
+        if (lane == 0) {
+            s_tot = a;
+            if (!shared) tot[s] = a;
+        }
+    }
+
+    const int ncg = (n_cols + 15) >> 4;
+    for (int rt = wave; rt < RT; rt += LS_WAVES) {
+        if (rt != wave) {
+#pragma unroll
+            for (int t = 0; t < 4; ++t) {
+                const int r = min(rt * 64 + 16 * t + lj, n_rows - 1);
+                LEVEL_FRAG_LOAD(KT, rows + (size_t)r * DA, lk, afr[t])
+            }
+        }
+        double4_t acc[4];
+#pragma unroll
+        for (int t = 0; t < 4; ++t) acc[t] = (double4_t){0.0, 0.0, 0.0, 0.0};
+        double b[2][KT], w[2];
+        double4_t cc[4];
+#define LS_LOAD(CG, Q)                                                                     \
+        {                                                                                  \
+            const int q_ = (CG) * 16 + lj, qc_ = min(q_, n_cols - 1);                      \
+            const int32_t c_ = s_c[qc_];                                                   \
+            w[Q] = q_ < n_cols ? s_w[qc_] : 0.0;                                           \
+            LEVEL_FRAG_LOAD(KT, cand + (size_t)c_ * DA, lk, b[Q])                          \
+        }
+#define LS_STEP(Q)                                                                         \
+        {                                                                                  \
+            LEVEL_ARGS_MFMA(KT, afr, b[Q], cc)                                             \
+            _Pragma("unroll") for (int t = 0; t < 4; ++t) LEVEL_ENTRIES_ADD(KIND, cc[t], s_T, w[Q], acc[t]) \
+        }
+        LS_LOAD(0, 0)
+        for (int cg = 0; cg < ncg; cg += 2) {
+            LS_LOAD(cg + 1, 1)
+            LS_STEP(0)
+            if (cg + 1 < ncg) {
+                LS_LOAD(cg + 2, 0)
+                LS_STEP(1)
+            }
+        }
+#undef LS_LOAD
+#undef LS_STEP
+#pragma unroll
+        for (int t = 0; t < 4; ++t)
+#pragma unroll
+            for (int r = 0; r < 4; ++r) {
+                const double v = row16_sum(acc[t][r]);
+                if (lj == 0) s_g[rt * 64 + 16 * t + lk + 4 * r] = v;
+            }
+    }
+    __syncthreads();
+
+    const double tv = s_tot;
+    const int grp = tid >> 4, l16 = tid & 15;
+    constexpr int NG = LS_THREADS / 16, NO = 4;
+    const int slot = extra ? 1 + x : 0, n_part = 1 + n_x;
+    double* const slots = ws + 1;
+    const size_t ld = (size_t)n + 1;
+    for (int i = grp; i < n; i += NO * NG) {
+        const double* pr[NO];
+#pragma unroll
+        for (int o = 0; o < NO; ++o) pr[o] = P + (size_t)min(i + o * NG, n - 1) * n_rows;
+        double a[NO];
+        if (p_vec2) ls_dots<2, NO, 11>(pr, s_g, n_rows, l16, a);
+        else ls_dots<1, NO, 11>(pr, s_g, n_rows, l16, a);
+        if (l16 == 0) {
+#pragma unroll
+            for (int o = 0; o < NO; ++o) {
+                const int io = i + o * NG;
+                if (io < n) {
+                    if (!shared) {
+                        X_tmp[(size_t)s * ldx + io] = a[o] / tv;
+                        if (Xtr != nullptr) Xtr[(size_t)io * S + s] = a[o];
+                    } else __hip_atomic_store(slots + slot * ld + io, a[o], __ATOMIC_RELAXED, __HIP_MEMORY_SCOPE_AGENT);
+                }
+            }
+        }
+    }
+    if (!shared) return;
+
+    if (tid == 0) __hip_atomic_store(slots + slot * ld + n, tv, __ATOMIC_RELAXED, __HIP_MEMORY_SCOPE_AGENT);
+    __syncthreads();
+    if (tid == 0) {
+        const unsigned before = __hip_atomic_fetch_add((unsigned*)ws, 1u, __ATOMIC_ACQ_REL, __HIP_MEMORY_SCOPE_AGENT);
+        s_last = before + 1u == (unsigned)n_part ? 1 : 0;
+        if (s_last) __hip_atomic_store((unsigned*)ws, 0u, __ATOMIC_RELAXED, __HIP_MEMORY_SCOPE_AGENT);
+    }
+    __syncthreads();
+    if (!s_last) return;
+    __builtin_amdgcn_fence(__ATOMIC_ACQUIRE, "agent");
+    double mass = 0.0;
+    for (int k = 0; k < n_part; ++k) mass += __hip_atomic_load(slots + k * ld + n, __ATOMIC_RELAXED, __HIP_MEMORY_SCOPE_AGENT);
+    for (int i = tid; i < n; i += LS_THREADS) {
+        double a = 0.0;
+        for (int k = 0; k < n_part; ++k) a += __hip_atomic_load(slots + k * ld + i, __ATOMIC_RELAXED, __HIP_MEMORY_SCOPE_AGENT);
+        X_tmp[(size_t)s * ldx + i] = a / mass;
+        if (Xtr != nullptr) Xtr[(size_t)i * S + s] = a;
+    }
+    if (tid == 0) tot[s] = mass;
+}
+
+template <int KIND, int KT>
+static int launch_ls(const double* rows, int n_rows, const double* cand, const int32_t* idx, int64_t count_ub, int S,
+                     const double* mu, const double* wmul, double os, const double* P, int n, const int64_t* dR,
+                     double* X_tmp, int ldx, double* tot, double* ws, int64_t R_val, double* Xtr, hipStream_t st) {
+    const int64_t cols_cap = level_small_cols(count_ub, S);
+    const size_t lds = level_small_lds(n_rows, cols_cap);
+    const int p_vec2 = ((n_rows & 1) == 0 && ((uintptr_t)P & 15) == 0 && n_rows >= 2) ? 1 : 0;
+    SOBER_LAUNCH_TIMED((k_level_small<KIND, KT>), dim3((unsigned)(S + level_small_xwg(S))), dim3(LS_THREADS), lds, st, rows,
+                       n_rows, cand, idx, count_ub, S, mu, wmul, os, P, n, p_vec2, dR, X_tmp, tot, (int)cols_cap, ws,
+                       R_val, Xtr, ldx);
+    LAUNCH_CHECK();
+    return 0;
+}
+
+}
+
+using namespace sober;
+
+extern "C" int sober_level_small_e(void) { return SOBER_LEVEL_SMALL_E; }
+
+extern "C" int64_t sober_level_small_ws_doubles(int n, int S) {
+    if (n <= 0 || S <= 1) return SOBER_E_ARG;
+    return level_small_ws(n, S);
+}
+
+extern "C" int sober_level_small_supported(int n_rows, int n, int da, int S, int64_t count_ub) {
+    if (n_rows <= 0 || n <= 0 || S <= 1 || count_ub <= 0 || da < 4 || da > 32 || (da & 3)) return 0;
+    if (count_ub + 2 * (int64_t)S > 0x7fffffffLL) return 0;
+    return level_small_lds(n_rows, level_small_cols(count_ub, S)) <= LS_MAX_LDS ? 1 : 0;
+}
+
+static int level_small_impl(int kind, const double* rows, int n_rows, const double* cand, int da, const int32_t* idx,
+                            int64_t count_ub, int S, const double* mu, const double* wmul, double outputscale,
+                            const double* P, int n, const int64_t* dR, int64_t R_val, double* X_tmp, int ldx, double* tot, double* Xtr,
+                            double* ws, int64_t ws_doubles, void* stream);
+
+extern "C" int sober_level_small_queued(int kind, const double* rows, int n_rows, const double* cand, int da,
+                                        const int32_t* idx, int64_t count_ub, int S, const double* mu, const double* wmul,
+                                        double outputscale, const double* P, int n, const int64_t* dR, double* X_tmp,
+                                        int ldx, double* tot, double* ws, int64_t ws_doubles, void* stream) {
+    if (!dR || ldx < n) return SOBER_E_ARG;
+    return level_small_impl(kind, rows, n_rows, cand, da, idx, count_ub, S, mu, wmul, outputscale, P, n, dR, 0, X_tmp, ldx, tot,
+                            nullptr, ws, ws_doubles, stream);
+}
+
+extern "C" int sober_level_small_sized(int kind, const double* rows, int n_rows, const double* cand, int da,
+                                       const int32_t* idx, int64_t R, int S, const double* mu, const double* wmul,
+                                       double outputscale, const double* P, int n, double* X_tmp, double* tot, double* Xtr,
+                                       double* ws, int64_t ws_doubles, void* stream) {
+    if (R <= S) return SOBER_E_ARG;
+    return level_small_impl(kind, rows, n_rows, cand, da, idx, R, S, mu, wmul, outputscale, P, n, nullptr, R, X_tmp, n, tot,
+                            Xtr, ws, ws_doubles, stream);
+}
+
+static int level_small_impl(int kind, const double* rows, int n_rows, const double* cand, int da, const int32_t* idx,
+                            int64_t count_ub, int S, const double* mu, const double* wmul, double outputscale,
+                            const double* P, int n, const int64_t* dR, int64_t R_val, double* X_tmp, int ldx, double* tot, double* Xtr,
+                            double* ws, int64_t ws_doubles, void* stream) {
+    if (!rows || !cand || !idx || !mu || !P || !X_tmp || !tot || !ws) return SOBER_E_ARG;
+    if (n_rows <= 0 || n <= 0 || S <= 1 || count_ub <= 0) return SOBER_E_ARG;
+    if (ws_doubles < level_small_ws(n, S)) return SOBER_E_WS;
+    if (kind != SOBER_KIND_RBF && kind != SOBER_KIND_MATERN52) return SOBER_E_ARG;
+    if (!sober_level_small_supported(n_rows, n, da, S, count_ub)) return SOBER_E_DIM;
+    hipStream_t st = (hipStream_t)stream;
+#define LS_CASE(K, T)                                                                                          \
+    case 4 * T:                                                                                                \
+        return launch_ls<K, T>(rows, n_rows, cand, idx, count_ub, S, mu, wmul, outputscale, P, n, dR, X_tmp, ldx, tot, ws, R_val, \
+                               Xtr, st);
+    switch (kind) {
+        case SOBER_KIND_RBF:
+            switch (da) { LS_CASE(SOBER_KIND_RBF, 1) LS_CASE(SOBER_KIND_RBF, 2) LS_CASE(SOBER_KIND_RBF, 3)
+                          LS_CASE(SOBER_KIND_RBF, 4) LS_CASE(SOBER_KIND_RBF, 5) LS_CASE(SOBER_KIND_RBF, 6)
+                          LS_CASE(SOBER_KIND_RBF, 7) LS_CASE(SOBER_KIND_RBF, 8) default: return SOBER_E_DIM; }
+        default:
+            switch (da) { LS_CASE(SOBER_KIND_MATERN52, 1) LS_CASE(SOBER_KIND_MATERN52, 2)
+                          LS_CASE(SOBER_KIND_MATERN52, 3) LS_CASE(SOBER_KIND_MATERN52, 4)
+                          LS_CASE(SOBER_KIND_MATERN52, 5) LS_CASE(SOBER_KIND_MATERN52, 6)
+                          LS_CASE(SOBER_KIND_MATERN52, 7) LS_CASE(SOBER_KIND_MATERN52, 8)
+                          default: return SOBER_E_DIM; }
+    }
+#undef LS_CASE
+}
```
